# scale-lab/MTLoRA

Measured on AMD Instinct MI355X. Metric: images/sec (train step) Swin-T/448 r=64 4-task, higher is better.
Workload: dtype bf16; 1 GPU; BASELINE configs[1]: Swin-T 448, 4 tasks (semseg,normals,sal,human_parts), r_shared=64 r_task=4 scale4; train step (fwd+loss+bwd+clip+AdamW), dropout .05, drop_path .2; per_gpu_batch=32, global_batch=32, img_size=448, parallelism=dp1, trainable_params=8344634, allreduce_bytes=0

## Files before the change

### include/mtlora_hip.h

```cpp
#ifndef MTLORA_HIP_H
#define MTLORA_HIP_H

#include <stdint.h>

#ifdef __cplusplus
extern "C" {
#endif

#define MTLORA_ABI_VERSION 12
#define MTLORA_MAX_TASKS 8

typedef enum mtlora_dtype {
    MTLORA_F32 = 0,
    MTLORA_BF16 = 1,
    MTLORA_F16 = 2,
    MTLORA_U8 = 3
} mtlora_dtype;

typedef enum mtlora_status {
    MTLORA_OK = 0,
    MTLORA_ERR_DTYPE = -1,
    MTLORA_ERR_SHAPE = -2,
    MTLORA_ERR_ALIGN = -3,
    MTLORA_ERR_NULL = -4,
// ... 82 lines not shown
int mtlora_mlp_hid_proj(const mtlora_linear_desc* d1, const mtlora_linear_desc* d2, const void* h_base, const void* ctx1,
                        void* ctx2, void* scratch, int64_t scratch_bytes, void* stream);
int mtlora_mlp_hid_bwd(const mtlora_linear_desc* d1, const mtlora_linear_desc* d2, const void* h_base, const void* dh_s,
                       const void* ctx1, const void* ctx2, const void* scratch2, void* scratch1, void* g, float* const* dB1_t,
                       float* const* dA2_t, void* part, int64_t part_bytes, void* stream);

int64_t mtlora_gemm_tn_scratch_bytes(int64_t M, int Na, int Nb);
int mtlora_gemm_tn(const void* a, const void* b, float* out, int64_t M, int Na, int Nb, int64_t lda, int64_t ldb,
                   int dtype, void* scratch, int64_t scratch_bytes, void* stream);

typedef struct mtlora_attn_desc {
    int64_t B;
    int32_t H, W;
    int32_t window_size;
    int32_t shift;
    int32_t num_heads;
    int32_t head_dim;
    int32_t image_layout;
    int32_t dtype;
    float scale;
    float mask_value;
} mtlora_attn_desc;

int64_t mtlora_window_attn_bwd_scratch_bytes(const mtlora_attn_desc* d);

int mtlora_window_attn_fwd(const mtlora_attn_desc* d, const void* qkv, const float* bias, const float* mask,
                           const int32_t* mask_ids, void* out, void* stream);
int mtlora_window_attn_bwd(const mtlora_attn_desc* d, const void* qkv, const float* bias, const float* mask,
                           const int32_t* mask_ids, const void* dout, void* dqkv, float* dbias, void* scratch,
                           int64_t scratch_bytes, void* stream);

int mtlora_layernorm_fwd(const void* x, const float* gamma, const float* beta, void* y, float* mean, float* rstd,
                         int64_t M, int64_t C, float eps, int x_dtype, int y_dtype, int merge_h, int merge_w, void* stream);
int64_t mtlora_layernorm_bwd_scratch_bytes(int64_t M, int64_t C, int x_dtype);
int mtlora_layernorm_bwd(const void* dy, const void* x, const float* gamma, const float* mean, const float* rstd,
                         void* dx, float* dgamma, float* dbeta, int64_t M, int64_t C, int x_dtype, int dy_dtype,
                         void* scratch, int64_t scratch_bytes, const void* dx_addend, int merge_h, int merge_w, void* stream);

int mtlora_residual_layernorm_fwd(const void* shortcut, const void* branch, const float* scale, int64_t B, const float* gamma,
                                  const float* beta, void* x_new, void* y, float* mean, float* rstd, int64_t M, int64_t C,
                                  float eps, int x_dtype, int y_dtype, void* stream);
int mtlora_residual_layernorm_bwd(const void* dy, const void* x_new, const float* gamma, const float* mean, const float* rstd,
                                  void* d_shortcut, void* d_branch, float* dgamma, float* dbeta, const float* scale,
                                  int64_t B, int64_t M, int64_t C, int x_dtype, int dy_dtype, void* scratch,
                                  int64_t scratch_bytes, const void* dx_addend, void* stream);

int64_t mtlora_layernorm_multi_bwd_scratch_bytes(int n, int64_t M, int64_t C, int x_dtype);
int mtlora_layernorm_multi_fwd(int n, const void* const* x, const float* gamma, const float* beta, void* const* y,
                               float* const* mean, float* const* rstd, int64_t M, int64_t C, float eps, int x_dtype, int y_dtype,
                               int merge_h, int merge_w, void* stream);
int mtlora_layernorm_multi_bwd(int n, const void* const* dy, const void* const* x, const float* gamma, const float* const* mean,
                               const float* const* rstd, void* const* dx, float* dgamma, float* dbeta, int64_t M, int64_t C,
                               int x_dtype, int dy_dtype, void* scratch, int64_t scratch_bytes, const void* const* dx_addend,
                               int merge_h, int merge_w, void* stream);

int mtlora_residual_layernorm_streams_fwd(int n, const void* const* res, const void* const* branch, const float* scale,
                                          int64_t B, const float* gamma, const float* beta, void* const* x_new, void* const* y,
                                          float* const* mean, float* const* rstd, int64_t M, int64_t C, float eps, int x_dtype,
                                          int y_dtype, int merge_h, int merge_w, void* stream);
int mtlora_residual_layernorm_streams_bwd(int n, const void* const* dy, const void* const* x_new, const float* gamma,
                                          const float* const* mean, const float* const* rstd, void* const* d_res,
                                          void* const* d_branch, float* dgamma, float* dbeta, const float* scale, int64_t B,
                                          int64_t M, int64_t C, int x_dtype, int dy_dtype, void* scratch, int64_t scratch_bytes,
                                          const void* const* dx_addend, int merge_h, int merge_w, void* stream);

int mtlora_residual_layernorm_multi_fwd(int n, const void* shortcut, const void* const* branch, const float* scale, int64_t B,
                                        const float* gamma, const float* beta, void* const* x_new, void* const* y,
                                        float* const* mean, float* const* rstd, int64_t M, int64_t C, float eps, int x_dtype,
                                        int y_dtype, void* stream);
int mtlora_residual_layernorm_multi_bwd(int n, const void* const* dy, const void* const* x_new, const float* gamma,
                                        const float* const* mean, const float* const* rstd, const void* const* dx_addend,
                                        void* d_shortcut, void* const* d_branch, float* dgamma, float* dbeta, const float* scale,
                                        int64_t B, int64_t M, int64_t C, int x_dtype, int dy_dtype, void* scratch,
                                        int64_t scratch_bytes, void* stream);

int64_t mtlora_bn_scratch_bytes(int64_t R, int64_t C, int dtype);
int mtlora_bn_relu_fwd(const void* x, const float* gamma, const float* beta, float* running_mean, float* running_var,
                       float momentum, float eps, int relu, void* y, float* save_mean, float* save_rstd,
                       float* save_scale, float* save_shift, int64_t R, int64_t C, int dtype, void* scratch,
                       int64_t scratch_bytes, void* stream);
int mtlora_bn_relu_bwd(const void* dy, const void* x, const float* save_mean, const float* save_rstd,
                       const float* save_scale, const float* save_shift, int relu, void* dx, float* dgamma, float* dbeta,
                       int64_t R, int64_t C, int dtype, void* scratch, int64_t scratch_bytes, void* stream);

int mtlora_residual_droppath_fwd(int n, const void* const* res, const void* const* y, void* const* out,
                                 const float* scale, int64_t M, int64_t C, int64_t B, int res_dtype, int y_dtype,
                                 void* stream);
int mtlora_residual_droppath_bwd(int n, const void* const* g, void* const* dy, void* dres, const float* scale,
                                 int64_t M, int64_t C, int64_t B, int res_dtype, int y_dtype, void* stream);

int64_t mtlora_upsample_loss_partials(int64_t B, int h, int w, int scale);
int mtlora_upsample_loss(int kind, const void* low, const float* label, const float* stat, void* dlow, float* partials,
                         int64_t B, int h, int w, int C, int scale, int dtype, float ignore_index, void* stream);

int mtlora_upsample_metrics_sizes(int kind, int64_t B, int h, int w, int C, int scale, int64_t* n_int64,
                                  int64_t* n_float_partials);
int mtlora_upsample_metrics(int kind, const void* low, const float* label, const float* stat, int64_t* counts,
                            float* fpartials, int64_t B, int h, int w, int C, int scale, int dtype, float ignore_index,
                            void* stream);

int mtlora_upsample_predict(int kind, const void* low, void* out, int64_t B, int h, int w, int C, int scale, int dtype,
                            int out_dtype, void* stream);

int64_t mtlora_colsum_scratch_bytes(int64_t M, int64_t N);
int mtlora_colsum(const void* x, int64_t M, int64_t N, int dtype, float* out, void* scratch, int64_t scratch_bytes, void* stream);
int64_t mtlora_label_stat_scratch_bytes(int64_t n);
int mtlora_label_stat(const float* label, int64_t n, int kind, float ignore_index, float* out, void* scratch,
                      int64_t scratch_bytes, void* stream);

int mtlora_upsample_cl_fwd(const void* coarse, void* fine, int64_t B, int h, int w, int C, int scale, int64_t ld_fine,
                           int dtype, void* stream);
int mtlora_upsample_cl_bwd(const void* grad_fine, void* grad_coarse, int64_t B, int h, int w, int C, int scale,
                           int64_t ld_fine, int dtype, void* stream);

typedef struct mtlora_block_desc {
    int64_t B;
    int32_t H, W, C, hidden;
    int32_t num_heads, window_size, shift;
    int32_t dtype;
    int32_t x_dtype;
    int32_t has_norm1;
    float eps1, eps2, eps_next;
    float attn_scale, mask_value;
    mtlora_linear_desc lin[4];
} mtlora_block_desc;

typedef struct mtlora_block_params {
    const float *norm1_g, *norm1_b;
    const float *norm2_g, *norm2_b, *next_g, *next_b;
    const void* W[4];
    const void* Wt[4];
    const float* bias[4];
    const float* A[4];
    const float* Bf[4];
    const float* attn_bias;
    const int32_t* mask_ids;
    const float* mask;
    const float *scale1, *scale2;
} mtlora_block_params;

typedef struct mtlora_block_grads {
    void* g_x;
    void* g_normed;
    float *d_norm1_g, *d_norm1_b;
    float *d_norm2_g, *d_norm2_b, *d_next_g, *d_next_b;
    float* dA[4];
    float* dB[4];
    float* dbias;
} mtlora_block_grads;

int64_t mtlora_block_save_bytes(const mtlora_block_desc* d);
int64_t mtlora_block_fwd_tmp_bytes(const mtlora_block_desc* d);
int64_t mtlora_block_bwd_scratch_bytes(const mtlora_block_desc* d);
int mtlora_block_fwd(const mtlora_block_desc* d, const mtlora_block_params* p, const void* x, const void* normed, void* x_out,
                     void* normed_out, void* save, int64_t save_bytes, void* tmp, int64_t tmp_bytes, void* stream);
int mtlora_block_bwd(const mtlora_block_desc* d, const mtlora_block_params* p, const void* x, const void* normed,
                     const void* x_out, const void* g_x_out, const void* g_normed_out, const void* save, int64_t save_bytes,
                     const mtlora_block_grads* g, void* scratch, int64_t scratch_bytes, int phase, void* stream);

#define MTLORA_ADAMW_CHUNK 4096
#define MTLORA_ADAMW_MAX_GROUPS 16
#define MTLORA_ADAMW_CTRL_WORDS 64
#define MTLORA_ADAMW_GROUPS_DEV_BYTES 1152
typedef struct mtlora_adamw_group {
    double lr, beta1, beta2, eps, weight_decay;
} mtlora_adamw_group;
// ... 76 lines not shown
```

### mtlora_amd/_lib.py

```python
from __future__ import annotations

import ctypes
import os
from ctypes import POINTER, Structure, c_char_p, c_double, c_float, c_int, c_int32, c_int64, c_uint64, c_void_p

import torch

MAX_TASKS = 8
ABI_VERSION = 12
F32, BF16, F16, U8 = 0, 1, 2, 3
_DT = {torch.float32: F32, torch.bfloat16: BF16, torch.float16: F16}

_HERE = os.path.dirname(os.path.abspath(__file__))
LIB_PATH = os.path.join(_HERE, "csrc", "libmtlora_hip.so")


class LinearDesc(Structure):
    _fields_ = [("M", c_int64), ("K", c_int64), ("N", c_int64), ("dtype", c_int32), ("mode", c_int32),
                ("T", c_int32), ("r_s", c_int32), ("r_t", c_int32 * MAX_TASKS), ("scale_s", c_float),
                ("scale_t", c_float * MAX_TASKS), ("has_x_tasks", c_int32), ("dropout_p", c_float),
                ("seed", c_uint64), ("seed_offset", c_void_p), ("bwd_phase", c_int32),
                ("sel_stream", c_int32), ("sel_dense", c_int32), ("sel_tn", c_int32), ("sel_projk", c_int32),
                ("max_cu", c_int32), ("packed", c_void_p),
                ("hid", c_int32), ("hid_pad_", c_int32), ("hid_ptr", c_void_p)]
# ... 61 lines not shown


PtrArr = c_void_p * MAX_TASKS
PtrArr9 = c_void_p * (MAX_TASKS + 1)

_SIGS = {
    "mtlora_version": (c_int, []),
    "mtlora_error_string": (c_char_p, [c_int]),
    "mtlora_roll_and_window_partition_forward": (c_int, [c_void_p, c_void_p, c_int64, c_int64, c_int64, c_int64, c_int, c_int, c_int, c_void_p]),
    "mtlora_roll_and_window_partition_backward": (c_int, [c_void_p, c_void_p, c_int64, c_int64, c_int64, c_int64, c_int, c_int, c_int, c_void_p]),
    "mtlora_window_merge_and_roll_forward": (c_int, [c_void_p, c_void_p, c_int64, c_int64, c_int64, c_int64, c_int, c_int, c_int, c_void_p]),
    "mtlora_window_merge_and_roll_backward": (c_int, [c_void_p, c_void_p, c_int64, c_int64, c_int64, c_int64, c_int, c_int, c_int, c_void_p]),
    "mtlora_linear_ctx_bytes": (c_int64, [POINTER(LinearDesc)]),
    "mtlora_linear_bwd_scratch_bytes": (c_int64, [POINTER(LinearDesc)]),
    "mtlora_linear_packed_bytes": (c_int64, [POINTER(LinearDesc)]),
    "mtlora_linear_pack": (c_int, [POINTER(LinearDesc), c_void_p, c_void_p, POINTER(c_void_p), POINTER(c_void_p), c_void_p, c_int64,
                                   c_void_p]),
    "mtlora_linear_pack_entry_bytes": (c_int64, []),
    "mtlora_linear_pack_entry": (c_int, [POINTER(LinearDesc), c_void_p, c_void_p, POINTER(c_void_p), POINTER(c_void_p), c_void_p, c_int64,
                                         c_void_p]),
    "mtlora_linear_pack_table": (c_int, [c_void_p, c_int, c_int, c_void_p]),
    "mtlora_linear_fwd": (c_int, [POINTER(LinearDesc), c_void_p, POINTER(c_void_p), c_void_p, c_void_p, c_void_p, c_void_p,
                                  POINTER(c_void_p), POINTER(c_void_p), c_void_p, POINTER(c_void_p), c_void_p, c_int64,
                                  c_void_p]),
    "mtlora_linear_bwd": (c_int, [POINTER(LinearDesc), c_void_p, POINTER(c_void_p), c_void_p, c_void_p, POINTER(c_void_p),
                                  c_void_p, c_int64, c_void_p, POINTER(c_void_p), c_void_p, c_void_p, POINTER(c_void_p),
                                  POINTER(c_void_p), c_void_p, c_int64, c_void_p]),
    "mtlora_gemm_tn_scratch_bytes": (c_int64, [c_int64, c_int, c_int]),
    "mtlora_gemm_tn": (c_int, [c_void_p, c_void_p, c_void_p, c_int64, c_int, c_int, c_int64, c_int64, c_int, c_void_p, c_int64,
                               c_void_p]),
    "mtlora_linear_fwd_gelu": (c_int, [POINTER(LinearDesc), c_void_p, POINTER(c_void_p), c_void_p, c_void_p, c_void_p, c_void_p,
                                       POINTER(c_void_p), POINTER(c_void_p), c_void_p, POINTER(c_void_p), c_void_p,
                                       POINTER(c_void_p), c_void_p, c_int64, c_void_p]),
    "mtlora_linear_bwd_gelu": (c_int, [POINTER(LinearDesc), c_void_p, POINTER(c_void_p), c_void_p, c_void_p, POINTER(c_void_p),
                                       c_void_p, c_int64, c_void_p, POINTER(c_void_p), c_void_p, c_void_p, POINTER(c_void_p),
                                       POINTER(c_void_p), c_void_p, c_int64, c_void_p, POINTER(c_void_p), c_void_p]),
    "mtlora_mlp_hid_supported": (c_int, [POINTER(LinearDesc), POINTER(LinearDesc)]),
    "mtlora_mlp_hid_bwd_scratch_bytes": (c_int64, [POINTER(LinearDesc), POINTER(LinearDesc)]),
    "mtlora_mlp_hid_fwd_scratch_bytes": (c_int64, [POINTER(LinearDesc), POINTER(LinearDesc)]),
    "mtlora_mlp_hid_proj": (c_int, [POINTER(LinearDesc), POINTER(LinearDesc), c_void_p, c_void_p, c_void_p, c_void_p, c_int64, c_void_p]),
    "mtlora_mlp_hid_bwd": (c_int, [POINTER(LinearDesc), POINTER(LinearDesc), c_void_p, c_void_p, c_void_p, c_void_p, c_void_p, c_void_p,
                                   c_void_p, POINTER(c_void_p), POINTER(c_void_p), c_void_p, c_int64, c_void_p]),
    "mtlora_window_attn_bwd_scratch_bytes": (c_int64, [POINTER(AttnDesc)]),
    "mtlora_window_attn_fwd": (c_int, [POINTER(AttnDesc), c_void_p, c_void_p, c_void_p, c_void_p, c_void_p, c_void_p]),
    "mtlora_window_attn_bwd": (c_int, [POINTER(AttnDesc), c_void_p, c_void_p, c_void_p, c_void_p, c_void_p, c_void_p,
                                       c_void_p, c_void_p, c_int64, c_void_p]),
    "mtlora_layernorm_fwd": (c_int, [c_void_p, c_void_p, c_void_p, c_void_p, c_void_p, c_void_p, c_int64, c_int64, c_float,
                                     c_int, c_int, c_int, c_int, c_void_p]),
    "mtlora_layernorm_bwd_scratch_bytes": (c_int64, [c_int64, c_int64, c_int]),
    "mtlora_residual_layernorm_fwd": (c_int, [c_void_p, c_void_p, c_void_p, c_int64, c_void_p, c_void_p, c_void_p, c_void_p,
                                              c_void_p, c_void_p, c_int64, c_int64, c_float, c_int, c_int, c_void_p]),
    "mtlora_layernorm_multi_bwd_scratch_bytes": (c_int64, [c_int, c_int64, c_int64, c_int]),
    "mtlora_layernorm_multi_fwd": (c_int, [c_int, POINTER(c_void_p), c_void_p, c_void_p, POINTER(c_void_p), POINTER(c_void_p),
                                           POINTER(c_void_p), c_int64, c_int64, c_float, c_int, c_int, c_int, c_int, c_void_p]),
    "mtlora_layernorm_multi_bwd": (c_int, [c_int, POINTER(c_void_p), POINTER(c_void_p), c_void_p, POINTER(c_void_p),
                                           POINTER(c_void_p), POINTER(c_void_p), c_void_p, c_void_p, c_int64, c_int64, c_int,
                                           c_int, c_void_p, c_int64, POINTER(c_void_p), c_int, c_int, c_void_p]),
    "mtlora_residual_layernorm_streams_fwd": (c_int, [c_int, POINTER(c_void_p), POINTER(c_void_p), c_void_p, c_int64, c_void_p,
                                                      c_void_p, POINTER(c_void_p), POINTER(c_void_p), POINTER(c_void_p),
                                                      POINTER(c_void_p), c_int64, c_int64, c_float, c_int, c_int, c_int, c_int,
                                                      c_void_p]),
    "mtlora_residual_layernorm_streams_bwd": (c_int, [c_int, POINTER(c_void_p), POINTER(c_void_p), c_void_p, POINTER(c_void_p),
                                                      POINTER(c_void_p), POINTER(c_void_p), POINTER(c_void_p), c_void_p, c_void_p,
                                                      c_void_p, c_int64, c_int64, c_int64, c_int, c_int, c_void_p, c_int64,
                                                      POINTER(c_void_p), c_int, c_int, c_void_p]),
    "mtlora_residual_layernorm_multi_fwd": (c_int, [c_int, c_void_p, POINTER(c_void_p), c_void_p, c_int64, c_void_p, c_void_p,
                                                    POINTER(c_void_p), POINTER(c_void_p), POINTER(c_void_p), POINTER(c_void_p),
                                                    c_int64, c_int64, c_float, c_int, c_int, c_void_p]),
    "mtlora_residual_layernorm_multi_bwd": (c_int, [c_int, POINTER(c_void_p), POINTER(c_void_p), c_void_p, POINTER(c_void_p),
                                                    POINTER(c_void_p), POINTER(c_void_p), c_void_p, POINTER(c_void_p), c_void_p,
                                                    c_void_p, c_void_p, c_int64, c_int64, c_int64, c_int, c_int, c_void_p, c_int64,
                                                    c_void_p]),
    "mtlora_residual_layernorm_bwd": (c_int, [c_void_p, c_void_p, c_void_p, c_void_p, c_void_p, c_void_p, c_void_p, c_void_p,
                                              c_void_p, c_void_p, c_int64, c_int64, c_int64, c_int, c_int, c_void_p, c_int64,
                                              c_void_p, c_void_p]),
    "mtlora_layernorm_bwd": (c_int, [c_void_p, c_void_p, c_void_p, c_void_p, c_void_p, c_void_p, c_void_p, c_void_p,
                                     c_int64, c_int64, c_int, c_int, c_void_p, c_int64, c_void_p, c_int, c_int, c_void_p]),
    "mtlora_bn_scratch_bytes": (c_int64, [c_int64, c_int64, c_int]),
    "mtlora_bn_relu_fwd": (c_int, [c_void_p, c_void_p, c_void_p, c_void_p, c_void_p, c_float, c_float, c_int, c_void_p,
                                   c_void_p, c_void_p, c_void_p, c_void_p, c_int64, c_int64, c_int, c_void_p, c_int64,
                                   c_void_p]),
    "mtlora_bn_relu_bwd": (c_int, [c_void_p, c_void_p, c_void_p, c_void_p, c_void_p, c_void_p, c_int, c_void_p, c_void_p,
                                   c_void_p, c_int64, c_int64, c_int, c_void_p, c_int64, c_void_p]),
    "mtlora_residual_droppath_fwd": (c_int, [c_int, POINTER(c_void_p), POINTER(c_void_p), POINTER(c_void_p), c_void_p,
                                             c_int64, c_int64, c_int64, c_int, c_int, c_void_p]),
    "mtlora_residual_droppath_bwd": (c_int, [c_int, POINTER(c_void_p), POINTER(c_void_p), c_void_p, c_void_p, c_int64,
                                             c_int64, c_int64, c_int, c_int, c_void_p]),
    "mtlora_upsample_loss_partials": (c_int64, [c_int64, c_int, c_int, c_int]),
    "mtlora_colsum_scratch_bytes": (c_int64, [c_int64, c_int64]),
    "mtlora_colsum": (c_int, [c_void_p, c_int64, c_int64, c_int, c_void_p, c_void_p, c_int64, c_void_p]),
    "mtlora_label_stat_scratch_bytes": (c_int64, [c_int64]),
    "mtlora_label_stat": (c_int, [c_void_p, c_int64, c_int, c_float, c_void_p, c_void_p, c_int64, c_void_p]),
    "mtlora_upsample_loss": (c_int, [c_int, c_void_p, c_void_p, c_void_p, c_void_p, c_void_p, c_int64, c_int, c_int, c_int,
                                     c_int, c_int, ctypes.c_float, c_void_p]),
    "mtlora_upsample_metrics_sizes": (c_int, [c_int, c_int64, c_int, c_int, c_int, c_int, POINTER(c_int64), POINTER(c_int64)]),
    "mtlora_upsample_metrics": (c_int, [c_int, c_void_p, c_void_p, c_void_p, c_void_p, c_void_p, c_int64, c_int, c_int, c_int,
                                        c_int, c_int, ctypes.c_float, c_void_p]),
    "mtlora_upsample_predict": (c_int, [c_int, c_void_p, c_void_p, c_int64, c_int, c_int, c_int, c_int, c_int, c_int, c_void_p]),
    "mtlora_upsample_cl_fwd": (c_int, [c_void_p, c_void_p, c_int64, c_int, c_int, c_int, c_int, c_int64, c_int, c_void_p]),
    "mtlora_upsample_cl_bwd": (c_int, [c_void_p, c_void_p, c_int64, c_int, c_int, c_int, c_int, c_int64, c_int, c_void_p]),
    "mtlora_block_save_bytes": (c_int64, [POINTER(BlockDesc)]),
    "mtlora_block_fwd_tmp_bytes": (c_int64, [POINTER(BlockDesc)]),
    "mtlora_block_bwd_scratch_bytes": (c_int64, [POINTER(BlockDesc)]),
    "mtlora_block_fwd": (c_int, [POINTER(BlockDesc), POINTER(BlockParams), c_void_p, c_void_p, c_void_p, c_void_p, c_void_p, c_int64,
                                 c_void_p, c_int64, c_void_p]),
    "mtlora_block_bwd": (c_int, [POINTER(BlockDesc), POINTER(BlockParams), c_void_p, c_void_p, c_void_p, c_void_p, c_void_p, c_void_p,
                                 c_int64, POINTER(BlockGrads), c_void_p, c_int64, c_int, c_void_p]),
    "mtlora_adamw_sizes": (c_int, [c_int64, POINTER(c_int64), POINTER(c_int64), POINTER(c_int64), POINTER(c_int64)]),
    "mtlora_adamw_table": (c_int, [c_int64, POINTER(c_int64), POINTER(c_int32), POINTER(c_void_p), POINTER(c_void_p), POINTER(c_void_p),
                                   c_void_p, c_int64]),
    "mtlora_adamw_update": (c_int, [c_void_p, c_void_p, c_int64, c_int64, POINTER(AdamwGroup), c_int, c_float, c_void_p, c_void_p,
                                    c_void_p, c_void_p, c_float, c_float, c_int, c_void_p, c_int64, c_void_p]),
    "mtlora_adamw_update_dev": (c_int, [c_void_p, c_void_p, c_int64, c_int64, c_void_p, c_int, c_float, c_void_p, c_void_p,
                                        c_void_p, c_void_p, c_double, c_double, c_int, c_void_p, c_int64, c_void_p]),
    "mtlora_adamw_accum_layout": (c_int, [c_int64, POINTER(c_int64), POINTER(c_int64), POINTER(c_int64)]),
    "mtlora_adamw_accum_update_dev": (c_int, [c_void_p, c_void_p, c_int64, c_int64, c_void_p, c_int, c_float, c_void_p, c_void_p,
                                              c_void_p, c_void_p, c_double, c_double, c_int, c_void_p, c_int64, c_void_p, c_void_p,
                                              c_int, c_void_p]),
    "mtlora_ingest_scratch_bytes": (c_int64, [c_int, c_int64]),
    "mtlora_ingest_batch": (c_int, [POINTER(IngestJob), c_int, c_int64, c_int32, c_int32, c_void_p, c_void_p, c_void_p, c_int64,
                                    c_void_p]),
    "mtlora_augment_batch": (c_int, [POINTER(AugmentJob), c_int, c_int64, c_int32, c_int32, c_int32, c_int32, c_void_p, c_void_p,
                                     c_void_p, c_void_p, c_void_p, c_void_p]),
    "mtlora_selftest_layouts": (c_int, [c_void_p, c_void_p]),
    "mtlora_prof_begin": (c_int, [c_int]),
    "mtlora_prof_end": (c_int, [POINTER(ProfSummary)]),
    "mtlora_prof_kind_name": (c_char_p, [c_int]),
}
EXPORTS = tuple(_SIGS)

_lib = None


def lib() -> ctypes.CDLL:
    global _lib
    if _lib is None:
        if not os.path.exists(LIB_PATH):
            raise RuntimeError(
                f"mtlora_amd: {LIB_PATH} not found. Build it with `python -m mtlora_amd.csrc.build` "
                "(or __graft_entry__.build()). There is no eager/CPU fallback for the MTLoRA hot path.")
        L = ctypes.CDLL(LIB_PATH)
        for name, (res, args) in _SIGS.items():
            fn = getattr(L, name)
            fn.restype, fn.argtypes = res, args
        v = L.mtlora_version()
        if v != ABI_VERSION:
            raise RuntimeError(f"mtlora_amd: libmtlora_hip.so ABI {v} != binding ABI {ABI_VERSION}; rebuild")
        _lib = L
    return _lib


def check(status: int, what: str) -> None:
    if status != 0:
        msg = lib().mtlora_error_string(status).decode()
        raise RuntimeError(f"mtlora_amd: {what} failed: {msg} (status {status})")


def dtype_code(t: torch.Tensor, allow_f16: bool = True) -> int:
    code = _DT.get(t.dtype)
    if code is None or (code == F16 and not allow_f16):
        raise RuntimeError(f"mtlora_amd: unsupported dtype {t.dtype} (fp32, bf16 and fp16 are supported)")
    return code


def require_gpu(*tensors: torch.Tensor) -> None:
    cur = None
# ... 41 lines not shown
```

### mtlora_amd/csrc/dense.h

```cpp
#pragma once

#include "nt.h"
#include "stream.h"

namespace {

constexpr int ND_TM = 256, ND_TN = 128, ND_KE = 64;
constexpr int ND_ROWS = ND_TM + ND_TN;
constexpr int ND_STAGE = ND_ROWS * 128;
constexpr int ND_NST = 3;
constexpr int ND_LDS = ND_NST * ND_STAGE;
constexpr int ND_DPW = ND_ROWS / 8 / 8;
constexpr int ND_OPS = ND_DPW;
constexpr int ND_ORS = 128 + 8;

template <bool ACT, bool MLR, bool GATE>
__global__ __launch_bounds__(512, 2) void k_ntd(const NlParams P) {
    constexpr int EPI_OPS = 8 * (1 + (ACT ? 1 : 0));
    extern __shared__ __attribute__((aligned(16))) unsigned char smem[];
    const int tid = threadIdx.x, lane = tid & 63, wave = __builtin_amdgcn_readfirstlane(tid >> 6);
    const int wm = wave >> 1, wn = wave & 1;
    const int h = lane >> 5, rl = lane & 31;
    const int M = P.M, n_rows = P.n_rows, Kb = P.K, seg_lo = P.seg_lo, seg_hi = P.seg_hi, n_tiles = P.n_tiles;
    const uint32_t q8 = P.q8, r8 = P.r8, nt_magic = P.nt_magic;
// ... 170 lines not shown
                            }
                    }
                }
            }
            slot = slot == ND_NST - 1 ? 0 : slot + 1;
        }
        const int img_slot = slot >= 1 ? slot - 1 : ND_NST - 1;
        const int m0c = m0, n0c = n0;
        {
            const uint32_t nt = tile + gridDim.x;
            if (nt < n_wg_tiles) {
                tile_coords(nt, m0, n0);
                set_rows(m0, n0);
                issue(0, slot);
                if (total > 1) issue(1, slot == ND_NST - 1 ? 0 : slot + 1);
            }
        }
        base_slot = slot;
        first = false;

        if (!bias_first && (alpha || bias) && use_base) {
#pragma unroll
            for (int sn = 0; sn < 2; ++sn)
#pragma unroll
                for (int q = 0; q < 4; ++q) {
                    int n = n0c + wn * 64 + sn * 32 + 8 * q + 4 * h;
                    n = n < n_rows - 4 ? n : n_rows - 4;
                    f32x4 al = {1.f, 1.f, 1.f, 1.f}, bi = {0.f, 0.f, 0.f, 0.f};
                    if (alpha) al = *reinterpret_cast<const f32x4*>(alpha + n);
                    if (bias) bi = *reinterpret_cast<const f32x4*>(bias + n);
#pragma unroll
                    for (int sm = 0; sm < 2; ++sm)
#pragma unroll
                        for (int e = 0; e < 4; ++e) acc[sn][sm][q * 4 + e] = acc[sn][sm][q * 4 + e] * al[e] + bi[e];
                }
        }

        __syncthreads();
        unsigned char* img = smem + img_slot * ND_STAGE + wave * (32 * ND_ORS);
        const int c16 = lane & 7;
        const int n = n0c + wn * 64 + c16 * 8;
#pragma unroll
        for (int sm = 0; sm < 2; ++sm) {
#pragma unroll
            for (int sn = 0; sn < 2; ++sn)
#pragma unroll
                for (int q = 0; q < 4; ++q) {
                    const int nl = sn * 32 + 8 * q + 4 * h;
                    u32x2 pk = {mtl_pack_bf16(acc[sn][sm][q * 4], acc[sn][sm][q * 4 + 1]),
                                mtl_pack_bf16(acc[sn][sm][q * 4 + 2], acc[sn][sm][q * 4 + 3])};
                    *reinterpret_cast<u32x2*>(img + rl * ND_ORS + nl * 2) = pk;
                }
            __builtin_amdgcn_s_waitcnt(0xc07f);
            __builtin_amdgcn_wave_barrier();
#pragma unroll
            for (int it = 0; it < 4; ++it) {
                const int ml = it * 8 + (lane >> 3);
                const int m = m0c + wm * 64 + sm * 32 + ml;
                u32x4 v = *reinterpret_cast<const u32x4*>(img + ml * ND_ORS + c16 * 16);
                const uint32_t off = (m < M && n < n_rows) ? (uint32_t)m * ldo2 + (uint32_t)n * 2u : 0xFFFFFFFFu;
                if constexpr (GATE) {
                    v = mtl_gelu_gate_pk4<bf16, false>(v, hv[sm][it]);
                }
                sp_bstore(v, orsrc, off);
                if constexpr (ACT) {
                    const u32x4 av = mtl_gelu_pk4<bf16, false>(v);
                    sp_bstore(av, arsrc, off);
                }
            }
            __builtin_amdgcn_wave_barrier();
        }
    }
}


constexpr int NE_TM = 256, NE_TN = 128, NE_KE = 32;
constexpr int NE_ROWS = NE_TM + NE_TN;
constexpr int NE_STAGE = NE_ROWS * 64;
constexpr int NE_NST = 3;
constexpr int NE_LDS = NE_NST * NE_STAGE;
constexpr int NE_DPW = NE_ROWS / 16 / 4;
constexpr int NE_ORS = 128 + 8;

template <bool ACT, bool MLR, bool GATE>
__global__ __launch_bounds__(256, 2) void k_nte(const NlParams P) {
    constexpr int EPI_OPS = 16 * (1 + (ACT ? 1 : 0)) + (GATE ? 16 : 0);
    extern __shared__ __attribute__((aligned(16))) unsigned char smem[];
    const int tid = threadIdx.x, lane = tid & 63, wave = __builtin_amdgcn_readfirstlane(tid >> 6);
    const int wm = wave >> 1, wn = wave & 1;
    const int h = lane >> 5, rl = lane & 31;
    const int M = P.M, n_rows = P.n_rows, Kb = P.K, seg_lo = P.seg_lo, seg_hi = P.seg_hi, n_tiles = P.n_tiles;
    const uint32_t q8 = P.q8, r8 = P.r8, nt_magic = P.nt_magic;
    const unsigned char* const wgt_b = reinterpret_cast<const unsigned char*>(P.wgt);
    const unsigned char* const act_b = reinterpret_cast<const unsigned char*>(P.act);
    const unsigned char* const wgt_r = reinterpret_cast<const unsigned char*>(P.Rm);
    const unsigned char* const act_r = reinterpret_cast<const unsigned char*>(P.L);
    const uint32_t ldw_b = (uint32_t)(P.ld_wgt * 2), lda_b = (uint32_t)(P.ld_act * 2), ldw_r = (uint32_t)(P.ldR * 2), lda_r = (uint32_t)(P.ldL * 2);
    const uint32_t ldo2 = (uint32_t)(P.ld_out * 2);
    const float* const bias = P.bias;
    const float* const alpha = P.alpha;
    const int use_base = P.use_base;
    DropoutCfg drop = P.drop;
    mtl_dropout_resolve(drop);
    const __amdgpu_buffer_rsrc_t orsrc = sp_rsrc(P.out, (int64_t)M * P.ld_out * 2);
    const __amdgpu_buffer_rsrc_t arsrc = sp_rsrc(P.act2, ACT ? (int64_t)M * P.ld_out * 2 : 0);
    const __amdgpu_buffer_rsrc_t grsrc = sp_rsrc(const_cast<bf16*>(P.gate), GATE ? (int64_t)M * P.ld_out * 2 : 0);
    (void)arsrc;
    (void)grsrc;

    const int n1 = seg_hi > seg_lo ? (seg_hi - seg_lo + NE_KE - 1) / NE_KE : 0;
    const int n2 = (use_base && Kb > 0) ? (Kb + NE_KE - 1) / NE_KE : 0;
    const int total = n1 + n2;
    const uint32_t n_wg_tiles = q8 * 8u + r8;
    if (total == 0) return;

    int co[2];
#pragma unroll
    for (int ks = 0; ks < 2; ++ks) co[ks] = (((2 * ks + h) ^ ((rl >> 2) & 3)) << 4) + rl * 64;
    const int w_off = (wn * 64) * 64, a_off = (NE_TN + wm * 128) * 64;

    uint32_t rowc[NE_DPW], q16[NE_DPW];
#pragma unroll
    for (int t = 0; t < NE_DPW; ++t) {
        const int row = 16 * (wave + 4 * t) + (lane >> 2), p = lane & 3;
        q16[t] = (uint32_t)((p ^ ((row >> 2) & 3)) * 16);
    }
    auto tile_coords = [&](uint32_t tile, int& m0, int& n0) __attribute__((always_inline)) {
        uint32_t b = tile;
        b = ((b & 7u) < r8 ? (b & 7u) * (q8 + 1u) : r8 * (q8 + 1u) + ((b & 7u) - r8) * q8) + (b >> 3);
        const uint32_t bm = n_tiles == 1 ? b : __umulhi(b, nt_magic);
        m0 = (int)bm * NE_TM;
        n0 = (int)(b - bm * (uint32_t)n_tiles) * NE_TN;
    };
    auto set_rows = [&](int m0, int n0) __attribute__((always_inline)) {
#pragma unroll
        for (int t = 0; t < NE_DPW; ++t) {
            const int j = wave + 4 * t, row = 16 * j + (lane >> 2);
            if (j < NE_TN / 16) {
                const int wr = n0 + row;
                rowc[t] = (uint32_t)(wr < n_rows ? wr : n_rows - 1);
            } else {
                const int ar = m0 + row - NE_TN;
                rowc[t] = (uint32_t)(ar < M ? ar : M - 1);
            }
        }
    };
    auto issue = [&](int i, int slot) __attribute__((always_inline)) {
        const bool lr = i < n1;
        const int k0 = lr ? seg_lo + i * NE_KE : (i - n1) * NE_KE;
        const int khi = lr ? seg_hi : Kb;
        unsigned char* dst = smem + slot * NE_STAGE;
        const unsigned char* wb = (lr ? wgt_r : wgt_b) + (int64_t)k0 * 2;
        const unsigned char* ab = (lr ? act_r : act_b) + (int64_t)k0 * 2;
        const uint32_t ldw2 = lr ? ldw_r : ldw_b, lda2 = lr ? lda_r : lda_b;
        if (k0 + NE_KE <= khi) {
#pragma unroll
            for (int t = 0; t < NE_DPW; ++t) {
                const int j = wave + 4 * t;
                const bool isw = j < NE_TN / 16;
                sp_dma16((isw ? wb : ab) + (rowc[t] * (isw ? ldw2 : lda2) + q16[t]), dst + j * 1024);
            }
        } else {
#pragma unroll
            for (int t = 0; t < NE_DPW; ++t) {
                const int j = wave + 4 * t;
                const bool isw = j < NE_TN / 16;
                const void* g = k0 + (int)(q16[t] >> 1) < khi ? (const void*)((isw ? wb : ab) + (rowc[t] * (isw ? ldw2 : lda2) + q16[t]))
                                                              : (const void*)g_zero16;
// ... 35 lines not shown
            const bool nxt = i + 1 < total, epi = !first && i < 2;
            if (nxt && epi)
                SP_WAIT_VM(NE_DPW + EPI_OPS);
            else if (epi)
                SP_WAIT_VM(EPI_OPS);
            else if (nxt)
                SP_WAIT_VM(NE_DPW);
            else
                SP_WAIT_VM(0);
            __syncthreads();
            if (i + 2 < total) issue(i + 2, slot >= 1 ? slot - 1 : slot + 2);
            const unsigned char* st = smem + slot * NE_STAGE;
            const unsigned char* sw = st + w_off;
            const unsigned char* sa = st + a_off;
#pragma unroll
            for (int ks = 0; ks < 2; ++ks) {
                u32x4 fw[2], fa[4];
#pragma unroll
                for (int bq = 0; bq < 2; ++bq) fw[bq] = *reinterpret_cast<const u32x4*>(sw + bq * 32 * 64 + co[ks]);
#pragma unroll
                for (int bq = 0; bq < 4; ++bq) fa[bq] = *reinterpret_cast<const u32x4*>(sa + bq * 32 * 64 + co[ks]);
#pragma unroll
                for (int sm = 0; sm < 4; ++sm)
#pragma unroll
                    for (int sn = 0; sn < 2; ++sn) sp_mma1<bf16>(fw[sn], fa[sm], acc[sn][sm]);
            }
            if constexpr (MLR) {
                if (i + 1 == n1 && drop.thr16 != 0) {
#pragma unroll
                    for (int sm = 0; sm < 4; ++sm) {
                        const uint32_t rh = mtl_dropout_rowhash(drop, 0u, (uint32_t)(m0 + wm * 128 + sm * 32 + rl));
#pragma unroll
                        for (int sn = 0; sn < 2; ++sn)
#pragma unroll
                            for (int q = 0; q < 4; ++q) {
                                const int n = n0 + wn * 64 + sn * 32 + 8 * q + 4 * h;
                                const uint32_t h0 = mtl_dropout_pairbits(drop, rh, (uint32_t)n);
                                const uint32_t h1 = mtl_dropout_pairbits(drop, rh, (uint32_t)(n + 2));
                                if ((h0 & 0xFFFFu) < drop.thr16) acc[sn][sm][q * 4 + 0] = 0.f;
                                if ((h0 >> 16) < drop.thr16) acc[sn][sm][q * 4 + 1] = 0.f;
                                if ((h1 & 0xFFFFu) < drop.thr16) acc[sn][sm][q * 4 + 2] = 0.f;
                                if ((h1 >> 16) < drop.thr16) acc[sn][sm][q * 4 + 3] = 0.f;
                            }
                    }
                }
            }
            slot = slot == NE_NST - 1 ? 0 : slot + 1;
        }
        const int img_slot = slot >= 1 ? slot - 1 : NE_NST - 1;
        const int m0c = m0, n0c = n0;
        {
            const uint32_t nt = tile + gridDim.x;
            if (nt < n_wg_tiles) {
                tile_coords(nt, m0, n0);
                set_rows(m0, n0);
                issue(0, slot);
                if (total > 1) issue(1, slot == NE_NST - 1 ? 0 : slot + 1);
            }
        }
        base_slot = slot;
        first = false;

        if (!bias_first && (alpha || bias) && use_base) {
#pragma unroll
            for (int sn = 0; sn < 2; ++sn)
#pragma unroll
                for (int q = 0; q < 4; ++q) {
                    int n = n0c + wn * 64 + sn * 32 + 8 * q + 4 * h;
                    n = n < n_rows - 4 ? n : n_rows - 4;
                    f32x4 al = {1.f, 1.f, 1.f, 1.f}, bi = {0.f, 0.f, 0.f, 0.f};
                    if (alpha) al = *reinterpret_cast<const f32x4*>(alpha + n);
                    if (bias) bi = *reinterpret_cast<const f32x4*>(bias + n);
#pragma unroll
                    for (int sm = 0; sm < 4; ++sm)
#pragma unroll
                        for (int e = 0; e < 4; ++e) acc[sn][sm][q * 4 + e] = acc[sn][sm][q * 4 + e] * al[e] + bi[e];
                }
        }

        __syncthreads();
        unsigned char* img = smem + img_slot * NE_STAGE + wave * (32 * NE_ORS);
        const int c16 = lane & 7;
        const int n = n0c + wn * 64 + c16 * 8;
#pragma unroll
        for (int sm = 0; sm < 4; ++sm) {
            u32x4 hv[4];
            (void)hv;
            if constexpr (GATE) {
#pragma unroll
                for (int it = 0; it < 4; ++it) {
                    const int m = m0c + wm * 128 + sm * 32 + it * 8 + (lane >> 3);
                    const uint32_t off = (m < M && n < n_rows) ? (uint32_t)m * ldo2 + (uint32_t)n * 2u : 0xFFFFFFFFu;
                    hv[it] = __builtin_amdgcn_raw_buffer_load_b128(grsrc, (int)off, 0, 0);
                }
            }
#pragma unroll
            for (int sn = 0; sn < 2; ++sn)
#pragma unroll
                for (int q = 0; q < 4; ++q) {
                    const int nl = sn * 32 + 8 * q + 4 * h;
                    u32x2 pk = {mtl_pack_bf16(acc[sn][sm][q * 4], acc[sn][sm][q * 4 + 1]),
                                mtl_pack_bf16(acc[sn][sm][q * 4 + 2], acc[sn][sm][q * 4 + 3])};
                    *reinterpret_cast<u32x2*>(img + rl * NE_ORS + nl * 2) = pk;
                }
            __builtin_amdgcn_s_waitcnt(0xc07f);
            __builtin_amdgcn_wave_barrier();
#pragma unroll
            for (int it = 0; it < 4; ++it) {
                const int ml = it * 8 + (lane >> 3);
                const int m = m0c + wm * 128 + sm * 32 + ml;
                u32x4 v = *reinterpret_cast<const u32x4*>(img + ml * NE_ORS + c16 * 16);
                const uint32_t off = (m < M && n < n_rows) ? (uint32_t)m * ldo2 + (uint32_t)n * 2u : 0xFFFFFFFFu;
                if constexpr (GATE) {
                    v = mtl_gelu_gate_pk4<bf16, false>(v, hv[it]);
                }
                sp_bstore(v, orsrc, off);
                if constexpr (ACT) {
                    const u32x4 av = mtl_gelu_pk4<bf16, false>(v);
                    sp_bstore(av, arsrc, off);
                }
            }
            __builtin_amdgcn_wave_barrier();
        }
    }
}

}
```

### mtlora_amd/csrc/glue.hip

```cpp
#include "common.h"
#include "internal.h"
#include "vec.h"

namespace {

struct BnParams {
    const void* x;
    const void* dy;
    void* y;
    void* dx;
    const float* gamma;
    const float* beta;
    float* running_mean;
    float* running_var;
    float* mean;
    float* rstd;
    float* scale;
    float* shift;
    float* part;
    float* dgamma;
    float* dbeta;
    float* c1;
    float* c2;
    int64_t R;
// ... 160 lines not shown
    constexpr int UN = 4;
    const int tid = threadIdx.x;
    const int ro = tid / p.VW, v = tid % p.VW;
    if (ro >= p.rows_per_iter) return;
    const T* x = reinterpret_cast<const T*>(p.x);
    const T* dy = reinterpret_cast<const T*>(p.dy);
    T* out = reinterpret_cast<T*>(BWD ? p.dx : p.y);
    float sc[VE], sh[VE], kx[VE], k0[VE];
#pragma unroll
    for (int e = 0; e < VE; ++e) {
        const int c = v * VE + e;
        sc[e] = p.scale[c];
        sh[e] = p.shift[c];
        if (BWD) {
            const float t = sc[e] * p.c2[c] * p.rstd[c];
            kx[e] = -t;
            k0[e] = t * p.mean[c] - sc[e] * p.c1[c];
        }
    }
    const int64_t rows_blk = mtl_ceil_div(p.R, (int64_t)gridDim.x);
    const int64_t r_lo = (int64_t)blockIdx.x * rows_blk;
    int64_t r_hi = r_lo + rows_blk;
    if (r_hi > p.R) r_hi = p.R;
    for (int64_t r = r_lo + ro; r < r_hi; r += (int64_t)UN * p.rows_per_iter) {
        u32x4 rx[UN], rg[UN];
#pragma unroll
        for (int u = 0; u < UN; ++u) {
            const int64_t rr = r + (int64_t)u * p.rows_per_iter;
            const bool ok = rr < r_hi;
            rx[u] = ok ? *reinterpret_cast<const u32x4*>(x + rr * p.C + v * VE) : u32x4{0u, 0u, 0u, 0u};
            if (BWD) rg[u] = ok ? *reinterpret_cast<const u32x4*>(dy + rr * p.C + v * VE) : u32x4{0u, 0u, 0u, 0u};
        }
#pragma unroll
        for (int u = 0; u < UN; ++u) {
            const int64_t rr = r + (int64_t)u * p.rows_per_iter;
            if (rr >= r_hi) continue;
            float fx[8], o[8];
            cvt_vec<T>(rx[u], fx);
            if (!BWD) {
#pragma unroll
                for (int e = 0; e < VE; ++e) {
                    const float yv = fx[e] * sc[e] + sh[e];
                    o[e] = (p.relu && yv < 0.f) ? 0.f : yv;
                }
            } else {
                float fg[8];
                cvt_vec<T>(rg[u], fg);
#pragma unroll
                for (int e = 0; e < VE; ++e) {
                    const float yv = fx[e] * sc[e] + sh[e];
                    const float g = (p.relu && yv <= 0.f) ? 0.f : fg[e];
                    o[e] = sc[e] * g + kx[e] * fx[e] + k0[e];
                }
            }
            st_vec<T, VE>(out + rr * p.C + v * VE, o);
        }
    }
}

int bn_setup(BnParams& p, int64_t R, int64_t C, int dtype) {
    if (dtype != MTLORA_F32 && dtype != MTLORA_BF16 && dtype != MTLORA_F16) return MTLORA_ERR_DTYPE;
    const int ve = dtype == MTLORA_F32 ? 4 : 8;
    if (R <= 0 || C <= 0 || C % ve) return MTLORA_ERR_SHAPE;
    p.R = R;
    p.C = (int)C;
    p.VW = (int)(C / ve);
    if (p.VW > 512) return MTLORA_ERR_UNSUPPORTED;
    p.rows_per_iter = 512 / p.VW;
    if (p.rows_per_iter > 8) p.rows_per_iter = 8;
    int64_t nblk = mtl_ceil_div(R, 64);
    if (nblk > 512) nblk = 512;
    p.nblk = (int)nblk;
    return MTLORA_OK;
}

}

extern "C" {

int64_t mtlora_bn_scratch_bytes(int64_t R, int64_t C, int dtype) {
    BnParams p = {};
    if (bn_setup(p, R, C, dtype) != MTLORA_OK) return -1;
    return ((int64_t)p.nblk * 2 * C + 4 * C) * 4 + 256;
}

int mtlora_bn_relu_fwd(const void* x, const float* gamma, const float* beta, float* running_mean, float* running_var,
                       float momentum, float eps, int relu, void* y, float* save_mean, float* save_rstd,
                       float* save_scale, float* save_shift, int64_t R, int64_t C, int dtype, void* scratch,
                       int64_t scratch_bytes, void* stream) {
    BnParams p = {};
    int st = bn_setup(p, R, C, dtype);
    if (st != MTLORA_OK) return st;
    if (!x || !gamma || !beta || !y || !save_mean || !save_rstd || !save_scale || !save_shift || !scratch)
        return MTLORA_ERR_NULL;
    if (((uintptr_t)x | (uintptr_t)y | (uintptr_t)scratch) & 15u) return MTLORA_ERR_ALIGN;
    if (scratch_bytes < mtlora_bn_scratch_bytes(R, C, dtype) - 256) return MTLORA_ERR_WORKSPACE;
    p.x = x;
    p.y = y;
    p.gamma = gamma;
    p.beta = beta;
    p.running_mean = running_mean;
    p.running_var = running_var;
    p.mean = save_mean;
    p.rstd = save_rstd;
    p.scale = save_scale;
    p.shift = save_shift;
    p.part = reinterpret_cast<float*>(scratch);
    p.momentum = momentum;
    p.eps = eps;
    p.relu = relu;
    hipStream_t s = (hipStream_t)stream;
    const int threads = (int)mtl_round_up((int64_t)p.rows_per_iter * p.VW, 64);
    const unsigned apply_blocks = (unsigned)(mtl_ceil_div(R, 16) < BN_APPLY_BLOCKS ? mtl_ceil_div(R, 16) : BN_APPLY_BLOCKS);
    const size_t lds = (size_t)p.rows_per_iter * 2 * C * 4;
    const int es = mtl_elem_size(dtype);
    {
        MtlProfScope prof(PK_BN, (double)R * C * es, s);
        if (dtype == MTLORA_F32)
            hipLaunchKernelGGL((k_bn_colsum<float, false>), dim3(p.nblk), dim3(threads), lds, s, p);
        else if (dtype == MTLORA_F16)
            hipLaunchKernelGGL((k_bn_colsum<f16, false>), dim3(p.nblk), dim3(threads), lds, s, p);
        else
            hipLaunchKernelGGL((k_bn_colsum<bf16, false>), dim3(p.nblk), dim3(threads), lds, s, p);
    }
    hipLaunchKernelGGL(k_bn_finalize, dim3((unsigned)mtl_ceil_div(C, 64)), dim3(64 * BN_FW), 0, s, p);
    {
        MtlProfScope prof(PK_BN, (double)R * C * es * 2, s);
        if (dtype == MTLORA_F32)
            hipLaunchKernelGGL((k_bn_apply<float, false>), dim3(apply_blocks), dim3(threads), 0, s, p);
        else if (dtype == MTLORA_F16)
            hipLaunchKernelGGL((k_bn_apply<f16, false>), dim3(apply_blocks), dim3(threads), 0, s, p);
        else
            hipLaunchKernelGGL((k_bn_apply<bf16, false>), dim3(apply_blocks), dim3(threads), 0, s, p);
    }
    MTL_CHECK_LAUNCH();
    return MTLORA_OK;
}

int mtlora_bn_relu_bwd(const void* dy, const void* x, const float* save_mean, const float* save_rstd,
                       const float* save_scale, const float* save_shift, int relu, void* dx, float* dgamma, float* dbeta,
                       int64_t R, int64_t C, int dtype, void* scratch, int64_t scratch_bytes, void* stream) {
    BnParams p = {};
    int st = bn_setup(p, R, C, dtype);
    if (st != MTLORA_OK) return st;
    if (!dy || !x || !save_mean || !save_rstd || !save_scale || !save_shift || !dx || !dgamma || !dbeta || !scratch)
        return MTLORA_ERR_NULL;
    if (((uintptr_t)x | (uintptr_t)dy | (uintptr_t)dx | (uintptr_t)scratch) & 15u) return MTLORA_ERR_ALIGN;
    if (scratch_bytes < mtlora_bn_scratch_bytes(R, C, dtype) - 256) return MTLORA_ERR_WORKSPACE;
    p.x = x;
    p.dy = dy;
    p.dx = dx;
    p.mean = const_cast<float*>(save_mean);
    p.rstd = const_cast<float*>(save_rstd);
    p.scale = const_cast<float*>(save_scale);
    p.shift = const_cast<float*>(save_shift);
    p.part = reinterpret_cast<float*>(scratch);
    p.c1 = p.part + (int64_t)p.nblk * 2 * C;
    p.c2 = p.c1 + C;
    p.dgamma = dgamma;
    p.dbeta = dbeta;
    p.relu = relu;
    hipStream_t s = (hipStream_t)stream;
    const int threads = (int)mtl_round_up((int64_t)p.rows_per_iter * p.VW, 64);
    const unsigned apply_blocks = (unsigned)(mtl_ceil_div(R, 16) < BN_APPLY_BLOCKS ? mtl_ceil_div(R, 16) : BN_APPLY_BLOCKS);
    const size_t lds = (size_t)p.rows_per_iter * 2 * C * 4;
    const int es = mtl_elem_size(dtype);
    {
        MtlProfScope prof(PK_BN, (double)R * C * es * 2, s);
        if (dtype == MTLORA_F32)
            hipLaunchKernelGGL((k_bn_colsum<float, true>), dim3(p.nblk), dim3(threads), lds, s, p);
        else if (dtype == MTLORA_F16)
            hipLaunchKernelGGL((k_bn_colsum<f16, true>), dim3(p.nblk), dim3(threads), lds, s, p);
        else
            hipLaunchKernelGGL((k_bn_colsum<bf16, true>), dim3(p.nblk), dim3(threads), lds, s, p);
    }
    hipLaunchKernelGGL(k_bn_bwd_finalize, dim3((unsigned)mtl_ceil_div(C, 64)), dim3(64 * BN_FW), 0, s, p);
    {
        MtlProfScope prof(PK_BN, (double)R * C * es * 3, s);
        if (dtype == MTLORA_F32)
            hipLaunchKernelGGL((k_bn_apply<float, true>), dim3(apply_blocks), dim3(threads), 0, s, p);
        else if (dtype == MTLORA_F16)
            hipLaunchKernelGGL((k_bn_apply<f16, true>), dim3(apply_blocks), dim3(threads), 0, s, p);
        else
            hipLaunchKernelGGL((k_bn_apply<bf16, true>), dim3(apply_blocks), dim3(threads), 0, s, p);
    }
    MTL_CHECK_LAUNCH();
    return MTLORA_OK;
}
}

namespace {

struct ResParams {
    const void* res[MTLORA_MAX_TASKS + 1];
    const void* y[MTLORA_MAX_TASKS + 1];
    void* out[MTLORA_MAX_TASKS + 1];
    void* dres;
    const float* scale;
    int64_t M;
    int C, n, B;
    int64_t rows_per_sample;
};

template <typename TR, typename TY>
__global__ __launch_bounds__(256) void k_residual_fwd(const ResParams p) {
    const int64_t nvec = p.M * p.C / 8;
    const int k = blockIdx.y;
    const TR* res = reinterpret_cast<const TR*>(p.res[k]);
    const TY* y = reinterpret_cast<const TY*>(p.y[k]);
    TR* out = reinterpret_cast<TR*>(p.out[k]);
    for (int64_t i = (int64_t)blockIdx.x * 256 + threadIdx.x; i < nvec; i += (int64_t)gridDim.x * 256) {
        const int64_t row = (i * 8) / p.C;
        const float s = p.scale ? p.scale[(int64_t)k * p.B + row / p.rows_per_sample] : 1.f;
        float fr[8], fy[8], o[8];
        if constexpr (sizeof(TR) == 4) {
            ld_vec<TR>(res + i * 8, fr);
            float hi[8];
            ld_vec<TR>(res + i * 8 + 4, hi);
#pragma unroll
// ... 155 lines not shown
```

### mtlora_amd/csrc/linear.hip

```cpp
#include <string.h>
#include <algorithm>
#include <atomic>
#include <type_traits>

#include "common.h"
#include "internal.h"
#include "hid_params.h"
#include "nt.h"
#include "stream.h"
#include "dense.h"
#include "pq.h"
#include "tn.h"

namespace {

static Segs make_segs(const mtlora_linear_desc* d) {
    Segs s;
    s.n = 1 + d->T;
    int off = 0;
    for (int o = 0; o < s.n; ++o) {
        int r = (o == 0) ? d->r_s : d->r_t[o - 1];
        s.r[o] = r;
        s.rp[o] = (int)mtl_round_up(r, 8);
        s.off[o] = off;
// ... 56 lines not shown
};
static Tune make_tune(const mtlora_linear_desc* d) {
    auto tri = [](int v) { return v == 1 ? 0 : (v == 2 ? 2 : 1); };
    Tune t;
    t.sp = d->sel_stream == 1 ? 0 : 1;
    t.ntd = d->sel_dense >= 3 ? d->sel_dense : tri(d->sel_dense);
    t.tn = tri(d->sel_tn);
    t.projk = d->sel_projk == 3 ? 3 : tri(d->sel_projk);
    t.max_cu = d->max_cu > 0 ? d->max_cu : 0;
    return t;
}
constexpr int MTL_MAX_DEV = 64;
static int cur_dev() {
    int dev = 0;
    (void)hipGetDevice(&dev);
    return dev >= 0 && dev < MTL_MAX_DEV ? dev : 0;
}
static int dev_num_cu() {
    static std::atomic<int> cache[MTL_MAX_DEV];
    const int dev = cur_dev();
    int cu = cache[dev].load(std::memory_order_relaxed);
    if (cu == 0) {
        cu = 256;
        (void)hipDeviceGetAttribute(&cu, hipDeviceAttributeMultiprocessorCount, dev);
        if (cu <= 0) cu = 256;
        cache[dev].store(cu, std::memory_order_relaxed);
    }
    return cu;
}
static int num_cu(const Tune& tu) {
    const int cu = dev_num_cu();
    return tu.max_cu > 0 && tu.max_cu < cu ? tu.max_cu : cu;
}
static bool raise_lds(std::atomic<unsigned long long>& done, const void* fn, int bytes) {
    const int dev = cur_dev();
    if ((done.load(std::memory_order_relaxed) >> dev) & 1ull) return true;
    if (hipFuncSetAttribute(fn, hipFuncAttributeMaxDynamicSharedMemorySize, bytes) != hipSuccess) {
        (void)hipGetLastError();
        return false;
    }
    done.fetch_or(1ull << dev, std::memory_order_relaxed);
    return true;
}
#define MTL_RAISE_LDS(KERNEL, BYTES)                                        \
    do {                                                                    \
        static std::atomic<unsigned long long> done__{0};                   \
        (void)raise_lds(done__, (const void*)(KERNEL), (int)(BYTES));       \
    } while (0)

static bool nte_prefer(int64_t tiles, int ksteps, int64_t cus) {
    const double eff_d = (double)tiles / (double)(mtl_ceil_div(tiles, cus) * cus);
    return (ksteps >= 4 && ksteps <= 12 && tiles * 2 >= 3 * cus) || (ksteps >= 6 && eff_d < 0.7 && tiles >= cus);
}

static NlParams make_nl(const NtParams& P, int64_t mt, int64_t nt, bool dense) {
    NlParams q;
    q.act = reinterpret_cast<const bf16*>(P.act[0]);
    q.wgt = reinterpret_cast<const bf16*>(P.wgt);
    q.L = reinterpret_cast<const bf16*>(P.L);
    q.Rm = reinterpret_cast<const bf16*>(P.Rm);
    q.out = reinterpret_cast<bf16*>(P.out[0].ptr);
    q.act2 = reinterpret_cast<bf16*>(P.out[0].act);
    q.gate = dense ? reinterpret_cast<const bf16*>(P.out[0].gate) : nullptr;
    q.bias = P.bias;
    q.alpha = P.alpha;
    q.ld_act = P.ld_act;
    q.ld_wgt = P.ld_wgt;
    q.ldL = P.ldL;
    q.ldR = P.ldR;
    q.ld_out = P.ld_out;
    q.M = (int)P.M;
    q.n_rows = P.n_rows;
    q.K = P.act[0] ? P.K : 0;
    q.seg_lo = P.L ? P.out[0].seg_lo : 0;
    q.seg_hi = P.L ? P.out[0].seg_hi : 0;
    q.n_tiles = (int)nt;
    q.nt_magic = (uint32_t)(((uint64_t)1 << 32) / (uint64_t)nt) + 1u;
    const uint32_t nwg = (uint32_t)(mt * nt);
    q.q8 = nwg / 8u;
    q.r8 = nwg % 8u;
    q.act_mask = dense ? 0 : P.act_mask;
    q.use_base = P.out[0].use_base;
    q.drop = P.drop;
    return q;
}

template <typename F>
static void nl_dispatch(const NlParams& q, bool ml0, F&& go) {
    using Y = std::true_type;
    using N = std::false_type;
    if (q.act2)
        go(Y{}, N{}, N{});
    else if (q.gate && ml0)
        go(N{}, Y{}, Y{});
    else if (q.gate)
        go(N{}, N{}, Y{});
    else if (ml0)
        go(N{}, Y{}, N{});
    else
        go(N{}, N{}, N{});
}

template <typename T>
static void launch_nt(const Tune& tu, const NtParams& P, hipStream_t s, int kind, double alg_bytes, double s8d_bytes = 0.0, double flops = 0.0) {
    mtl_prof_tag("M%lld K%d N%d ldL%lld no%d na%d nz%d", (long long)P.M, P.K, P.n_rows, (long long)P.ldL, P.n_out, P.n_act, P.nz);
    MtlProfScope prof(kind, alg_bytes, s, s8d_bytes, flops);
    int max_rows = P.n_rows;
    if (P.nz > 0) {
        max_rows = 0;
        for (int z = 0; z < P.nz; ++z) max_rows = P.zrows[z] > max_rows ? P.zrows[z] : max_rows;
    }
    const int64_t m_tiles = mtl_ceil_div(P.M, TILE);
    const int64_t n_tiles = mtl_ceil_div(max_rows, TILE);
    if (m_tiles * n_tiles == 0) return;
    dim3 g((unsigned)(m_tiles * n_tiles), 1, (unsigned)(P.nz > 0 ? P.nz : 1));
    int base_users = 0;
    for (int o = 0; o < P.n_out; ++o) base_users += P.out[o].use_base ? 1 : 0;
    const size_t lds = (size_t)STAGE_BYTES;
    const int variant = base_users > 1 ? 0 : (P.n_act > 1 ? 1 : 2);
    constexpr bool W8 = sizeof(T) == 2;
    bool mlr = false, gated = false, acted = false;
    for (int o = 0; o < P.n_out; ++o) {
        mlr = mlr || P.out[o].mask_lr != 0;
        gated = gated || P.out[o].gate != nullptr;
        acted = acted || P.out[o].act != nullptr;
    }
    mlr = mlr && P.drop.enabled();
    if constexpr (std::is_same<T, bf16>::value) {
        const int ntd_mode = tu.ntd;
        bool dense = false, use_e = false;
        int ksteps = 0;
        if (variant == 2 && P.n_out == 1 && P.nz == 0 && ntd_mode != 0 && P.act_mask == 0 && P.n_rows % 8 == 0 && P.n_rows >= 64 &&
            P.M < (int64_t)0x7FFFFF00 && P.out[0].ptr != nullptr && !(P.out[0].gate && P.out[0].act)) {
            const int seg = P.L ? P.out[0].seg_hi - P.out[0].seg_lo : 0;
            const int kk = (P.act[0] && P.out[0].use_base ? P.K : 0);
            ksteps = (seg + ND_KE - 1) / ND_KE + (kk + ND_KE - 1) / ND_KE;
            const int64_t tiles = mtl_ceil_div(P.M, ND_TM) * mtl_ceil_div(P.n_rows, ND_TN);
            const int64_t lim = ((int64_t)1 << 32) - 4096;
            const bool fits = P.M * P.ld_out * 2 < lim && P.M * P.ld_act * 2 < lim && P.M * P.ldL * 2 < lim && (int64_t)P.n_rows * P.ld_wgt * 2 < lim &&
                              (int64_t)P.n_rows * P.ldR * 2 < lim && P.K % 8 == 0 && seg % 8 == 0 && (P.ld_act % 8) == 0 && (P.ld_wgt % 8) == 0 &&
                              (P.ldL % 8) == 0 && (P.ldR % 8) == 0 && (P.L == nullptr || (P.out[0].seg_lo % 8) == 0);
            const int64_t slots = num_cu(tu);
            const double eff = (double)tiles / (double)(mtl_ceil_div(tiles, slots) * slots);
            use_e = ntd_mode == 3 || (ntd_mode == 1 && nte_prefer(tiles, ksteps, slots) && (P.n_rows % ND_TN == 0 || P.n_rows > 2 * ND_TN));
            dense = fits && ksteps >= 1 &&
                    (ntd_mode == 2 || ntd_mode == 3 || use_e ||
                     (ksteps >= 6 && (eff >= 0.7 || (tiles <= slots && tiles >= slots / 2)) && (P.n_rows % ND_TN == 0 || P.n_rows > 2 * ND_TN)));
        }
        if (dense) {
            const int64_t mt = mtl_ceil_div(P.M, ND_TM), nt = mtl_ceil_div(P.n_rows, ND_TN);
            const NlParams q = make_nl(P, mt, nt, true);
            const bool ml0 = P.out[0].mask_lr != 0 && P.drop.enabled() && q.seg_hi > q.seg_lo;
            const uint32_t nwg = (uint32_t)(mt * nt), cus = (uint32_t)num_cu(tu);
            nl_dispatch(q, ml0, [&](auto ac, auto ml, auto ga) {
                constexpr bool AC = decltype(ac)::value, ML = decltype(ml)::value, GA = decltype(ga)::value;
                if (use_e) {
                    MTL_RAISE_LDS((k_nte<AC, ML, GA>), SP_LDS_MAX);
                    hipLaunchKernelGGL((k_nte<AC, ML, GA>), dim3(nwg < 2u * cus ? nwg : 2u * cus), dim3(256), (size_t)NE_LDS, s, q);
                } else {
                    MTL_RAISE_LDS((k_ntd<AC, ML, GA>), SP_LDS_MAX);
                    hipLaunchKernelGGL((k_ntd<AC, ML, GA>), dim3(nwg < cus ? nwg : cus), dim3(512), (size_t)ND_LDS, s, q);
                }
            });
            return;
        }
        if (variant == 2 && P.n_out == 1 && P.out[0].gate == nullptr && P.nz == 0 && P.M < (int64_t)0x7FFFFF00 &&
            m_tiles * n_tiles < ((int64_t)1 << 28) && P.n_rows >= 8 && P.n_rows % 8 == 0) {
            if (P.out[0].ptr == nullptr) return;
            const int64_t t128 = m_tiles * mtl_ceil_div(P.n_rows, 128), t192 = m_tiles * mtl_ceil_div(P.n_rows, 192);
            const int64_t slots = 2 * (int64_t)dev_num_cu();
            const double c128 = (double)mtl_ceil_div(t128, slots), c192 = 1.5 * (double)mtl_ceil_div(t192, slots);
            const bool wide = !P.out[0].act && P.n_rows >= 192 && c192 < c128 - 0.01;
            const int64_t nt = wide ? mtl_ceil_div(P.n_rows, 192) : n_tiles;
            const NlParams q = make_nl(P, m_tiles, nt, false);
            const bool ml0 = P.out[0].mask_lr != 0 && P.drop.enabled() && q.seg_hi > q.seg_lo;
            const uint32_t nwg = (uint32_t)(m_tiles * nt);
            constexpr size_t LDS192 = (size_t)(192 + 128) * LDSB;
#define MTL_NTL_GO(AC, ML, SNV, LDSV)                                                         \
    do {                                                                                      \
        if ((LDSV) > 64 * 1024) MTL_RAISE_LDS((k_ntl<AC, ML, SNV>), 160 * 1024 - 512);        \
        hipLaunchKernelGGL((k_ntl<AC, ML, SNV>), dim3(nwg), dim3(512), (size_t)(LDSV), s, q); \
    } while (0)
            if (q.act2)
                MTL_NTL_GO(true, false, 2, STAGE_BYTES);
            else if (wide && ml0)
                MTL_NTL_GO(false, true, 3, LDS192);
            else if (wide)
                MTL_NTL_GO(false, false, 3, LDS192);
            else if (ml0)
                MTL_NTL_GO(false, true, 2, STAGE_BYTES);
            else
                MTL_NTL_GO(false, false, 2, STAGE_BYTES);
#undef MTL_NTL_GO
            return;
        }
    }
#define MTL_NT_GO(MU, MSRC, ML, GA, AC)                                                                   \
    do {                                                                                                \
        if (W8 && !(MU))                                                                                \
            hipLaunchKernelGGL((k_nt<T, false, MSRC, ML, 8, GA, AC>), g, dim3(512), lds, s, P);         \
        else                                                                                            \
            hipLaunchKernelGGL((k_nt<T, MU, MSRC, ML, 4, GA, AC>), g, dim3(256), lds, s, P);            \
    } while (0)
    if (acted) {
        if (variant == 0)
            MTL_NT_GO(true, false, false, false, true);
        else
            MTL_NT_GO(false, false, false, false, true);
    } else if (gated) {
        if (variant == 1)
            MTL_NT_GO(false, true, true, true, false);
        else if (mlr)
            MTL_NT_GO(false, false, true, true, false);
        else
            MTL_NT_GO(false, false, false, true, false);
    } else if (variant == 0) {
        MTL_NT_GO(true, false, false, false, false);
    } else if (variant == 1) {
        MTL_NT_GO(false, true, true, false, false);
    } else if (mlr) {
        MTL_NT_GO(false, false, true, false, false);
    } else {
        MTL_NT_GO(false, false, false, false, false);
    }
#undef MTL_NT_GO
}

template <typename T>
static int sp_proj_plan(const Tune& tu, SpProjParams& q, int& ch) {
    if (sizeof(T) != 2 || tu.sp == 0 || q.M <= 0 || q.n_src <= 0) return 0;
    ch = q.K % 96 == 0 ? 96 : (q.K % 64 == 0 ? 64 : 0);
    if (ch == 0 || q.M >= ((int64_t)1 << 31) - 64) return 0;
    q.n_blk_total = (q.Rw + 31) / 32;
    for (int s = 0; s < q.n_src; ++s) {
        if (q.src[s].n_blk > SP_MAXB || q.src[s].n_blk <= 0) return 0;
        if (((uintptr_t)q.src[s].act & 15u) != 0) return 0;
    }
    if ((q.ld_out % 8) != 0 || ((uintptr_t)q.out & 15u) != 0 || ((uintptr_t)q.wproj & 15u) != 0) return 0;
    if (q.M * q.ld_out * 2 >= ((int64_t)1 << 32) - 64) return 0;
    q.n_slabs = (int)mtl_ceil_div(q.M, 32);
    if ((int64_t)q.n_slabs * q.n_src >= ((int64_t)1 << 30)) return 0;
    q.n_items = q.n_slabs * q.n_src;
    const int64_t wbytes = (int64_t)q.n_blk_total * 32 * q.K * 2;
    const int64_t slot = 32 * ch * 2;
    for (int ns = 3; ns >= 1; --ns)
        if (wbytes + (int64_t)SP_WAVES * ns * slot <= SP_LDS_MAX) return ns;
    return 0;
}
template <typename T>
static void launch_sp_proj(const Tune& tu, const SpProjParams& q, int ch, int ns, hipStream_t s, int kind, double alg_bytes, double s8d, double flops) {
    mtl_prof_tag("sp_proj M%lld K%d R%d src%d ch%d ns%d", (long long)q.M, q.K, q.Rw, q.n_src, ch, ns);
    MtlProfScope prof(kind, alg_bytes, s, s8d, flops);
    const size_t lds = (size_t)q.n_blk_total * 32 * q.K * 2 + (size_t)SP_WAVES * ns * 32 * ch * 2;
    const int per_cu = lds * 2 <= (size_t)SP_LDS_MAX ? 2 : 1;
    int64_t wgs = mtl_ceil_div(q.n_items, SP_WAVES);
    if (wgs > (int64_t)num_cu(tu) * per_cu) wgs = (int64_t)num_cu(tu) * per_cu;
#define MTL_SP_PROJ(CHV, NSV)                                                                              \
    do {                                                                                                   \
        MTL_RAISE_LDS((k_sp_proj<T, CHV, NSV>), SP_LDS_MAX);                                               \
        hipLaunchKernelGGL((k_sp_proj<T, CHV, NSV>), dim3((unsigned)wgs), dim3(64 * SP_WAVES), lds, s, q); \
    } while (0)
    if constexpr (sizeof(T) == 2) {
        if (ch == 96) {
            if (ns == 3) MTL_SP_PROJ(96, 3);
            else if (ns == 2) MTL_SP_PROJ(96, 2);
            else MTL_SP_PROJ(96, 1);
        } else {
            if (ns == 3) MTL_SP_PROJ(64, 3);
            else if (ns == 2) MTL_SP_PROJ(64, 2);
            else MTL_SP_PROJ(64, 1);
        }
    }
#undef MTL_SP_PROJ
}

template <typename T>
static int pq_plan(const Tune& tu, const SpProjParams& q, PqParams& pq) {
    if (sizeof(T) != 2 || tu.sp == 0 || tu.projk == 0 || tu.projk == 2 || q.M <= 0 || q.n_src < 1 || q.n_src > MAXO) return 0;
    if (q.Rw % 8 != 0 || q.K % 8 != 0 || q.K < 32 || (q.ld_out % 8) != 0) return 0;
    if ((((uintptr_t)q.wproj | (uintptr_t)q.out) & 15u) != 0) return 0;
    if (q.M >= ((int64_t)1 << 31) - 256 || q.M * q.ld_out * 2 >= ((int64_t)1 << 32) - 64) return 0;
    int wmax = 0;
    for (int s = 0; s < q.n_src; ++s) {
        const SpSrc& ss = q.src[s];
        if (((uintptr_t)ss.act & 15u) != 0 || ss.col_lo % 8 != 0 || ss.col_hi % 8 != 0 || ss.col_hi <= ss.col_lo || ss.col_hi > q.Rw) return 0;
        if (ss.col_hi - ss.col_lo > 1024) return 0;
        pq.src[s].act = ss.act;
// ... 514 lines not shown
    } else if (mb > 0) {
        launch_pq<T>(pq, mb, s, j.kind, j.alg_bytes, j.s8d, j.flops);
    } else {
        NtParams q = {};
        q.n_act = 1;
        q.ld_act = j.K;
        q.wgt = j.wcat;
        q.ld_wgt = j.K;
        q.M = j.M;
        q.K = j.K;
        q.alpha = j.alpha;
        q.n_out = 1;
        q.out[0].ptr = j.out;
        q.out[0].use_base = 1;
        q.ld_out = sg.R;
        q.drop = dc;
        if (j.one_panel) {
            q.act[0] = src[0].act;
            q.act_mask = src[0].mask;
            q.n_rows = sg.R;
        } else {
            for (int i = 0; i < n_src; ++i) {
                q.zact[i] = src[i].act;
                q.zrow0[i] = src[i].col_lo;
                q.zrows[i] = src[i].col_hi - src[i].col_lo;
                q.zmask[i] = src[i].mask;
            }
            q.nz = n_src;
        }
        launch_nt<T>(tu, q, s, j.kind, j.alg_bytes, j.s8d, j.flops);
    }
}

static double rank_sum(const Segs& sg, const void* const* live = nullptr) {
    double rsum = 0.0;
    for (int o = 0; o < sg.n; ++o)
        if (!live || (sg.rp[o] > 0 && live[o])) rsum += sg.r[o];
    return rsum;
}
static double fused_bytes(const mtlora_linear_desc* d, int es) { return (double)es * d->M * (d->K + (double)d->N); }
static double fused_flops(const mtlora_linear_desc* d, const Segs& sg) {
    return 2.0 * d->M * (double)d->K * d->N + 2.0 * d->M * (double)sg.r[0] * (d->K + d->N);
}

template <typename T>
static bool fwd_one_pass(const mtlora_linear_desc* d, const Tune& tu, const Segs& sg, const CtxLayout& L, const unsigned char* pk, const void* x,
                         const void* W, const float* bias, void* y_s, void* a_s, T* Pm, const DropoutCfg& dc, hipStream_t s) {
    SpLinParams q = {};
    q.act = x;
    q.w = W;
    q.proj = pk + L.a_proj;
    q.expand = pk + L.b_frag;
    q.bias = bias;
    q.out = y_s;
    q.out2 = a_s;
    q.pout = Pm;
    q.ld_out = d->N;
    q.ldp = sg.R;
    q.M = d->M;
    q.n_cols = (int)d->N;
    q.R = sg.R;
    q.mask_act = 1;
    q.mask_lr = 0;
    q.drop = dc;
    SpXresPlan pl;
    const double b8d = fused_bytes(d, (int)sizeof(T)), fl = fused_flops(d, sg);
    if (sp_xres_plan<T>(tu, q, (int)d->K, pl)) {
        launch_sp_xres<T>(q, pl, a_s != nullptr, s, PK_NT_FWD_MAIN, b8d + (a_s ? (double)sizeof(T) * d->M * d->N : 0.0), b8d, fl);
        return true;
    }
    SpAresPlan pa;
    q.estep = q.estep2 = 0;
    if (a_s == nullptr && sp_ares_plan<T>(tu, q, (int)d->K, pa)) {
        launch_sp_ares<T>(q, pa, s, PK_NT_FWD_MAIN, b8d, b8d, fl);
        return true;
    }
    return false;
}

template <typename T>
static int fwd_impl(const mtlora_linear_desc* d, const void* x, const void* const* x_t, const void* W,
                    const float* bias, const float* A_s, const float* B_s, const float* const* A_t,
                    const float* const* B_t, void* y_s, void* const* y_t, void* ctx, hipStream_t s, void* a_s = nullptr,
                    void* const* a_t = nullptr) {
    const Segs sg = make_segs(d);
    const Tune tu = make_tune(d);
    const CtxLayout L = ctx_layout(d, sg);
    unsigned char* c = reinterpret_cast<unsigned char*>(ctx);
    unsigned char* pk = d->packed ? const_cast<unsigned char*>(reinterpret_cast<const unsigned char*>(d->packed)) : c;
    T* a_cat = reinterpret_cast<T*>(pk + L.a_cat);
    T* b_cat = reinterpret_cast<T*>(pk + L.b_cat);
    float* alpha = reinterpret_cast<float*>(pk + L.alpha);
    T* Pm = reinterpret_cast<T*>(c + L.p);
    const DropoutCfg dc = mtl_make_dropout(d->dropout_p, d->seed, d->seed_offset);

    if (sg.R > 0) {
        if (!d->packed) launch_pack<T>(d, sg, L, pk, A_s, B_s, A_t, B_t, s);
        if (d->T == 0 && d->mode == 0 && fwd_one_pass<T>(d, tu, sg, L, pk, x, W, bias, y_s, a_s, Pm, dc, s)) return MTLORA_OK;

        const bool own = d->T > 0 && d->has_x_tasks;
        ProjSrc src[MAXO];
        int n_src = 0;
        if (!own) src[n_src++] = ProjSrc{x, 0, sg.used, 1};
        for (int o = 0; own && o < sg.n; ++o) {
            if (sg.rp[o] == 0) continue;
            if (o > 0 && (d->hid & MTLORA_HID_P_GIVEN)) continue;
            src[n_src++] = ProjSrc{o == 0 ? x : x_t[o - 1], sg.off[o], sg.off[o] + sg.rp[o], o == 0 ? 1 : 0};
        }
        const double xb = (double)sizeof(T) * ((d->has_x_tasks && !(d->hid & MTLORA_HID_P_GIVEN)) ? d->T : 0) * d->M * d->K;
        ProjJob<T> j = {};
        j.wproj = pk + L.a_proj;
        j.wcat = a_cat;
        j.alpha = alpha;
        j.out = Pm;
        j.M = d->M;
        j.K = (int)d->K;
        j.one_panel = !own;
        j.kind = PK_NT_FWD_P;
        j.alg_bytes = j.s8d = xb;
        j.flops = 2.0 * d->M * d->K * rank_sum(sg);
        launch_proj<T>(tu, sg, dc, s, src, n_src, j);
    }

    NtParams m = {};
    m.act[0] = x;
    m.n_act = 1;
    m.ld_act = d->K;
    m.wgt = W;
    m.ld_wgt = d->K;
    m.M = d->M;
    m.n_rows = (int)d->N;
    m.K = (int)d->K;
    m.bias = bias;
    m.L = Pm;
    m.ldL = sg.R;
    m.Rm = b_cat;
    m.ldR = sg.R;
    m.ld_out = d->N;
    m.drop = dc;
    m.n_out = 1 + d->T;
    for (int o = 0; o < sg.n; ++o) {
        NtOut& O = m.out[o];
        O.ptr = (o == 0) ? y_s : y_t[o - 1];
        O.seg_lo = sg.off[o];
        O.seg_hi = sg.off[o] + sg.rp[o];
        O.use_base = 1;
        O.mask_lr = 0;
        O.fold = (o == 0 && d->mode == 1 && d->T > 0) ? 1 : 0;
        O.act = (o == 0) ? a_s : (a_t ? a_t[o - 1] : nullptr);
    }
    if (d->hid & MTLORA_HID_FWD_BASE) {
        m.n_out = 2;
        NtOut& O = m.out[1];
        O.ptr = const_cast<void*>(d->hid_ptr);
        O.seg_lo = O.seg_hi = 0;
        O.use_base = 1;
        O.mask_lr = 0;
        O.fold = 0;
        O.act = nullptr;
    }
    int n_actout = 0;
    for (int o = 0; o < m.n_out; ++o) n_actout += m.out[o].act ? 1 : 0;
    const double b8d = (double)sizeof(T) * d->M * (d->K + (double)(1 + d->T) * d->N);
    const double fl = 2.0 * d->M * d->K * d->N + 2.0 * d->M * d->N * rank_sum(sg);
    const bool plain = sg.R == 0;
    launch_nt<T>(tu, m, s, plain ? PK_NT_PLAIN_FWD : PK_NT_FWD_MAIN, b8d + (double)sizeof(T) * d->M * (double)n_actout * d->N,
                 plain ? 0.0 : b8d, fl);
    return MTLORA_OK;
}

constexpr int64_t TN_TARGET_CTAS = 512;
struct BwdScratch {
    int64_t q, g, part, total;
    int nsplit;
    int64_t rows_per_split;
};
static BwdScratch bwd_scratch(const mtlora_linear_desc* d, const Segs& sg) {
    const int es = mtl_elem_size(d->dtype);
    BwdScratch S;
    int64_t o = 0;
    auto take = [&](int64_t bytes) {
        int64_t at = o;
        o += mtl_round_up(bytes, 256);
        return at;
    };
    S.q = take(d->M * sg.R * es);
    S.g = take(d->T > 0 ? d->M * d->N * es : 0);
    int64_t tiles = 0;
    for (int oo = 0; oo < sg.n; ++oo) {
        if (sg.rp[oo] == 0) continue;
        tiles += mtl_ceil_div(sg.rp[oo], TN_A) * mtl_ceil_div(d->N, TN_B);
        tiles += mtl_ceil_div(sg.rp[oo], TN_A) * mtl_ceil_div(d->K, TN_B);
    }
    int nsplit = 1;
    if (tiles > 0) {
        nsplit = (int)(TN_TARGET_CTAS / tiles);
        const int64_t max_by_rows = mtl_ceil_div(d->M, 256);
        if (nsplit > max_by_rows) nsplit = (int)max_by_rows;
        if (nsplit > 256) nsplit = 256;
        if (nsplit < 1) nsplit = 1;
    }
    S.nsplit = nsplit;
    int64_t rps = mtl_ceil_div(d->M > 0 ? d->M : 1, nsplit);
    rps = mtl_round_up(rps, 64);
    S.rows_per_split = rps;
    {
        const int64_t tiled = tiles * nsplit * (int64_t)TN_TILE * 4, streamed = sp_tn_part_bytes(d, sg);
        S.part = take(tiled > streamed ? tiled : streamed);
    }
    S.total = o;
    return S;
}

template <typename T>
struct Bwd {
    const mtlora_linear_desc* d;
    Segs sg;
    Tune tu;
    CtxLayout L;
    BwdScratch S;
    hipStream_t s;
    DropoutCfg dc;
// ... 790 lines not shown
    memcpy(entry_host, &e, sizeof(e));
    return MTLORA_OK;
}

int mtlora_linear_pack_table(const void* table_dev, int n_entries, int dtype, void* stream) {
    if (dtype != MTLORA_F32 && dtype != MTLORA_BF16 && dtype != MTLORA_F16) return MTLORA_ERR_DTYPE;
    if (n_entries < 0 || n_entries > 65535) return MTLORA_ERR_SHAPE;
    if (n_entries == 0) return MTLORA_OK;
    if (!table_dev) return MTLORA_ERR_NULL;
    if (((uintptr_t)table_dev & 7u) != 0) return MTLORA_ERR_ALIGN;
    hipStream_t s = (hipStream_t)stream;
    const PackEntry* tb = reinterpret_cast<const PackEntry*>(table_dev);
    MtlProfScope prof(PK_PACK, 0.0, s);
    const dim3 g(256, (unsigned)n_entries);
    if (dtype == MTLORA_F32)
        hipLaunchKernelGGL(k_pack_table<float>, g, dim3(256), 0, s, tb);
    else if (dtype == MTLORA_F16)
        hipLaunchKernelGGL(k_pack_table<f16>, g, dim3(256), 0, s, tb);
    else
        hipLaunchKernelGGL(k_pack_table<bf16>, g, dim3(256), 0, s, tb);
    MTL_CHECK_LAUNCH();
    return MTLORA_OK;
}

static int linear_fwd_entry(const mtlora_linear_desc* d, const void* x, const void* const* x_t, const void* W,
                            const float* bias, const float* A_s, const float* B_s, const float* const* A_t,
                            const float* const* B_t, void* y_s, void* const* y_t, void* a_s, void* const* a_t, void* ctx,
                            int64_t ctx_bytes, void* stream) {
    int st = check_desc(d);
    if (st != MTLORA_OK) return st;
    if (!x || !W || !y_s) return MTLORA_ERR_NULL;
    if (d->r_s > 0 && !d->packed && (!A_s || !B_s)) return MTLORA_ERR_NULL;
    if (misaligned(x) || misaligned(W) || misaligned(y_s) || misaligned(bias) || misaligned(d->packed)) return MTLORA_ERR_ALIGN;
    const bool hid_base = (d->hid & MTLORA_HID_FWD_BASE) != 0, hid_p = (d->hid & MTLORA_HID_P_GIVEN) != 0;
    if (hid_base && (!d->hid_ptr || d->T < 1 || !d->has_x_tasks || d->mode != 0)) return MTLORA_ERR_NULL;
    if (hid_base && misaligned(d->hid_ptr)) return MTLORA_ERR_ALIGN;
    if (hid_p && (d->T < 1 || !d->has_x_tasks || d->mode != 0)) return MTLORA_ERR_UNSUPPORTED;
    for (int t = 0; t < d->T; ++t) {
        if (!hid_base && (!y_t || !y_t[t])) return MTLORA_ERR_NULL;
        if (!d->packed && (!A_t || !B_t || !A_t[t] || !B_t[t])) return MTLORA_ERR_NULL;
        if (!hid_base && misaligned(y_t[t])) return MTLORA_ERR_ALIGN;
        if (d->has_x_tasks && !hid_p && (!x_t || !x_t[t])) return MTLORA_ERR_NULL;
        if (d->has_x_tasks && !hid_p && misaligned(x_t[t])) return MTLORA_ERR_ALIGN;
    }
    const Segs sg = make_segs(d);
    if (sg.R > 0) {
        if (!ctx) return MTLORA_ERR_NULL;
        if (misaligned(ctx)) return MTLORA_ERR_ALIGN;
        if (ctx_bytes < ctx_layout(d, sg).total) return MTLORA_ERR_WORKSPACE;
    }
    if (d->M == 0) return MTLORA_OK;
    hipStream_t s = (hipStream_t)stream;
    if (d->dtype == MTLORA_F32)
        st = fwd_impl<float>(d, x, x_t, W, bias, A_s, B_s, A_t, B_t, y_s, y_t, ctx, s, a_s, a_t);
    else if (d->dtype == MTLORA_F16)
        st = fwd_impl<f16>(d, x, x_t, W, bias, A_s, B_s, A_t, B_t, y_s, y_t, ctx, s, a_s, a_t);
    else
        st = fwd_impl<bf16>(d, x, x_t, W, bias, A_s, B_s, A_t, B_t, y_s, y_t, ctx, s, a_s, a_t);
    if (st != MTLORA_OK) return st;
    MTL_CHECK_LAUNCH();
    return MTLORA_OK;
}

int mtlora_linear_fwd(const mtlora_linear_desc* d, const void* x, const void* const* x_t, const void* W,
                      const float* bias, const float* A_s, const float* B_s, const float* const* A_t,
                      const float* const* B_t, void* y_s, void* const* y_t, void* ctx, int64_t ctx_bytes,
                      void* stream) {
    return linear_fwd_entry(d, x, x_t, W, bias, A_s, B_s, A_t, B_t, y_s, y_t, nullptr, nullptr, ctx, ctx_bytes, stream);
}

int mtlora_linear_fwd_gelu(const mtlora_linear_desc* d, const void* x, const void* const* x_t, const void* W,
                           const float* bias, const float* A_s, const float* B_s, const float* const* A_t,
                           const float* const* B_t, void* y_s, void* const* y_t, void* a_s, void* const* a_t, void* ctx,
                           int64_t ctx_bytes, void* stream) {
    if (!a_s || !d) return MTLORA_ERR_NULL;
    if (misaligned(a_s)) return MTLORA_ERR_ALIGN;
    for (int t = 0; t < d->T && !(d->hid & MTLORA_HID_FWD_BASE); ++t) {
        if (!a_t || !a_t[t]) return MTLORA_ERR_NULL;
        if (misaligned(a_t[t])) return MTLORA_ERR_ALIGN;
    }
    return linear_fwd_entry(d, x, x_t, W, bias, A_s, B_s, A_t, B_t, y_s, y_t, a_s, a_t, ctx, ctx_bytes, stream);
}

static int linear_bwd_entry(const mtlora_linear_desc* d, const void* x, const void* const* x_t, const void* Wt,
                            const void* dy_s, const void* const* dy_t, const void* ctx, int64_t ctx_bytes, void* dx,
                            void* const* dx_t, float* dA_s, float* dB_s, float* const* dA_t, float* const* dB_t,
                            void* scratch, int64_t scratch_bytes, const void* gate_s, const void* const* gate_t,
                            void* stream) {
    int st = check_desc(d);
    if (st != MTLORA_OK) return st;
    if (!x || !Wt) return MTLORA_ERR_NULL;
    if (misaligned(x) || misaligned(Wt) || misaligned(dx) || misaligned(dy_s)) return MTLORA_ERR_ALIGN;
    const Segs sg = make_segs(d);
    if (sg.R > 0) {
        if (!ctx || !scratch) return MTLORA_ERR_NULL;
        if (misaligned(ctx) || misaligned(scratch)) return MTLORA_ERR_ALIGN;
        if (ctx_bytes < ctx_layout(d, sg).total) return MTLORA_ERR_WORKSPACE;
        if (scratch_bytes < bwd_scratch(d, sg).total) return MTLORA_ERR_WORKSPACE;
    }
    if ((d->hid & MTLORA_HID_Q_GIVEN) && (d->T < 1 || !d->has_x_tasks || d->mode != 0 || misaligned(d->hid_ptr))) return MTLORA_ERR_UNSUPPORTED;
    for (int t = 0; t < d->T; ++t) {
        if (d->has_x_tasks && dA_t && dA_t[t] && (!x_t || !x_t[t])) return MTLORA_ERR_NULL;
        if (d->has_x_tasks && x_t && misaligned(x_t[t])) return MTLORA_ERR_ALIGN;
        if (dy_t && misaligned(dy_t[t])) return MTLORA_ERR_ALIGN;
        if (dx_t && misaligned(dx_t[t])) return MTLORA_ERR_ALIGN;
    }
    if (d->M == 0) return MTLORA_OK;
    hipStream_t s = (hipStream_t)stream;
    if (d->dtype == MTLORA_F32)
        st = bwd_impl<float>(d, x, x_t, Wt, dy_s, dy_t, ctx, dx, dx_t, dA_s, dB_s, dA_t, dB_t, scratch, s, gate_s, gate_t);
    else if (d->dtype == MTLORA_F16)
        st = bwd_impl<f16>(d, x, x_t, Wt, dy_s, dy_t, ctx, dx, dx_t, dA_s, dB_s, dA_t, dB_t, scratch, s, gate_s, gate_t);
    else
        st = bwd_impl<bf16>(d, x, x_t, Wt, dy_s, dy_t, ctx, dx, dx_t, dA_s, dB_s, dA_t, dB_t, scratch, s, gate_s, gate_t);
    if (st != MTLORA_OK) return st;
    MTL_CHECK_LAUNCH();
    return MTLORA_OK;
}

int mtlora_linear_bwd(const mtlora_linear_desc* d, const void* x, const void* const* x_t, const void* Wt,
                      const void* dy_s, const void* const* dy_t, const void* ctx, int64_t ctx_bytes, void* dx,
                      void* const* dx_t, float* dA_s, float* dB_s, float* const* dA_t, float* const* dB_t,
                      void* scratch, int64_t scratch_bytes, void* stream) {
    return linear_bwd_entry(d, x, x_t, Wt, dy_s, dy_t, ctx, ctx_bytes, dx, dx_t, dA_s, dB_s, dA_t, dB_t, scratch, scratch_bytes,
                            nullptr, nullptr, stream);
}

int mtlora_linear_bwd_gelu(const mtlora_linear_desc* d, const void* x, const void* const* x_t, const void* Wt,
                           const void* dy_s, const void* const* dy_t, const void* ctx, int64_t ctx_bytes, void* dx,
                           void* const* dx_t, float* dA_s, float* dB_s, float* const* dA_t, float* const* dB_t,
                           void* scratch, int64_t scratch_bytes, const void* h_s, const void* const* h_t, void* stream) {
    if (!h_s || !dx) return MTLORA_ERR_NULL;
    if (misaligned(h_s)) return MTLORA_ERR_ALIGN;
    for (int t = 0; t < d->T && d->has_x_tasks; ++t) {
        if (dx_t && dx_t[t] && (!h_t || !h_t[t])) return MTLORA_ERR_NULL;
        if (h_t && misaligned(h_t[t])) return MTLORA_ERR_ALIGN;
    }
    return linear_bwd_entry(d, x, x_t, Wt, dy_s, dy_t, ctx, ctx_bytes, dx, dx_t, dA_s, dB_s, dA_t, dB_t, scratch, scratch_bytes,
                            h_s, h_t, stream);
}

static int tn_plan(int64_t M, int Na, int Nb, int& tiles_a, int& tiles_b, int& nsplit, int64_t& rps) {
    tiles_a = (int)mtl_ceil_div(Na, TN_A);
    tiles_b = (int)mtl_ceil_div(Nb, TN_B);
    const int64_t tiles = (int64_t)tiles_a * tiles_b;
    nsplit = (int)(TN_TARGET_CTAS / (tiles > 0 ? tiles : 1));
    const int64_t max_by_rows = mtl_ceil_div(M, 256);
    if (nsplit > max_by_rows) nsplit = (int)max_by_rows;
    if (nsplit > 256) nsplit = 256;
    if (nsplit < 1) nsplit = 1;
    rps = mtl_round_up(mtl_ceil_div(M > 0 ? M : 1, nsplit), 64);
    return MTLORA_OK;
}

int64_t mtlora_gemm_tn_scratch_bytes(int64_t M, int Na, int Nb) {
    if (M < 0 || Na <= 0 || Nb <= 0) return -1;
    int ta, tb, ns;
    int64_t rps;
    tn_plan(M, Na, Nb, ta, tb, ns, rps);
    return (int64_t)ta * tb * ns * TN_TILE * 4 + 256;
}

int mtlora_gemm_tn(const void* a, const void* b, float* out, int64_t M, int Na, int Nb, int64_t lda, int64_t ldb,
                   int dtype, void* scratch, int64_t scratch_bytes, void* stream) {
    if (dtype != MTLORA_F32 && dtype != MTLORA_BF16 && dtype != MTLORA_F16) return MTLORA_ERR_DTYPE;
    const int vec = dtype == MTLORA_F32 ? 4 : 8;
// ... 53 lines not shown
```

### mtlora_amd/csrc/nt.h

```cpp
#pragma once

#include "common.h"
#include "internal.h"

namespace {

constexpr int TILE = 128;
constexpr int SUBT = 3;
constexpr int VPT = SUBT;
constexpr int ROWB = 64 * SUBT;
constexpr int LDSB = ROWB + 16;
constexpr int EPI_ROW = 64 * 2 + 8;
constexpr int EPI_BYTES = 4 * 64 * EPI_ROW;
constexpr int STAGE_BYTES = 2 * TILE * LDSB > EPI_BYTES ? 2 * TILE * LDSB : EPI_BYTES;
constexpr int MAXO = MTLORA_MAX_TASKS + 1;

struct Segs {
    int n;
    int r[MAXO], rp[MAXO], off[MAXO];
    int R;
    int used;
};
struct CtxLayout {
    int64_t a_cat, b_cat, at_cat, bt_cat, alpha, a_proj, bt_proj, b_frag, at_frag, pack_total, p, total;
// ... 87 lines not shown
                if (rr < R && n < N) {
                    const float v = tile[tx][rl];
                    bt_cat[(int64_t)rr * N + n] = mtl_from_f32<T>(v);
                    bt_proj[(int64_t)rr * N + n] = mtl_from_f32<T>(v * p.alpha[pack_seg_of(p, rr)]);
                }
            }
        }
        if constexpr (FRAG) {
            T* __restrict__ dst = isa ? at_frag : b_frag;
            const int blk0 = (isa ? col0 : row0) >> 5, t0 = (isa ? row0 : col0) >> 4, nblk32 = (isa ? K32 : N32) >> 5;
#pragma unroll
            for (int h2 = 0; h2 < 2; ++h2) {
                const int q = threadIdx.x + 256 * h2, fl = q >> 6, ln = q & 63;
                const int bl = fl >> 2, tl = fl & 3, rl = bl * 32 + (ln & 31);
                if (blk0 + bl < nblk32 && t0 + tl < R16) {
                    T tmp[8];
#pragma unroll
                    for (int sidx = 0; sidx < 8; ++sidx) {
                        const int kl = 16 * tl + 8 * (sidx >> 2) + 4 * (ln >> 5) + (sidx & 3);
                        tmp[sidx] = mtl_from_f32<T>(isa ? tile[kl][rl] : tile[rl][kl]);
                    }
                    const int64_t f = (int64_t)(blk0 + bl) * R16 + (t0 + tl);
                    *reinterpret_cast<uint4*>(dst + f * 512 + ln * 8) = *reinterpret_cast<const uint4*>(tmp);
                }
            }
        }
        __syncthreads();
    }
}

template <typename T>
__global__ __launch_bounds__(256) void k_pack(PackParams p, T* a_cat, T* b_cat, T* at_cat, T* bt_cat, float* alpha, T* a_proj,
                                              T* bt_proj, T* b_frag, T* at_frag) {
    pack_body<T>(p, a_cat, b_cat, at_cat, bt_cat, alpha, a_proj, bt_proj, b_frag, at_frag, (int)blockIdx.x, (int)gridDim.x);
}

struct PackEntry {
    PackParams pp;
    unsigned char* dst;
    int64_t off[9];
};
template <typename T>
__global__ __launch_bounds__(256) void k_pack_table(const PackEntry* __restrict__ table) {
    const PackEntry& e = table[blockIdx.y];
    unsigned char* d = e.dst;
    pack_body<T>(e.pp, reinterpret_cast<T*>(d + e.off[0]), reinterpret_cast<T*>(d + e.off[1]), reinterpret_cast<T*>(d + e.off[2]),
                 reinterpret_cast<T*>(d + e.off[3]), reinterpret_cast<float*>(d + e.off[4]), reinterpret_cast<T*>(d + e.off[5]),
                 reinterpret_cast<T*>(d + e.off[6]), reinterpret_cast<T*>(d + e.off[7]), reinterpret_cast<T*>(d + e.off[8]), (int)blockIdx.x,
                 (int)gridDim.x);
}

struct NtOut {
    void* ptr;
    int seg_lo, seg_hi;
    int use_base;
    int mask_lr;
    int fold;
    const void* gate;
    void* act;
};

struct NtParams {
    const void* act[MAXO];
    int n_act;
    int act_mask;
    int64_t ld_act;
    const void* wgt;
    int64_t ld_wgt;
    int64_t M;
    int n_rows;
    int K;
    const float* bias;
    const float* alpha;
    const void* L;
    const void* Rm;
    int64_t ldL, ldR;
    int n_out;
    NtOut out[MAXO];
    int64_t ld_out;
    int nz;
    const void* zact[MAXO];
    int zrow0[MAXO], zrows[MAXO], zmask[MAXO];
    DropoutCfg drop;
};

typedef const __attribute__((address_space(4))) NtParams* NtPtr;

template <int RI>
__device__ __forceinline__ void nt_map(int tid, int slot, int& row, int& vec) {
    constexpr int NT = 512 / RI;
    if constexpr (RI == 2) {
        row = (tid >> 2) + (slot & 1) * 64;
        vec = (tid & 3) + 4 * (slot >> 1);
    } else if (slot < 2 * RI) {
        const int idx = tid + NT * slot;
        row = idx >> 3;
        vec = idx & 7;
    } else {
        const int idx = tid + NT * (slot - 2 * RI);
        const int g = idx >> 3, l = idx & 7;
        row = (g >> 2) * 8 + (g & 3) + 4 * (l >> 2);
        vec = 8 + (l & 3);
    }
}

template <typename T, int RI>
struct TileRegs {
    u32x4 w[3 * RI], a[3 * RI];
    int mask;
    int k0;
};

template <typename T, bool MS, int RI>
__device__ __forceinline__ void nt_load(TileRegs<T, RI>& rg, int tid, const T* wgt, int64_t ld_w, int w_row0, int w_rows,
                                        const void* act0, NtPtr P, int n_act, int64_t ld_a, int64_t a_row0,
                                        int64_t a_rows, int k0, int k_hi, bool mask, int w_lo = 0) {
    constexpr int VEC = ET<T>::VEC;
    rg.mask = mask ? 1 : 0;
    rg.k0 = k0;
#pragma unroll
    for (int sl = 0; sl < 3 * RI; ++sl) {
        int r, v;
        nt_map<RI>(tid, sl, r, v);
        const int k = k0 + v * VEC;
        const bool kin = k < k_hi;
        const int wr = w_row0 + r;
        const bool wok = wr < w_rows && wr >= w_lo;
        rg.w[sl] = (kin && wok) ? *reinterpret_cast<const u32x4*>(wgt + (int64_t)wr * ld_w + k) : u32x4{0u, 0u, 0u, 0u};
        const int64_t ar = a_row0 + r;
        const bool aok = ar < a_rows && act0 != nullptr;
        const int64_t aoff = ar * ld_a;
        if (kin && aok) {
            u32x4 x = *reinterpret_cast<const u32x4*>(reinterpret_cast<const T*>(act0) + aoff + k);
            if (MS && n_act > 1) {
                if constexpr (sizeof(T) == 4) {
                    f32x4 fx = __builtin_bit_cast(f32x4, x);
#pragma unroll
                    for (int s = 1; s < MAXO; ++s) {
                        if (s < n_act) fx += *reinterpret_cast<const f32x4*>(reinterpret_cast<const T*>(P->act[s]) + aoff + k);
                    }
                    x = __builtin_bit_cast(u32x4, fx);
                } else {
                    float f[8];
                    VOps<T>::unpack(x, f);
#pragma unroll
                    for (int s = 1; s < MAXO; ++s) {
                        if (s < n_act) {
                            const u32x4 y = *reinterpret_cast<const u32x4*>(reinterpret_cast<const T*>(P->act[s]) + aoff + k);
                            float g[8];
                            VOps<T>::unpack(y, g);
#pragma unroll
                            for (int e = 0; e < 8; ++e) f[e] += g[e];
                        }
                    }
                    x = VOps<T>::pack(f);
                }
            }
            rg.a[sl] = x;
        } else {
            rg.a[sl] = u32x4{0u, 0u, 0u, 0u};
        }
    }
}

template <typename T, int RI>
__device__ __forceinline__ void nt_store_lds(TileRegs<T, RI>& rg, int tid, unsigned char* sW, unsigned char* sA,
// ... 57 lines not shown
    O.use_base = P->out[o].use_base;
    O.mask_lr = P->out[o].mask_lr;
    O.fold = P->out[o].fold;
    O.gate = P->out[o].gate;
    O.act = P->out[o].act;
    return O;
}

template <bool MULTI>
__device__ __forceinline__ void nt_part(NtPtr P, int q, int& lr, int& k_lo, int& k_hi) {
    if (MULTI) {
        if (q == 0) {
            lr = 0;
            k_lo = 0;
            k_hi = P->K;
        } else {
            const NtOut O = nt_out(P, q - 1);
            lr = 1;
            k_lo = O.seg_lo;
            k_hi = O.seg_hi;
        }
    } else {
        const NtOut O = nt_out(P, q >> 1);
        if (q & 1) {
            lr = 0;
            k_lo = 0;
            k_hi = O.use_base ? P->K : 0;
        } else {
            lr = 1;
            k_lo = O.seg_lo;
            k_hi = O.seg_hi;
        }
    }
}

template <bool MULTI>
__device__ __forceinline__ NtCursor nt_seek(NtPtr P, int q, int nseq, int bn) {
    NtCursor c;
    c.valid = 0;
    c.q = q;
    c.k0 = c.k_hi = c.lr = 0;
    c.bn = bn;
    for (; q < nseq; ++q) {
        int lr, lo, hi;
        nt_part<MULTI>(P, q, lr, lo, hi);
        if (hi > lo) {
            c.q = q;
            c.k0 = lo;
            c.k_hi = hi;
            c.lr = lr;
            c.valid = 1;
            return c;
        }
    }
    return c;
}

__device__ __forceinline__ float gelu_grad(float h) {
    const float z = fabsf(h) * 0.70710678118654752f;
    const float t = __builtin_amdgcn_rcpf(1.f + 0.3275911f * z);
    const float e = __expf(-z * z);
    float p = 1.061405429f;
    p = p * t - 1.453152027f;
    p = p * t + 1.421413741f;
    p = p * t - 0.284496736f;
    p = p * t + 0.254829592f;
    const float erf_abs = 1.f - p * t * e;
    const float cdf = 0.5f + 0.5f * copysignf(erf_abs, h);
    return cdf + h * e * 0.39894228040143268f;
}

__device__ __forceinline__ float gelu_fwd(float h) {
    const float z = fabsf(h) * 0.70710678118654752f;
    const float t = __builtin_amdgcn_rcpf(1.f + 0.3275911f * z);
    float p = 1.061405429f;
    p = p * t - 1.453152027f;
    p = p * t + 1.421413741f;
    p = p * t - 0.284496736f;
    p = p * t + 0.254829592f;
    const float erf_abs = 1.f - p * t * __expf(-z * z);
    return h * (0.5f + 0.5f * copysignf(erf_abs, h));
}

template <typename T, bool MULTI, bool MS, bool MLR, int NW, bool GATE = false, bool ACT = false>
__global__ __launch_bounds__(64 * NW, NW == 4 ? 2 : 4) void k_nt(const NtParams Pv) {
    constexpr int SM = 8 / NW;
    constexpr int MW = 32 * SM;
    constexpr int NT = 64 * NW;
    (void)Pv;
    NtPtr P = (NtPtr)__builtin_amdgcn_kernarg_segment_ptr();
    constexpr int KE = ROWB / (int)sizeof(T);
    extern __shared__ __attribute__((aligned(16))) unsigned char smem[];
    unsigned char* sW = smem;
    unsigned char* sA = smem + TILE * LDSB;
    const int tid = threadIdx.x, lane = tid & 63, wave = tid >> 6;
    const int wn = NW == 4 ? wave >> 1 : wave >> 2, wm = NW == 4 ? wave & 1 : wave & 3;

    const void* act0 = P->act[0];
    int row_off = 0, n_rows = P->n_rows;
    bool act_mask = P->act_mask != 0;
    if (P->nz > 0) {
        const int z = blockIdx.z;
        act0 = P->zact[z];
        row_off = P->zrow0[z];
        n_rows = P->zrows[z];
        act_mask = P->zmask[z] != 0;
    }
    if (n_rows <= 0) return;
    act_mask = act_mask && P->drop.thr16 != 0;

    const int n_tiles = (n_rows + TILE - 1) / TILE;
    const int64_t m_tiles = (P->M + TILE - 1) / TILE;
    const int64_t nwg = m_tiles * n_tiles;
    int64_t b = blockIdx.x;
    if (b >= nwg) return;
    {
        const int64_t q = nwg / 8, r = nwg % 8, xcd = b % 8;
        b = (xcd < r ? xcd * (q + 1) : r * (q + 1) + (xcd - r) * q) + b / 8;
    }
    const int64_t bm = b / n_tiles;
    const int bn0 = (int)(b % n_tiles);
    const int64_t m0 = bm * TILE;
    const int n0 = bn0 * TILE;

    const T* wgt = reinterpret_cast<const T*>(P->wgt) + (int64_t)row_off * P->ld_wgt;
    DropoutCfg drop;
    drop.seed_lo = P->drop.seed_lo;
    drop.seed_hi = P->drop.seed_hi;
    drop.thr16 = P->drop.thr16;
    drop.off = P->drop.off;
    mtl_dropout_resolve(drop);
    const int nseq = MULTI ? 1 + P->n_out : 2 * P->n_out;

    TileRegs<T, SM> rg;
    NtCursor ld = nt_seek<MULTI>(P, 0, nseq, bn0);
    auto issue = [&](const NtCursor& c) __attribute__((always_inline)) {
        if (c.lr)
            nt_load<T, false, SM>(rg, tid, reinterpret_cast<const T*>(P->Rm), P->ldR, c.bn * TILE, n_rows, P->L, P, 1, P->ldL, m0, P->M, c.k0,
                                  c.k_hi, false);
        else
            nt_load<T, MS, SM>(rg, tid, wgt, P->ld_wgt, c.bn * TILE, n_rows, act0, P, P->n_act, P->ld_act, m0, P->M, c.k0, c.k_hi, act_mask);
    };
    if (ld.valid) issue(ld);
    auto step = [&](f32x16(&acc)[2][SM], int k_left) __attribute__((always_inline)) {
        nt_store_lds<T, SM>(rg, tid, sW, sA, drop, m0);
        __syncthreads();
        ld.k0 += KE;
        if (ld.k0 >= ld.k_hi) ld = nt_seek<MULTI>(P, ld.q + 1, nseq, bn0);
        if (ld.valid) issue(ld);
        if (n0 + wn * 64 < n_rows) nt_compute<T, SM>(acc, sW, sA, lane, wn, wm, k_left);
        __syncthreads();
    };
    auto run_part = [&](int q, f32x16(&acc)[2][SM]) __attribute__((always_inline)) {
        int lr, lo, hi;
        nt_part<MULTI>(P, q, lr, lo, hi);
        for (int k0 = lo; k0 < hi; k0 += KE) step(acc, hi - k0);
        return hi > lo;
    };
    auto zero = [](f32x16(&a)[2][SM]) __attribute__((always_inline)) {
#pragma unroll
        for (int i = 0; i < 2; ++i)
#pragma unroll
            for (int j = 0; j < SM; ++j)
#pragma unroll
                for (int r = 0; r < 16; ++r) a[i][j][r] = 0.f;
    };
    auto affine = [&](f32x16(&a)[2][SM]) __attribute__((always_inline)) {
        if (!(P->alpha || P->bias)) return;
#pragma unroll
        for (int sn = 0; sn < 2; ++sn)
#pragma unroll
            for (int q = 0; q < 4; ++q) {
                const int n = n0 + wn * 64 + sn * 32 + 8 * q + 4 * (lane >> 5);
                if (n < n_rows) {
                    f32x4 al = {1.f, 1.f, 1.f, 1.f}, bi = {0.f, 0.f, 0.f, 0.f};
                    if (P->alpha) al = *reinterpret_cast<const f32x4*>(P->alpha + row_off + n);
                    if (P->bias) bi = *reinterpret_cast<const f32x4*>(P->bias + row_off + n);
#pragma unroll
                    for (int sm = 0; sm < SM; ++sm)
#pragma unroll
                        for (int e = 0; e < 4; ++e) a[sn][sm][q * 4 + e] = a[sn][sm][q * 4 + e] * al[e] + bi[e];
                }
            }
    };
    auto apply_mask = [&](f32x16(&a)[2][SM]) __attribute__((always_inline)) {
#pragma unroll
        for (int sm = 0; sm < SM; ++sm) {
            const int64_t m = m0 + wm * MW + sm * 32 + (lane & 31);
            const uint32_t rh = mtl_dropout_rowhash(drop, 0u, (uint32_t)m);
#pragma unroll
            for (int sn = 0; sn < 2; ++sn)
#pragma unroll
                for (int q = 0; q < 4; ++q) {
                    const int n = n0 + wn * 64 + sn * 32 + 8 * q + 4 * (lane >> 5);
                    const uint32_t h0 = mtl_dropout_pairbits(drop, rh, (uint32_t)n);
                    const uint32_t h1 = mtl_dropout_pairbits(drop, rh, (uint32_t)(n + 2));
                    if ((h0 & 0xFFFFu) < drop.thr16) a[sn][sm][q * 4 + 0] = 0.f;
                    if ((h0 >> 16) < drop.thr16) a[sn][sm][q * 4 + 1] = 0.f;
                    if ((h1 & 0xFFFFu) < drop.thr16) a[sn][sm][q * 4 + 2] = 0.f;
                    if ((h1 >> 16) < drop.thr16) a[sn][sm][q * 4 + 3] = 0.f;
                }
        }
    };
    auto store = [&](const f32x16(&a)[2][SM], void* ptr, const void* gate_ptr, void* act_ptr) __attribute__((always_inline)) {
        T* outp = reinterpret_cast<T*>(ptr);
        const T* gate = reinterpret_cast<const T*>(gate_ptr);
        T* actp = reinterpret_cast<T*>(act_ptr);
        (void)gate;
        (void)actp;
        if (!outp || n0 + wn * 64 >= n_rows) return;
        if constexpr (sizeof(T) == 2) {
            constexpr int ORS = EPI_ROW;
            unsigned char* img = smem + wave * (MW * ORS);
#pragma unroll
            for (int sm = 0; sm < SM; ++sm)
#pragma unroll
                for (int sn = 0; sn < 2; ++sn)
#pragma unroll
                    for (int q = 0; q < 4; ++q) {
                        const int ml = sm * 32 + (lane & 31), nl = sn * 32 + 8 * q + 4 * (lane >> 5);
                        u32x2 pk = {mtl_pack2<T>(a[sn][sm][q * 4], a[sn][sm][q * 4 + 1]),
                                    mtl_pack2<T>(a[sn][sm][q * 4 + 2], a[sn][sm][q * 4 + 3])};
                        *reinterpret_cast<u32x2*>(img + ml * ORS + nl * 2) = pk;
                    }
            __builtin_amdgcn_s_waitcnt(0xc07f);
            __builtin_amdgcn_wave_barrier();
#pragma unroll
            for (int it = 0; it < 4 * SM; ++it) {
                const int ml = it * 8 + (lane >> 3), c16 = lane & 7;
                const int64_t m = m0 + wm * MW + ml;
                const int n = n0 + wn * 64 + c16 * 8;
                u32x4 v = *reinterpret_cast<const u32x4*>(img + ml * ORS + c16 * 16);
                if (m < P->M && n < n_rows) {
                    if constexpr (GATE) {
                        if (gate) {
                            const u32x4 hv = __builtin_nontemporal_load(reinterpret_cast<const u32x4*>(gate + m * P->ld_out + row_off + n));
                            v = mtl_gelu_gate_pk4<T, false>(v, hv);
                        }
                    }
                    __builtin_nontemporal_store(v, reinterpret_cast<u32x4*>(outp + m * P->ld_out + row_off + n));
                    if constexpr (ACT) {
                        if (actp) {
                            const u32x4 av = mtl_gelu_pk4<T, false>(v);
                            __builtin_nontemporal_store(av, reinterpret_cast<u32x4*>(actp + m * P->ld_out + row_off + n));
                        }
                    }
                }
            }
            __builtin_amdgcn_wave_barrier();
        } else {
#pragma unroll
            for (int sm = 0; sm < SM; ++sm) {
                const int64_t m = m0 + wm * MW + sm * 32 + (lane & 31);
#pragma unroll
                for (int sn = 0; sn < 2; ++sn)
#pragma unroll
                    for (int q = 0; q < 4; ++q) {
                        const int n = n0 + wn * 64 + sn * 32 + 8 * q + 4 * (lane >> 5);
                        if (m < P->M && n < n_rows) {
                            T* dst = outp + m * P->ld_out + row_off + n;
                            f32x4 o4 = {a[sn][sm][q * 4], a[sn][sm][q * 4 + 1], a[sn][sm][q * 4 + 2], a[sn][sm][q * 4 + 3]};
                            if constexpr (GATE) {
                                if (gate) {
                                    const f32x4 hv = *reinterpret_cast<const f32x4*>(gate + m * P->ld_out + row_off + n);
#pragma unroll
                                    for (int e = 0; e < 4; ++e) o4[e] *= gelu_grad(hv[e]);
                                }
                            }
                            *reinterpret_cast<f32x4*>(dst) = o4;
                            if constexpr (ACT) {
                                if (actp) {
                                    f32x4 a4;
#pragma unroll
                                    for (int e = 0; e < 4; ++e) a4[e] = gelu_fwd(o4[e]);
                                    *reinterpret_cast<f32x4*>(actp + m * P->ld_out + row_off + n) = a4;
                                }
                            }
                        }
                    }
            }
        }
    };

    if constexpr (MULTI) {
        f32x16 base[2][SM], acc[2][SM];
        zero(base);
        run_part(0, base);
        affine(base);
        for (int o = 0; o < P->n_out; ++o) {
            const NtOut O = nt_out(P, o);
#pragma unroll
            for (int i = 0; i < 2; ++i)
#pragma unroll
                for (int j = 0; j < SM; ++j) acc[i][j] = base[i][j];
            run_part(1 + o, acc);
            if (O.fold) {
#pragma unroll
                for (int i = 0; i < 2; ++i)
#pragma unroll
                    for (int j = 0; j < SM; ++j) base[i][j] = acc[i][j];
            }
            store(acc, O.ptr, O.gate, O.act);
            __syncthreads();
        }
    } else {
        f32x16 acc[2][SM];
        for (int o = 0; o < P->n_out; ++o) {
            const NtOut O = nt_out(P, o);
            zero(acc);
            const bool had_lr = run_part(2 * o, acc);
            if constexpr (MLR) {
                if (had_lr && O.mask_lr && drop.enabled()) apply_mask(acc);
            } else {
                (void)had_lr;
            }
            run_part(2 * o + 1, acc);
            if (O.use_base) affine(acc);
            store(acc, O.ptr, O.gate, O.act);
            __syncthreads();
        }
    }
}

__device__ __attribute__((aligned(16))) const uint32_t g_zero16[4] = {0u, 0u, 0u, 0u};

struct NlParams {
    const bf16* act;
    const bf16* wgt;
    const bf16* L;
    const bf16* Rm;
    bf16* out;
    bf16* act2;
    const bf16* gate;
    const float* bias;
    const float* alpha;
    int64_t ld_act, ld_wgt, ldL, ldR, ld_out;
    int M, n_rows, K, seg_lo, seg_hi;
    int n_tiles;
    uint32_t nt_magic;
    uint32_t q8, r8;
    int act_mask, use_base;
    DropoutCfg drop;
};

template <bool ACT, bool MLR, int SN>
__global__ __launch_bounds__(512, 4) void k_ntl(const NlParams P) {
    constexpr int KE = ROWB / 2;
    constexpr int TN = 64 * SN;
    extern __shared__ __attribute__((aligned(16))) unsigned char smem[];
    unsigned char* sW = smem;
    unsigned char* sA = smem + TN * LDSB;
    const int tid = threadIdx.x, lane = tid & 63, wave = tid >> 6;
    const int wn = wave >> 2, wm = wave & 3;

    uint32_t b = blockIdx.x;
    {
        const uint32_t xcd = b & 7u, q = P.q8, r = P.r8;
        b = (xcd < r ? xcd * (q + 1u) : r * (q + 1u) + (xcd - r) * q) + (b >> 3);
    }
    const uint32_t bm = P.n_tiles == 1 ? b : __umulhi(b, P.nt_magic);
    const int bn = (int)(b - bm * (uint32_t)P.n_tiles);
    const int m0 = (int)bm * TILE, n0 = bn * TN;
    const int M = P.M, n_rows = P.n_rows;

    DropoutCfg drop = P.drop;
    mtl_dropout_resolve(drop);
    const bool act_mask = P.act_mask != 0 && drop.thr16 != 0;

    const int n1 = P.seg_hi > P.seg_lo ? (P.seg_hi - P.seg_lo + KE - 1) / KE : 0;
    const int n2 = (P.use_base && P.K > 0) ? (P.K + KE - 1) / KE : 0;
    const int total = n1 + n2;

    f32x16 acc[SN];
    const bool bias_first = !MLR && P.bias != nullptr && P.alpha == nullptr && P.use_base != 0;
#pragma unroll
    for (int sn = 0; sn < SN; ++sn)
#pragma unroll
        for (int q = 0; q < 4; ++q) {
            f32x4 bi = {0.f, 0.f, 0.f, 0.f};
            if (bias_first) {
                int n = n0 + wn * (32 * SN) + sn * 32 + 8 * q + 4 * (lane >> 5);
                n = n < n_rows - 4 ? n : n_rows - 4;
                bi = *reinterpret_cast<const f32x4*>(P.bias + n);
            }
#pragma unroll
            for (int e = 0; e < 4; ++e) acc[sn][q * 4 + e] = bi[e];
        }

    u32x4 rw[3], rw2[SN == 3 ? 3 : 1], ra[3];
    (void)rw2;
    int cur_mask = 0, cur_k0 = 0;
    auto issue = [&](int i) __attribute__((always_inline)) {
        const bool lr = i < n1;
        const bf16* wp = lr ? P.Rm : P.wgt;
        const bf16* ap = lr ? P.L : P.act;
        const int64_t ldw = lr ? P.ldR : P.ld_wgt, lda = lr ? P.ldL : P.ld_act;
        const int k0 = lr ? P.seg_lo + i * KE : (i - n1) * KE;
        const int khi = lr ? P.seg_hi : P.K;
        cur_mask = (!lr && act_mask) ? 1 : 0;
        cur_k0 = k0;
        const bf16* zp = reinterpret_cast<const bf16*>(g_zero16);
#pragma unroll
        for (int sl = 0; sl < 3; ++sl) {
            int r, v;
            nt_map<1>(tid, sl, r, v);
            const int k = k0 + v * 8;
            const bool kin = k < khi;
            int wr = n0 + r, ar = m0 + r;
            wr = wr < n_rows ? wr : n_rows - 1;
            ar = ar < M ? ar : M - 1;
            rw[sl] = *reinterpret_cast<const u32x4*>(kin ? wp + (int64_t)wr * ldw + k : zp);
            ra[sl] = *reinterpret_cast<const u32x4*>(kin ? ap + (int64_t)ar * lda + k : zp);
            if constexpr (SN == 3) {
                int wr2 = n0 + 128 + r;
                wr2 = wr2 < n_rows ? wr2 : n_rows - 1;
                if (r < 64) rw2[sl] = *reinterpret_cast<const u32x4*>(kin ? wp + (int64_t)wr2 * ldw + k : zp);
            }
        }
    };
    auto stage = [&]() __attribute__((always_inline)) {
#pragma unroll
        for (int sl = 0; sl < 3; ++sl) {
            int r, v;
            nt_map<1>(tid, sl, r, v);
            if (cur_mask) {
                const uint32_t rh = mtl_dropout_rowhash(drop, 0u, (uint32_t)(m0 + r));
                VOps<bf16>::drop(ra[sl], drop, rh, (uint32_t)(cur_k0 + v * 8));
            }
            *reinterpret_cast<u32x4*>(sW + r * LDSB + v * 16) = rw[sl];
            *reinterpret_cast<u32x4*>(sA + r * LDSB + v * 16) = ra[sl];
            if constexpr (SN == 3) {
                if (r < 64) *reinterpret_cast<u32x4*>(sW + (128 + r) * LDSB + v * 16) = rw2[sl];
            }
        }
    };
    auto compute = [&](int k_left) __attribute__((always_inline)) {
        const int h = lane >> 5, rl = lane & 31;
#pragma unroll
        for (int t = 0; t < SUBT; ++t) {
            if (t * 32 >= k_left) break;
            Frag<bf16> fw[SN], fa;
#pragma unroll
            for (int sn = 0; sn < SN; ++sn) {
                const unsigned char* pw = sW + (wn * (32 * SN) + sn * 32 + rl) * LDSB + t * 64;
                fw[sn].v[0] = *reinterpret_cast<const u32x4*>(pw + h * 16);
                fw[sn].v[1] = *reinterpret_cast<const u32x4*>(pw + (2 + h) * 16);
            }
            const unsigned char* pa = sA + (wm * 32 + rl) * LDSB + t * 64;
            fa.v[0] = *reinterpret_cast<const u32x4*>(pa + h * 16);
            fa.v[1] = *reinterpret_cast<const u32x4*>(pa + (2 + h) * 16);
#pragma unroll
            for (int sn = 0; sn < SN; ++sn) mtl_mma(fw[sn], fa, acc[sn]);
        }
    };
    const bool wave_live = n0 + wn * (32 * SN) < n_rows;
    if (total > 0) issue(0);
    for (int i = 0; i < total; ++i) {
        const bool lr = i < n1;
        const int k_left = lr ? P.seg_hi - (P.seg_lo + i * KE) : P.K - (i - n1) * KE;
        stage();
        __syncthreads();
        if (i + 1 < total) issue(i + 1);
        if (wave_live) compute(k_left);
        if constexpr (MLR) {
            if (i + 1 == n1 && wave_live && drop.thr16 != 0) {
                const uint32_t rh = mtl_dropout_rowhash(drop, 0u, (uint32_t)(m0 + wm * 32 + (lane & 31)));
#pragma unroll
                for (int sn = 0; sn < SN; ++sn)
#pragma unroll
                    for (int q = 0; q < 4; ++q) {
                        const int n = n0 + wn * (32 * SN) + sn * 32 + 8 * q + 4 * (lane >> 5);
                        const uint32_t h0 = mtl_dropout_pairbits(drop, rh, (uint32_t)n);
                        const uint32_t h1 = mtl_dropout_pairbits(drop, rh, (uint32_t)(n + 2));
                        if ((h0 & 0xFFFFu) < drop.thr16) acc[sn][q * 4 + 0] = 0.f;
                        if ((h0 >> 16) < drop.thr16) acc[sn][q * 4 + 1] = 0.f;
                        if ((h1 & 0xFFFFu) < drop.thr16) acc[sn][q * 4 + 2] = 0.f;
                        if ((h1 >> 16) < drop.thr16) acc[sn][q * 4 + 3] = 0.f;
                    }
            }
        }
        __syncthreads();
    }
    if (!wave_live) return;

    if (!bias_first && (P.alpha || P.bias) && P.use_base) {
#pragma unroll
        for (int sn = 0; sn < SN; ++sn)
#pragma unroll
            for (int q = 0; q < 4; ++q) {
                int n = n0 + wn * (32 * SN) + sn * 32 + 8 * q + 4 * (lane >> 5);
                n = n < n_rows - 4 ? n : n_rows - 4;
                f32x4 al = {1.f, 1.f, 1.f, 1.f}, bi = {0.f, 0.f, 0.f, 0.f};
                if (P.alpha) al = *reinterpret_cast<const f32x4*>(P.alpha + n);
                if (P.bias) bi = *reinterpret_cast<const f32x4*>(P.bias + n);
#pragma unroll
                for (int e = 0; e < 4; ++e) acc[sn][q * 4 + e] = acc[sn][q * 4 + e] * al[e] + bi[e];
            }
    }

    {
        constexpr int ORS = 64 * SN + 8;
        constexpr int CPRW = 4 * SN;
        unsigned char* img = smem + wave * (32 * ORS);
#pragma unroll
        for (int sn = 0; sn < SN; ++sn)
#pragma unroll
            for (int q = 0; q < 4; ++q) {
                const int ml = lane & 31, nl = sn * 32 + 8 * q + 4 * (lane >> 5);
                u32x2 pk = {mtl_pack_bf16(acc[sn][q * 4], acc[sn][q * 4 + 1]), mtl_pack_bf16(acc[sn][q * 4 + 2], acc[sn][q * 4 + 3])};
                *reinterpret_cast<u32x2*>(img + ml * ORS + nl * 2) = pk;
            }
        __builtin_amdgcn_s_waitcnt(0xc07f);
        __builtin_amdgcn_wave_barrier();
#pragma unroll
        for (int it = 0; it < 2 * SN; ++it) {
            const int idx = it * 64 + lane;
            const int ml = idx / CPRW, c16 = idx - ml * CPRW;
            const int m = m0 + wm * 32 + ml;
            const int n = n0 + wn * (32 * SN) + c16 * 8;
            u32x4 v = *reinterpret_cast<const u32x4*>(img + ml * ORS + c16 * 16);
            if (m < M && n < n_rows) {
                const int64_t o = (int64_t)m * P.ld_out + n;
                __builtin_nontemporal_store(v, reinterpret_cast<u32x4*>(P.out + o));
                if constexpr (ACT) {
                    if (P.act2) {
                        const u32x4 av = mtl_gelu_pk4<bf16, false>(v);
                        __builtin_nontemporal_store(av, reinterpret_cast<u32x4*>(P.act2 + o));
                    }
                }
            }
        }
    }
}

}
```

### mtlora_amd/functional.py

```python
from __future__ import annotations

import ctypes
import os
from dataclasses import dataclass, field
from typing import List, Optional, Sequence, Tuple

import torch

from . import _lib as L

_seed_counter = 0


_seed_offset: Optional[torch.Tensor] = None


def set_seed_offset(t: Optional[torch.Tensor]) -> None:
    global _seed_offset
    if t is not None and not (t.is_cuda and t.dtype == torch.int64 and t.numel() == 1):
        raise RuntimeError("mtlora_amd: the seed offset must be a CUDA int64 tensor with one element")
    _seed_offset = t


_factor_stream: Optional["torch.cuda.Stream"] = None
# ... 1020 lines not shown
        C, M = 4 * Ct, B * Lt // 4
        r2 = [x.contiguous() for x in res]
        b2 = [x.contiguous() for x in brs]
        w, b = _ln_affine(weight, bias)
        xs = [torch.empty_like(x) for x in r2]
        y = torch.empty((n, M, C), dtype=out_dtype, device=r2[0].device)
        stats, means, rstds = _ln_stream_stats(n, M, r2[0].device)
        st = L.lib().mtlora_residual_layernorm_streams_fwd(n, L.ptr_array9(r2), L.ptr_array9(b2), L.ptr(scale), B, L.ptr(w), L.ptr(b),
                                                           L.ptr_array9(xs), L.ptr_array9([y[k] for k in range(n)]),
                                                           L.ptr_array9(means), L.ptr_array9(rstds), M, C, float(eps),
                                                           L.dtype_code(r2[0]), L.dtype_code(y), H, W, L.stream_ptr())
        L.check(st, "mtlora_residual_layernorm_streams_fwd")
        ctx.save_for_backward(w, stats, scale, *xs)
        ctx.cfg = (n, M, C, H, W, B, res[0].shape, brs[0].dtype)
        return y.view(n * B, Lt // 4, C)

    @staticmethod
    def backward(ctx, g):
        w, stats, scale, *xs = ctx.saved_tensors
        n, M, C, H, W, B, shape, bdt = ctx.cfg
        g3 = g.reshape(n, M, C)
        if g3.dtype != bdt:
            g3 = g3.to(bdt)
        g3 = g3.contiguous()
        dev = xs[0].device
        scratch, sb, dg, db = _ln_bwd_buffers(M, C, xs[0], n)
        dres = [torch.empty_like(x) for x in xs]
        dbr = [torch.empty(shape, dtype=bdt, device=dev) for _ in range(n)]
        _, means, rstds = _ln_stream_stats(n, M, stats=stats)
        st = L.lib().mtlora_residual_layernorm_streams_bwd(n, L.ptr_array9([g3[k] for k in range(n)]), L.ptr_array9(xs), L.ptr(w),
                                                       L.ptr_array9(means), L.ptr_array9(rstds), L.ptr_array9(dres),
                                                       L.ptr_array9(dbr), L.ptr(dg), L.ptr(db), L.ptr(scale), B, M, C,
                                                       L.dtype_code(xs[0]), L.dtype_code(g3), L.ptr(scratch), sb, L.ptr_array9(None),
                                                       H, W, L.stream_ptr())
        L.check(st, "mtlora_residual_layernorm_streams_bwd")
        return (None, dg, db, None, None, None, None, None, *[d.view(shape) for d in dres], *dbr)


def residual_merge_norm_streams(mod: torch.nn.Module, res, branches, H: int, W: int, drop_prob: float, training: bool):
    n = len(res)
    B, Lt, C = res[0].shape
    ok = (_ln_module_ok(mod) and 2 <= n <= L.MAX_TASKS + 1
          and len(branches) == n and all(x.is_cuda and x.dtype == res[0].dtype and x.shape == res[0].shape for x in res)
          and all(x.shape == res[0].shape and x.dtype == branches[0].dtype for x in branches)
          and _ln_width_ok(res[0], multiple=_ln_vec(res[0]), width=4 * C) and Lt == H * W and H % 2 == 0 and W % 2 == 0
          and torch.is_grad_enabled())
    if ok:
        out_dtype = glue_dtype(res[0])
        ok = branches[0].dtype == out_dtype
    if not ok:
        return None
    scale = None
    if training and drop_prob > 0.0:
        keep = 1.0 - drop_prob
        scale = droppath_scale(n, B, keep, res[0].device)
    return ResidualMergeNormStreamsFn.apply(scale, mod.weight, mod.bias, mod.eps, out_dtype, H, W, n, *res, *branches)


def layer_norm_merge_multi(mod: torch.nn.Module, xs, H: int, W: int):
    B, Lt, C = xs[0].shape
    ok = (_ln_module_ok(mod) and 2 <= len(xs) <= L.MAX_TASKS + 1
          and all(x.is_cuda and x.dtype == xs[0].dtype and x.shape == xs[0].shape for x in xs)
          and _ln_width_ok(xs[0], multiple=_ln_vec(xs[0]), width=4 * C) and Lt == H * W and H % 2 == 0 and W % 2 == 0)
    if not ok:
        return None
    return LayerNormMergeMultiFn.apply(mod.weight, mod.bias, mod.eps, glue_dtype(xs[0]), H, W, len(xs), *xs)


def layer_norm(mod: torch.nn.Module, x: torch.Tensor, feeds_linear: bool = True, _fork: bool = False):
    ok = _ln_module_ok(mod, last_dim_only=True) and _ln_width_ok(x, multiple=8, width=x.shape[-1])
    if not ok:
        return mod(x)
    if feeds_linear:
        out_dtype = glue_dtype(x)
    else:
        out_dtype = torch.float32 if torch.is_autocast_enabled() else x.dtype
    if _fork and x.requires_grad:
        return LayerNormForkFn.apply(x, mod.weight, mod.bias, mod.eps, out_dtype)
    return LayerNormFn.apply(x, mod.weight, mod.bias, mod.eps, out_dtype)


class BatchNormReluFn(torch.autograd.Function):
    @staticmethod
    def forward(ctx, x, weight, bias, running_mean, running_var, momentum: float, eps: float, relu: bool):
        L.require_gpu(x, weight, bias)
        R, C = x.shape
        x = x.contiguous()
        w, b = weight.detach().float().contiguous(), bias.detach().float().contiguous()
        y = torch.empty_like(x)
        saves = torch.empty(4, C, dtype=torch.float32, device=x.device)
        lib = L.lib()
        sb = lib.mtlora_bn_scratch_bytes(R, C, L.dtype_code(x))
        if sb < 0:
            raise RuntimeError(f"mtlora_amd: unsupported BatchNorm shape ({R}, {C}) {x.dtype}")
        scratch = torch.empty(sb, dtype=torch.uint8, device=x.device)
        st = lib.mtlora_bn_relu_fwd(L.ptr(x), L.ptr(w), L.ptr(b), L.ptr(running_mean), L.ptr(running_var), float(momentum),
                                    float(eps), int(relu), L.ptr(y), L.ptr(saves[0]), L.ptr(saves[1]), L.ptr(saves[2]),
                                    L.ptr(saves[3]), R, C, L.dtype_code(x), L.ptr(scratch), sb, L.stream_ptr())
        L.check(st, "mtlora_bn_relu_fwd")
        ctx.save_for_backward(x, saves)
        ctx.relu = relu
        return y

    @staticmethod
    def backward(ctx, dy):
        x, saves = ctx.saved_tensors
        R, C = x.shape
        dy = dy.to(x.dtype).contiguous()
        lib = L.lib()
        sb = lib.mtlora_bn_scratch_bytes(R, C, L.dtype_code(x))
        scratch = torch.empty(sb, dtype=torch.uint8, device=x.device)
        dx = torch.empty_like(x)
        dg = torch.empty(C, dtype=torch.float32, device=x.device)
        db = torch.empty(C, dtype=torch.float32, device=x.device)
        st = lib.mtlora_bn_relu_bwd(L.ptr(dy), L.ptr(x), L.ptr(saves[0]), L.ptr(saves[1]), L.ptr(saves[2]), L.ptr(saves[3]),
                                    int(ctx.relu), L.ptr(dx), L.ptr(dg), L.ptr(db), R, C, L.dtype_code(x), L.ptr(scratch), sb,
                                    L.stream_ptr())
        L.check(st, "mtlora_bn_relu_bwd")
        return dx, dg, db, None, None, None, None, None


class ResidualDropPathFn(torch.autograd.Function):

    @staticmethod
    def forward(ctx, scale, shared: bool, n: int, *tensors):
        nres = 1 if shared else n
        res, ys = list(tensors[:nres]), list(tensors[nres:nres + n])
        L.require_gpu(*res, *ys)
        B = res[0].shape[0]
        C = res[0].shape[-1]
        M = res[0].numel() // C
        res_c = [r.contiguous() for r in res]
        ys_c = [y.contiguous() for y in ys]
        outs = [torch.empty_like(res_c[0]) for _ in range(n)]
        rlist = res_c * n if shared else res_c
        st = L.lib().mtlora_residual_droppath_fwd(n, L.ptr_array9(rlist), L.ptr_array9(ys_c), L.ptr_array9(outs), L.ptr(scale),
                                                  M, C, B, L.dtype_code(res_c[0]), L.dtype_code(ys_c[0]), L.stream_ptr())
        L.check(st, "mtlora_residual_droppath_fwd")
        ctx.cfg = (shared, n, M, C, B, res_c[0].dtype, ys_c[0].dtype, res_c[0].shape)
        ctx.save_for_backward(scale)
        ctx.set_materialize_grads(False)
        return tuple(outs)

    @staticmethod
    def backward(ctx, *grads):
        shared, n, M, C, B, rdt, ydt, shape = ctx.cfg
        (scale,) = ctx.saved_tensors
        if all(g is None for g in grads):
            return (None,) * (3 + (1 if shared else n) + n)
        dev = next(g for g in grads if g is not None).device
        gs = [None if g is None else g.to(rdt).contiguous() for g in grads]
        dys = [None if g is None else torch.empty(shape, dtype=ydt, device=dev) for g in gs]
        dres = torch.empty(shape, dtype=rdt, device=dev) if shared else None
        st = L.lib().mtlora_residual_droppath_bwd(n, L.ptr_array9(gs), L.ptr_array9(dys), L.ptr(dres), L.ptr(scale), M, C, B,
                                                  L.dtype_code(gs[[g is not None for g in gs].index(True)]),
                                                  _DT_CODE.get(ydt, L.F32), L.stream_ptr())
        L.check(st, "mtlora_residual_droppath_bwd")
        dres_out = [dres] if shared else gs
        return (None, None, None, *dres_out, *dys)


def residual_droppath(res, ys, drop_prob: float, training: bool):
    shared = not isinstance(res, (list, tuple))
    rl = [res] if shared else list(res)
    n = len(ys)
    ok = (rl[0].is_cuda and rl[0].shape[-1] % 8 == 0 and all(t.dtype in _GLUE_DTYPES for t in rl + list(ys))
          and len({t.dtype for t in rl}) == 1 and len({t.dtype for t in ys}) == 1 and n <= L.MAX_TASKS + 1
          and all(t.shape == rl[0].shape for t in list(ys) + rl))
    scale = None
    if training and drop_prob > 0.0:
        keep = 1.0 - drop_prob
        scale = droppath_scale(n, rl[0].shape[0], keep, rl[0].device)
    if not ok:
        out = []
        for k in range(n):
            y = ys[k] if scale is None else ys[k] * scale[k].view(-1, *([1] * (ys[k].ndim - 1))).to(ys[k].dtype)
            out.append((rl[0] if shared else rl[k]) + y)
        return out
    return list(ResidualDropPathFn.apply(scale, shared, n, *rl, *ys))


def column_sum(g2: torch.Tensor) -> torch.Tensor:
    M, N = g2.shape
    ve = 4 if g2.dtype == torch.float32 else 8
    if g2.dtype not in (torch.float32, torch.bfloat16) or N % ve or not g2.is_contiguous() or M == 0:
        return g2.sum(0, dtype=torch.float32)
    lib = L.lib()
    sb = lib.mtlora_colsum_scratch_bytes(M, N)
    scratch = torch.empty(sb, dtype=torch.uint8, device=g2.device)
    out = torch.empty(N, dtype=torch.float32, device=g2.device)
    L.check(lib.mtlora_colsum(L.ptr(g2), M, N, L.dtype_code(g2), L.ptr(out), L.ptr(scratch), sb, L.stream_ptr()), "mtlora_colsum")
    return out


def label_stat(lab: torch.Tensor, kind: int, ignore_index: float) -> torch.Tensor:
    n = lab.numel()
    lib = L.lib()
    sb = lib.mtlora_label_stat_scratch_bytes(n)
    scratch = torch.empty(sb, dtype=torch.uint8, device=lab.device)
    out = torch.empty(1, dtype=torch.float32, device=lab.device)
    L.check(lib.mtlora_label_stat(L.ptr(lab), n, kind, float(ignore_index), L.ptr(out), L.ptr(scratch), sb, L.stream_ptr()),
            "mtlora_label_stat")
# ... 200 lines not shown
    for i, (kind, src) in enumerate(jobs):
        if kind not in AUGMENT_KINDS:
            raise RuntimeError(f"mtlora_amd: unknown augment kind {kind!r}")
        dt, C = _AUGMENT_FORM[kind]
        want = (B, Hc, Wc, 3) if C == 3 else (B, Hc, Wc)
        if src.dtype != dt or tuple(src.shape) != want or not src.is_contiguous():
            raise RuntimeError(f"mtlora_amd: augment job {i} ({kind}) must be a contiguous {dt} tensor of shape {want}, got "
                               f"{src.dtype} {tuple(src.shape)}")
        out = torch.empty((B, Ho, Wo, 3) if C == 3 else (B, Ho, Wo), dtype=dt, device=src.device)
        outs.append(out)
        arr[i].src, arr[i].dst, arr[i].kind = src.data_ptr(), out.data_ptr(), AUGMENT_KINDS[kind]
        arr[i].flags = 0 if renormalize else L.AUGMENT_FLAG_NO_RENORM
    st = L.lib().mtlora_augment_batch(arr, len(jobs), B, Hc, Wc, Ho, Wo, L.ptr(size), L.ptr(coef), L.ptr(side), L.ptr(cubic_q15),
                                      L.ptr(cubic_f32), L.stream_ptr())
    L.check(st, "mtlora_augment_batch")
    return outs


def _layout_weight(weight, bias, cdtype, col_index, n_cols, pad_rows):
    w = weight.detach().to(cdtype)
    if col_index is not None:
        w = w.new_zeros(w.shape[0], n_cols).index_copy(1, col_index, w)
    b = None if bias is None else bias.detach()
    if pad_rows:
        w = torch.cat([w, w.new_zeros(pad_rows, w.shape[1])], 0)
        b = None if b is None else torch.cat([b, b.new_zeros(pad_rows)], 0)
    return w.contiguous(), b


def _unlayout_grads(dw, db, col_index, pad_rows):
    if pad_rows:
        dw = None if dw is None else dw[:dw.shape[0] - pad_rows]
        db = None if db is None else db[:db.shape[0] - pad_rows].contiguous()
    if col_index is not None and dw is not None:
        dw = dw.index_select(1, col_index)
    elif dw is not None and pad_rows:
        dw = dw.contiguous()
    return dw, db


class SplitKLinearFn(torch.autograd.Function):

    @staticmethod
    def forward(ctx, x, weight, bias, splits: int, zero_bias_grad: bool, cdtype, col_index=None, n_cols=0, pad_rows=0):
        w, bl = _layout_weight(weight, bias, cdtype, col_index, n_cols, pad_rows)
        ctx.save_for_backward(x, w)
        ctx.wlayout = (col_index, pad_rows)
        ctx.has_bias = bias is not None
        ctx.splits = splits
        ctx.zero_bias_grad = zero_bias_grad
        ctx.wdtype = weight.dtype
        ctx.bdtype = None if bias is None else bias.dtype
        return torch.nn.functional.linear(x, w, None if bl is None else bl.to(cdtype))

    @staticmethod
    def backward(ctx, gy):
        x, w = ctx.saved_tensors
        gy = gy.contiguous()
        M, K = x.shape
        N = w.shape[0]
        S = ctx.splits
        dx = gy @ w if ctx.needs_input_grad[0] else None

        def wgrads():
            dw = None
            if ctx.needs_input_grad[1]:
                part = torch.bmm(gy.view(S, M // S, N).transpose(1, 2), x.view(S, M // S, K))
                dw = part.sum(0, dtype=torch.float32).to(ctx.wdtype)
            db = None
            if ctx.has_bias and ctx.needs_input_grad[2]:
                if ctx.zero_bias_grad:
                    db = torch.zeros(N, dtype=ctx.bdtype, device=gy.device)
                else:
                    db = column_sum(gy).to(ctx.bdtype)
            return _unlayout_grads(dw, db, *ctx.wlayout)

        dw, db = wgrads()
        return dx, dw, db, None, None, None, None, None, None


class PlainLinearFn(torch.autograd.Function):

    @staticmethod
    def forward(ctx, x, weight, bias, splits: int, zero_bias_grad: bool, cdtype, col_index=None, n_cols=0, pad_rows=0):
        L.require_gpu(x, weight)
        M, K = x.shape
        w, bias_l = _layout_weight(weight, bias, cdtype, col_index, n_cols, pad_rows)
        N = w.shape[0]
        meta = LinearMeta(K=K, N=N, r_s=0, r_t=(), scale_s=0.0, scale_t=(), mode=0, has_x_tasks=False, dropout_p=0.0, seed=0,
                          dtype=cdtype)
        d = meta.desc(M)
        lib = L.lib()
        ctx_bytes = _desc_bytes("ctx", lib.mtlora_linear_ctx_bytes, meta, M, d)
        if ctx_bytes < 0:
            raise RuntimeError(f"mtlora_amd: invalid plain-linear shape M={M} K={K} N={N}")
        ctxbuf = torch.empty(max(ctx_bytes, 16), dtype=torch.uint8, device=x.device)
        y = torch.empty((M, N), dtype=cdtype, device=x.device)
        bf = None if bias_l is None else bias_l.float().contiguous()
        st = lib.mtlora_linear_fwd(ctypes.byref(d), L.ptr(x), L.ptr_array(None), L.ptr(w), L.ptr(bf), L.ptr(None), L.ptr(None),
                                   L.ptr_array(None), L.ptr_array(None), L.ptr(y), L.ptr_array(None), L.ptr(ctxbuf), ctx_bytes,
                                   L.stream_ptr())
        L.check(st, "mtlora_linear_fwd (rank 0)")
        ctx.save_for_backward(x, w, ctxbuf)
        ctx.wlayout = (col_index, pad_rows)
        ctx.meta, ctx.splits, ctx.zero_bias_grad = meta, splits, zero_bias_grad
        ctx.has_bias, ctx.wdtype = bias is not None, weight.dtype
        ctx.bdtype = None if bias is None else bias.dtype
        return y

    @staticmethod
    def backward(ctx, gy):
        x, w, ctxbuf = ctx.saved_tensors
        gy = gy.contiguous()
        M, K = x.shape
        N = w.shape[0]
        S = ctx.splits
        dx = None
        if ctx.needs_input_grad[0]:
            d = ctx.meta.desc(M)
            lib = L.lib()
            sb = _desc_bytes("bwd", lib.mtlora_linear_bwd_scratch_bytes, ctx.meta, M, d)
            scratch = torch.empty(max(sb, 16), dtype=torch.uint8, device=x.device)
            wt = w.t().contiguous()
            dx = torch.empty((M, K), dtype=x.dtype, device=x.device)
            st = lib.mtlora_linear_bwd(ctypes.byref(d), L.ptr(x), L.ptr_array(None), L.ptr(wt), L.ptr(gy), L.ptr_array(None),
                                       L.ptr(ctxbuf), ctxbuf.numel(), L.ptr(dx), L.ptr_array(None), L.ptr(None), L.ptr(None),
                                       L.ptr_array(None), L.ptr_array(None), L.ptr(scratch), sb, L.stream_ptr())
            L.check(st, "mtlora_linear_bwd (rank 0)")
        def wgrads():
            dw = None
            if ctx.needs_input_grad[1]:
                if N <= 64:
                    dw = gemm_tn(gy, x).to(ctx.wdtype)
                else:
                    part = torch.bmm(gy.view(S, M // S, N).transpose(1, 2), x.view(S, M // S, K))
                    dw = part.sum(0, dtype=torch.float32).to(ctx.wdtype)
            db = None
            if ctx.has_bias and ctx.needs_input_grad[2]:
                if ctx.zero_bias_grad:
                    db = torch.zeros(N, dtype=ctx.bdtype, device=gy.device)
                else:
                    db = column_sum(gy).to(ctx.bdtype)
            return _unlayout_grads(dw, db, *ctx.wlayout)

        dw, db = wgrads()
        return dx, dw, db, None, None, None, None, None, None


def gemm_tn(a: torch.Tensor, b: torch.Tensor) -> torch.Tensor:
    L.require_gpu(a, b)
    if a.dtype != b.dtype or a.dim() != 2 or b.dim() != 2 or a.shape[0] != b.shape[0]:
        raise ValueError("gemm_tn: (M, Na) and (M, Nb) matrices of one dtype expected")
    a, b = a.contiguous(), b.contiguous()
    M, Na = a.shape
    Nb = b.shape[1]
    lib = L.lib()
    sb = lib.mtlora_gemm_tn_scratch_bytes(M, Na, Nb)
    if sb < 0:
        raise RuntimeError(f"mtlora_amd: invalid gemm_tn shape M={M} Na={Na} Nb={Nb}")
    scratch = torch.empty(sb, dtype=torch.uint8, device=a.device)
    out = torch.empty((Na, Nb), dtype=torch.float32, device=a.device)
    st = lib.mtlora_gemm_tn(L.ptr(a), L.ptr(b), L.ptr(out), M, Na, Nb, Na, Nb, _DT_CODE[a.dtype],
                            L.ptr(scratch), sb, L.stream_ptr())
    L.check(st, "mtlora_gemm_tn")
    return out


_PLAIN_VIA_KNT = os.environ.get("MTLORA_HEAD_GEMM", "knt") != "blas"


def _big_linear(x, weight, bias, S, feeds_batchnorm, cdtype, col_index=None, pad_rows=0):
    K, N = x.shape[1], weight.shape[0] + pad_rows
    if (_PLAIN_VIA_KNT and cdtype in _HOT_DTYPES and K % 8 == 0 and N % 8 == 0
            and x.dtype == cdtype):
        return PlainLinearFn.apply(x, weight, bias, S, feeds_batchnorm, cdtype, col_index, K, pad_rows)
    return SplitKLinearFn.apply(x, weight, bias, S, feeds_batchnorm, cdtype, col_index, K, pad_rows)


def linear_big_m(x: torch.Tensor, weight: torch.Tensor, bias: Optional[torch.Tensor],
                 feeds_batchnorm: bool = False, col_index: Optional[torch.Tensor] = None, pad_rows: int = 0) -> torch.Tensor:
    M = x.shape[0]
    if x.dim() == 2 and x.is_cuda and weight.requires_grad and torch.is_grad_enabled() and M >= 1 and x.is_contiguous():
        S = 1
        if M >= 16384:
            tiles = ((weight.shape[0] + 63) // 64) * ((weight.shape[1] + 63) // 64)
            S = 4
            while S < 64 and S * tiles < 2048 and M % (2 * S) == 0 and M // (2 * S) >= 1024:
                S *= 2
            if M % S:
                S = 1
        if torch.is_autocast_enabled("cuda"):
            dt = torch.get_autocast_dtype("cuda")
            with torch.autocast("cuda", enabled=False):
                return _big_linear(x.to(dt), weight, bias, S, feeds_batchnorm, dt, col_index, pad_rows)
        return _big_linear(x, weight, bias, S, feeds_batchnorm, x.dtype, col_index, pad_rows)
    if col_index is not None:
        weight = weight.new_zeros(weight.shape[0], x.shape[1]).index_copy(1, col_index, weight)
    if pad_rows:
        weight = torch.cat([weight, weight.new_zeros(pad_rows, weight.shape[1])], 0)
        bias = None if bias is None else torch.cat([bias, bias.new_zeros(pad_rows)], 0)
    return torch.nn.functional.linear(x, weight, bias)


def _pad4(c: int) -> int:
    return (c + 3) // 4 * 4


class ConcatUpsampleFn(torch.autograd.Function):

    @staticmethod
    def layout(channels):
        offs, o = [], 0
        for c in channels:
            offs.append(o)
            o += _pad4(c)
        return offs, (o + 7) // 8 * 8

    @staticmethod
    def forward(ctx, *maps):
        L.require_gpu(*maps)
        B, H, W, _ = maps[0].shape
        chans = [m.shape[3] for m in maps]
        offs, ld = ConcatUpsampleFn.layout(chans)
        dt = maps[0].dtype
        out = torch.empty(B * H * W, ld, dtype=dt, device=maps[0].device)
        o3 = out.view(B, H, W, ld)
        o3[..., :chans[0]].copy_(maps[0])
        lib = L.lib()
        end = chans[0]
        for i in range(1, len(maps)):
            if offs[i] > end:
                o3[..., end:offs[i]].zero_()
            m = maps[i].contiguous()
            _, h, w, C = m.shape
            if H % h or W % w or H // h != W // w or C % 4 or m.dtype != dt:
                raise RuntimeError("mtlora_amd: ConcatUpsampleFn needs integer scales, C % 4 == 0 and one dtype")
            st = lib.mtlora_upsample_cl_fwd(L.ptr(m), ctypes.c_void_p(out.data_ptr() + offs[i] * out.element_size()), B, h, w, C,
                                            H // h, ld, L.dtype_code(m), L.stream_ptr())
            L.check(st, "mtlora_upsample_cl_fwd")
            end = offs[i] + C
        if ld > end:
            o3[..., end:].zero_()
        ctx.shapes = [tuple(m.shape) for m in maps]
        ctx.offs, ctx.ld = offs, ld
        return out

    @staticmethod
    def backward(ctx, g):
        g = g.contiguous()
        B, H, W, C0 = ctx.shapes[0]
        ld = ctx.ld
        grads = [g.view(B, H, W, ld)[..., :C0]]
        lib = L.lib()
        for i in range(1, len(ctx.shapes)):
            _, h, w, C = ctx.shapes[i]
            d = torch.empty(ctx.shapes[i], dtype=g.dtype, device=g.device)
            st = lib.mtlora_upsample_cl_bwd(ctypes.c_void_p(g.data_ptr() + ctx.offs[i] * g.element_size()), L.ptr(d), B, h, w, C,
                                            H // h, ld, L.dtype_code(g), L.stream_ptr())
            L.check(st, "mtlora_upsample_cl_bwd")
            grads.append(d)
        return tuple(grads)


class BlockCall:
    __slots__ = ("has_norm1", "metas", "weights", "mask", "mask_ids", "H", "W", "num_heads", "window_size", "shift", "hidden",
                 "eps", "attn_scale", "mask_value", "factor_params", "norm_params", "desc", "params", "n_flat")

    def __init__(self, has_norm1, metas, weights, mask, mask_ids, H, W, num_heads, window_size, shift, hidden, eps, attn_scale,
                 factor_params, norm_params=(), mask_value=-100.0):
        self.has_norm1, self.metas, self.weights, self.mask, self.mask_ids = has_norm1, metas, weights, mask, mask_ids
        self.H, self.W, self.num_heads, self.window_size, self.shift, self.hidden = H, W, num_heads, window_size, shift, hidden
        self.eps, self.attn_scale, self.mask_value, self.factor_params = eps, attn_scale, mask_value, factor_params
        self.norm_params = tuple(norm_params)
        self.desc = self.params = None
        self.n_flat = 17 if has_norm1 else 15

    def build_desc(self, B: int, C: int, cdtype: torch.dtype, x_dtype: torch.dtype) -> "L.BlockDesc":
        d = L.BlockDesc()
# ... 157 lines not shown
```

### mtlora_amd/mtl_harness.py

```python
from __future__ import annotations

import contextlib
import ctypes
import os
from typing import Dict, List, Mapping, Optional, Sequence

import torch
import torch.nn as nn
import torch.nn.functional as F

from . import functional as Fn
from .functional import BatchNormReluFn, UpsampleLossFn
from .lora import MTLoRALinear, mark_only_lora_as_trainable
from .optim import FusedAdamW, accumulation_steps_of
from .swin_transformer_mtlora import SwinTransformerMTLoRA

NUM_OUTPUT = {"semseg": 21, "normals": 3, "sal": 1, "human_parts": 7, "depth": 1, "edge": 1}
EDGE_POS_WEIGHT = 0.95
NYUD4 = ("semseg", "depth", "normals", "edge")
NYUD_NUM_OUTPUT = {"semseg": 40}
LOSS_WEIGHTS = {"depth": 1.0, "semseg": 1.0, "human_parts": 2.0, "sal": 5.0, "edge": 50.0, "normals": 10.0}


def is_synthetic_task(t: str) -> bool:
# ... 42 lines not shown
    c = config(name)
    c.update(over)
    return build_model(img_size=c["img_size"], tasks=c["tasks"], embed_dim=c["embed_dim"], depths=c["depths"],
                       num_heads=c["num_heads"], r_shared=c["r_shared"], r_task=c["r_task"], seed=seed,
                       **{k: v for k, v in c.items() if k not in ("img_size", "tasks", "embed_dim", "depths", "num_heads",
                                                                    "r_shared", "r_task", "batch", "what")})


class AttrDict(dict):
    __getattr__ = dict.__getitem__
    __setattr__ = dict.__setitem__


def mtlora_namespace(tasks: Sequence[str], r_shared=64, r_task=4, scale=4.0, dropout=0.05, shared_mode="matrix",
                     n_stages=4, **over) -> AttrDict:
    ns = AttrDict(ENABLED=True, QKV_ENABLED=True, PROJ_ENABLED=True, FC1_ENABLED=True, FC2_ENABLED=True,
                  DOWNSAMPLER_ENABLED=False, INTERMEDIATE_SPECIALIZATION=False, TRAINABLE_SCALE_SHARED=False,
                  TRAINABLE_SCALE_PER_TASK=False, SHARED_MODE=shared_mode, DROPOUT=[dropout] * n_stages,
                  SHARED_SCALE=[scale] * n_stages,
                  R_PER_TASK_LIST=[{"shared": r_shared, **{t: r_task for t in tasks}} for _ in range(n_stages)],
                  SCALE_PER_TASK_LIST=[{t: scale for t in tasks} for _ in range(n_stages)])
    ns.update(over)
    return ns


_TASK_STREAMS = os.environ.get("MTLORA_TASK_STREAMS", "1") != "0"
_GRAPH_STREAMS = os.environ.get("MTLORA_GRAPH_STREAMS", "1") != "0"


def _streams_allowed() -> bool:
    return _GRAPH_STREAMS or not torch.cuda.is_current_stream_capturing()


class Downsampler(nn.Module):

    def __init__(self, dims, channels, input_res, bias=False, enabled=True):
        super().__init__()
        self.dims, self.input_res, self.enabled = dims, input_res, enabled
        if enabled:
            for i, (d, c) in enumerate(zip(dims, channels)):
                setattr(self, f"downsample_{i}", nn.Conv2d(d, c, 1, bias=bias))

    def forward(self, feats):
        maps = []
        for i, (f, r, d) in enumerate(zip(feats, self.input_res, self.dims)):
            if self.enabled:
                conv = getattr(self, f"downsample_{i}")
                B_, L_, _ = f.shape
                f = Fn.linear_big_m(f.reshape(B_ * L_, d), conv.weight.view(conv.out_channels, d), conv.bias).view(B_, L_, -1)
            maps.append(f.view(-1, r, r, f.shape[-1]).permute(0, 3, 1, 2))
        return maps


class HighResolutionHead(nn.Module):

    def __init__(self, backbone_channels, num_outputs):
        super().__init__()
        c = sum(backbone_channels)
        self.last_layer = nn.Sequential(nn.Conv2d(c, 4 * c, 1), nn.BatchNorm2d(4 * c, momentum=0.1),
                                        nn.ReLU(inplace=False), nn.Conv2d(4 * c, num_outputs, 1))

    def forward(self, x, channels_last_out: bool = False):
        B, _, Hh, Ww = x[0].shape
        c0, bn, _, c3 = self.last_layer
        w2d = c0.weight.view(c0.out_channels, c0.in_channels)
        xc = [m.permute(0, 2, 3, 1) for m in x]
        chans = [t.shape[3] for t in xc]
        if (x[0].is_cuda and all(t.is_contiguous() for t in xc) and all(c % 4 == 0 for c in chans[1:])
                and len({t.dtype for t in xc}) == 1 and xc[0].dtype in (torch.float32, torch.bfloat16, torch.float16)
                and all(Hh % t.shape[1] == 0 and Ww % t.shape[2] == 0 and Hh // t.shape[1] == Ww // t.shape[2] for t in xc)):
            t = Fn.ConcatUpsampleFn.apply(*xc)
            offs, ld = Fn.ConcatUpsampleFn.layout(chans)
            col_idx = None
            if ld != w2d.shape[1]:
                key = (tuple(offs), tuple(chans), w2d.device)
                if getattr(self, "_col_key", None) != key:
                    self._col_idx = torch.cat([torch.arange(o, o + c) for o, c in zip(offs, chans)]).to(w2d.device)
                    self._col_key = key
                col_idx = self._col_idx
        else:
            cat = torch.cat([x[0]] + [F.interpolate(m, (Hh, Ww), mode="bilinear") for m in x[1:]], 1)
            t = cat.permute(0, 2, 3, 1).reshape(B * Hh * Ww, cat.shape[1])
            col_idx = None
        h = Fn.linear_big_m(t, w2d, c0.bias, feeds_batchnorm=bn.training, col_index=col_idx)
        if bn.training and bn.track_running_stats and bn.num_batches_tracked is not None:
            bn.num_batches_tracked.add_(1)
        if bn.training and h.is_cuda and h.dtype in (torch.float32, torch.bfloat16, torch.float16) and h.shape[1] % 8 == 0:
            h = BatchNormReluFn.apply(h, bn.weight, bn.bias, bn.running_mean, bn.running_var, bn.momentum, bn.eps,
                                      getattr(self, "relu", True))
        else:
            h = F.batch_norm(h, bn.running_mean, bn.running_var, bn.weight, bn.bias, bn.training or not bn.track_running_stats,
                             bn.momentum, bn.eps)
            if getattr(self, "relu", True):
                h = F.relu(h)
        w3, b3, nc = c3.weight.view(c3.out_channels, c3.in_channels), c3.bias, c3.out_channels
        o = Fn.linear_big_m(h, w3, b3, pad_rows=(8 - nc % 8) if (h.is_cuda and nc % 8) else 0)
        o = (o if o.shape[1] == nc else o[:, :nc].contiguous()).view(B, Hh, Ww, nc)
        return o if channels_last_out else o.permute(0, 3, 1, 2)


class DecoderGroup(nn.Module):
    def __init__(self, tasks, num_outputs, channels, out_size):
        super().__init__()
        self.tasks, self.out_size = tasks, out_size
        self.decoders = nn.ModuleDict({t: HighResolutionHead(channels, num_outputs[t]) for t in tasks})

    def forward(self, x, upsample: bool = True, tasks=None):
        tasks = self.tasks if tasks is None else tasks
        if not upsample:
            return {t: self.decoders[t](x[t], channels_last_out=True) for t in tasks}
        return {t: F.interpolate(self.decoders[t](x[t]), self.out_size, mode="bilinear") for t in tasks}


class MultiTaskSwin(nn.Module):

    def __init__(self, backbone: SwinTransformerMTLoRA, tasks: Sequence[str], num_outputs: Mapping[str, int] = NUM_OUTPUT,
                 decoder_channels=(18, 36, 72, 144)):
        super().__init__()
        self.backbone = backbone
        self.tasks = list(tasks)
        res = backbone.patch_embed.patches_resolution
        n = backbone.num_layers
        self.dims = [int(backbone.embed_dim * 2 ** ((i + 1) if i < n - 1 else i)) for i in range(n)]
        self.input_res = [res[0] // (2 ** ((i + 1) if i < n - 1 else i)) for i in range(n)]
        self.img_size = backbone.patch_embed.img_size
        self.downsampler = nn.ModuleDict({t: Downsampler(self.dims, decoder_channels, self.input_res) for t in self.tasks})
        self.decoders = DecoderGroup(self.tasks, num_outputs, decoder_channels, self.img_size)

    def task_streams(self, device):
        key = str(device)
        if getattr(self, "_streams_key", None) != key:
            self._streams = [torch.cuda.Stream(device=device) for _ in self.tasks]
            self._streams_key = key
        return self._streams

    def forward(self, x, upsample: bool = True, per_task_fn=None, concurrent: Optional[bool] = None):
        stages = self.backbone(x, return_stages=True)
        if concurrent is None:
            concurrent = (x.is_cuda and _TASK_STREAMS and len(self.tasks) > 1 and torch.is_grad_enabled()
                          and _streams_allowed())
        if not concurrent:
            feats = {t: self.downsampler[t]([tl[t] for _, tl in stages]) for t in self.tasks}
            out = self.decoders(feats, upsample=upsample)
            return out if per_task_fn is None else {t: per_task_fn(t, out[t]) for t in self.tasks}
        main = torch.cuda.current_stream(x.device)
        streams = self.task_streams(x.device)
        out = {}
        for t, st in zip(self.tasks, streams):
            ins = [tl[t] for _, tl in stages]
            st.wait_stream(main)
            with torch.cuda.stream(st):
                for f in ins:
                    f.record_stream(st)
                y = self.decoders({t: self.downsampler[t](ins)}, upsample=upsample, tasks=[t])[t]
                if per_task_fn is not None:
                    y = per_task_fn(t, y)
                y.record_stream(main)
            out[t] = y
        for st in streams:
            main.wait_stream(st)
        return out


def task_loss(task: str, out: torch.Tensor, label: torch.Tensor) -> torch.Tensor:
    out = out.float()
    task = task_kind(task)
    if task in ("semseg", "human_parts"):
        return F.nll_loss(F.log_softmax(out, 1), label[:, 0].long(), ignore_index=255)
    if task == "normals":
        mask = (label != 255).to(out.dtype)
        on = out / (torch.norm(out, p=2, dim=1, keepdim=True) + 1e-12)
        return ((on - label).abs() * mask).sum() / mask.sum().clamp_min(1e-6)
# ... 481 lines not shown
```

Before: 1160 images/sec.

## Fuse BatchNorm column statistics into decoder head linear epilogue

After: 1165 images/sec, median of 6. Within noise of the previous version (+0.5%).

```diff
diff --git a/include/mtlora_hip.h b/include/mtlora_hip.h
--- a/include/mtlora_hip.h
+++ b/include/mtlora_hip.h
@@ -188,6 +188,14 @@
 int mtlora_bn_relu_bwd(const void* dy, const void* x, const float* save_mean, const float* save_rstd,
                        const float* save_scale, const float* save_shift, int relu, void* dx, float* dgamma, float* dbeta,
                        int64_t R, int64_t C, int dtype, void* scratch, int64_t scratch_bytes, void* stream);
+
+int64_t mtlora_linear_fwd_stats_blocks(const mtlora_linear_desc* d);
+int mtlora_linear_fwd_stats(const mtlora_linear_desc* d, const void* x, const void* W, const float* bias, void* y, float* part,
+                            int64_t part_bytes, void* stream);
+int mtlora_bn_relu_fwd_from_partials(const void* x, const float* gamma, const float* beta, float* running_mean, float* running_var,
+                                     float momentum, float eps, int relu, void* y, float* save_mean, float* save_rstd,
+                                     float* save_scale, float* save_shift, int64_t R, int64_t C, int dtype, const float* part,
+                                     int64_t nblk, int64_t part_bytes, void* stream);
 
 int mtlora_residual_droppath_fwd(int n, const void* const* res, const void* const* y, void* const* out,
                                  const float* scale, int64_t M, int64_t C, int64_t B, int res_dtype, int y_dtype,
diff --git a/mtlora_amd/_lib.py b/mtlora_amd/_lib.py
--- a/mtlora_amd/_lib.py
+++ b/mtlora_amd/_lib.py
@@ -167,6 +167,11 @@
                                    c_void_p]),
     "mtlora_bn_relu_bwd": (c_int, [c_void_p, c_void_p, c_void_p, c_void_p, c_void_p, c_void_p, c_int, c_void_p, c_void_p,
                                    c_void_p, c_int64, c_int64, c_int, c_void_p, c_int64, c_void_p]),
+    "mtlora_linear_fwd_stats_blocks": (c_int64, [POINTER(LinearDesc)]),
+    "mtlora_linear_fwd_stats": (c_int, [POINTER(LinearDesc), c_void_p, c_void_p, c_void_p, c_void_p, c_void_p, c_int64, c_void_p]),
+    "mtlora_bn_relu_fwd_from_partials": (c_int, [c_void_p, c_void_p, c_void_p, c_void_p, c_void_p, c_float, c_float, c_int, c_void_p,
+                                                 c_void_p, c_void_p, c_void_p, c_void_p, c_int64, c_int64, c_int, c_void_p, c_int64,
+                                                 c_int64, c_void_p]),
     "mtlora_residual_droppath_fwd": (c_int, [c_int, POINTER(c_void_p), POINTER(c_void_p), POINTER(c_void_p), c_void_p,
                                              c_int64, c_int64, c_int64, c_int, c_int, c_void_p]),
     "mtlora_residual_droppath_bwd": (c_int, [c_int, POINTER(c_void_p), POINTER(c_void_p), c_void_p, c_void_p, c_int64,
diff --git a/mtlora_amd/csrc/dense.h b/mtlora_amd/csrc/dense.h
--- a/mtlora_amd/csrc/dense.h
+++ b/mtlora_amd/csrc/dense.h
@@ -276,8 +276,10 @@
 constexpr int NE_DPW = NE_ROWS / 16 / 4;
 constexpr int NE_ORS = 128 + 8;
 
-template <bool ACT, bool MLR, bool GATE>
+template <bool ACT, bool MLR, bool GATE, bool STATS = false>
 __global__ __launch_bounds__(256, 2) void k_nte(const NlParams P) {
+    static_assert(!STATS || (!ACT && !GATE), "column statistics: the plain output only");
+    static_assert(4 * 32 * NE_ORS + 4 * CS_WAVE_FLOATS * 4 <= NE_STAGE, "images + statistics slots fit one ring slot");
     constexpr int EPI_OPS = 16 * (1 + (ACT ? 1 : 0)) + (GATE ? 16 : 0);
     extern __shared__ __attribute__((aligned(16))) unsigned char smem[];
     const int tid = threadIdx.x, lane = tid & 63, wave = __builtin_amdgcn_readfirstlane(tid >> 6);
@@ -479,6 +481,9 @@
         unsigned char* img = smem + img_slot * NE_STAGE + wave * (32 * NE_ORS);
         const int c16 = lane & 7;
         const int n = n0c + wn * 64 + c16 * 8;
+        ColStats<bf16> cst;
+        (void)cst;
+        if constexpr (STATS) cst.zero();
 #pragma unroll
         for (int sm = 0; sm < 4; ++sm) {
             u32x4 hv[4];
@@ -511,6 +516,7 @@
                 if constexpr (GATE) {
                     v = mtl_gelu_gate_pk4<bf16, false>(v, hv[it]);
                 }
+                if constexpr (STATS) cst.add(v, m < M && n < n_rows);
                 sp_bstore(v, orsrc, off);
                 if constexpr (ACT) {
                     const u32x4 av = mtl_gelu_pk4<bf16, false>(v);
@@ -519,6 +525,12 @@
             }
             __builtin_amdgcn_wave_barrier();
         }
+        if constexpr (STATS) {
+            float* slots = reinterpret_cast<float*>(smem + img_slot * NE_STAGE + 4 * 32 * NE_ORS);
+            cst.to_lds(slots + wave * CS_WAVE_FLOATS, lane);
+            __syncthreads();
+            colstats_store<2>(slots, P.stats + (int64_t)(m0c / NE_TM) * 2 * n_rows, n0c, n_rows, tid, [](int half, int m) { return m * 2 + half; });
+        }
     }
 }
 
diff --git a/mtlora_amd/csrc/glue.hip b/mtlora_amd/csrc/glue.hip
--- a/mtlora_amd/csrc/glue.hip
+++ b/mtlora_amd/csrc/glue.hip
@@ -266,6 +266,35 @@
     BnParams p = {};
     if (bn_setup(p, R, C, dtype) != MTLORA_OK) return -1;
     return ((int64_t)p.nblk * 2 * C + 4 * C) * 4 + 256;
+}
+
+static int bn_fwd_run(const BnParams& p, int dtype, bool colsum, hipStream_t s) {
+    const int64_t R = p.R, C = p.C;
+    const int threads = (int)mtl_round_up((int64_t)p.rows_per_iter * p.VW, 64);
+    const unsigned apply_blocks = (unsigned)(mtl_ceil_div(R, 16) < BN_APPLY_BLOCKS ? mtl_ceil_div(R, 16) : BN_APPLY_BLOCKS);
+    const size_t lds = (size_t)p.rows_per_iter * 2 * C * 4;
+    const int es = mtl_elem_size(dtype);
+    if (colsum) {
+        MtlProfScope prof(PK_BN, (double)R * C * es, s);
+        if (dtype == MTLORA_F32)
+            hipLaunchKernelGGL((k_bn_colsum<float, false>), dim3(p.nblk), dim3(threads), lds, s, p);
+        else if (dtype == MTLORA_F16)
+            hipLaunchKernelGGL((k_bn_colsum<f16, false>), dim3(p.nblk), dim3(threads), lds, s, p);
+        else
+            hipLaunchKernelGGL((k_bn_colsum<bf16, false>), dim3(p.nblk), dim3(threads), lds, s, p);
+    }
+    hipLaunchKernelGGL(k_bn_finalize, dim3((unsigned)mtl_ceil_div(C, 64)), dim3(64 * BN_FW), 0, s, p);
+    {
+        MtlProfScope prof(PK_BN, (double)R * C * es * 2, s);
+        if (dtype == MTLORA_F32)
+            hipLaunchKernelGGL((k_bn_apply<float, false>), dim3(apply_blocks), dim3(threads), 0, s, p);
+        else if (dtype == MTLORA_F16)
+            hipLaunchKernelGGL((k_bn_apply<f16, false>), dim3(apply_blocks), dim3(threads), 0, s, p);
+        else
+            hipLaunchKernelGGL((k_bn_apply<bf16, false>), dim3(apply_blocks), dim3(threads), 0, s, p);
+    }
+    MTL_CHECK_LAUNCH();
+    return MTLORA_OK;
 }
 
 int mtlora_bn_relu_fwd(const void* x, const float* gamma, const float* beta, float* running_mean, float* running_var,
@@ -293,32 +322,37 @@
     p.momentum = momentum;
     p.eps = eps;
     p.relu = relu;
-    hipStream_t s = (hipStream_t)stream;
-    const int threads = (int)mtl_round_up((int64_t)p.rows_per_iter * p.VW, 64);
-    const unsigned apply_blocks = (unsigned)(mtl_ceil_div(R, 16) < BN_APPLY_BLOCKS ? mtl_ceil_div(R, 16) : BN_APPLY_BLOCKS);
-    const size_t lds = (size_t)p.rows_per_iter * 2 * C * 4;
-    const int es = mtl_elem_size(dtype);
-    {
-        MtlProfScope prof(PK_BN, (double)R * C * es, s);
-        if (dtype == MTLORA_F32)
-            hipLaunchKernelGGL((k_bn_colsum<float, false>), dim3(p.nblk), dim3(threads), lds, s, p);
-        else if (dtype == MTLORA_F16)
-            hipLaunchKernelGGL((k_bn_colsum<f16, false>), dim3(p.nblk), dim3(threads), lds, s, p);
-        else
-            hipLaunchKernelGGL((k_bn_colsum<bf16, false>), dim3(p.nblk), dim3(threads), lds, s, p);
-    }
-    hipLaunchKernelGGL(k_bn_finalize, dim3((unsigned)mtl_ceil_div(C, 64)), dim3(64 * BN_FW), 0, s, p);
-    {
-        MtlProfScope prof(PK_BN, (double)R * C * es * 2, s);
-        if (dtype == MTLORA_F32)
-            hipLaunchKernelGGL((k_bn_apply<float, false>), dim3(apply_blocks), dim3(threads), 0, s, p);
-        else if (dtype == MTLORA_F16)
-            hipLaunchKernelGGL((k_bn_apply<f16, false>), dim3(apply_blocks), dim3(threads), 0, s, p);
-        else
-            hipLaunchKernelGGL((k_bn_apply<bf16, false>), dim3(apply_blocks), dim3(threads), 0, s, p);
-    }
-    MTL_CHECK_LAUNCH();
-    return MTLORA_OK;
+    return bn_fwd_run(p, dtype, true, (hipStream_t)stream);
+}
+
+int mtlora_bn_relu_fwd_from_partials(const void* x, const float* gamma, const float* beta, float* running_mean, float* running_var,
+                                     float momentum, float eps, int relu, void* y, float* save_mean, float* save_rstd,
+                                     float* save_scale, float* save_shift, int64_t R, int64_t C, int dtype, const float* part,
+                                     int64_t nblk, int64_t part_bytes, void* stream) {
+    BnParams p = {};
+    int st = bn_setup(p, R, C, dtype);
+    if (st != MTLORA_OK) return st;
+    if (nblk <= 0 || nblk > 0x7FFFFFFF) return MTLORA_ERR_SHAPE;
+    if (!x || !gamma || !beta || !y || !save_mean || !save_rstd || !save_scale || !save_shift || !part)
+        return MTLORA_ERR_NULL;
+    if (((uintptr_t)x | (uintptr_t)y | (uintptr_t)part) & 15u) return MTLORA_ERR_ALIGN;
+    if (part_bytes < nblk * 2 * C * (int64_t)sizeof(float)) return MTLORA_ERR_WORKSPACE;
+    p.x = x;
+    p.y = y;
+    p.gamma = gamma;
+    p.beta = beta;
+    p.running_mean = running_mean;
+    p.running_var = running_var;
+    p.mean = save_mean;
+    p.rstd = save_rstd;
+    p.scale = save_scale;
+    p.shift = save_shift;
+    p.part = const_cast<float*>(part);
+    p.nblk = (int)nblk;
+    p.momentum = momentum;
+    p.eps = eps;
+    p.relu = relu;
+    return bn_fwd_run(p, dtype, false, (hipStream_t)stream);
 }
 
 int mtlora_bn_relu_bwd(const void* dy, const void* x, const float* save_mean, const float* save_rstd,
diff --git a/mtlora_amd/csrc/linear.hip b/mtlora_amd/csrc/linear.hip
--- a/mtlora_amd/csrc/linear.hip
+++ b/mtlora_amd/csrc/linear.hip
@@ -162,6 +162,7 @@
     q.act_mask = dense ? 0 : P.act_mask;
     q.use_base = P.out[0].use_base;
     q.drop = P.drop;
+    q.stats = P.stats;
     return q;
 }
 
@@ -181,6 +182,32 @@
         go(N{}, N{}, N{});
 }
 
+static bool nt_dense_plan(const Tune& tu, const NtParams& P, int variant, bool& use_e) {
+    const int ntd_mode = tu.ntd;
+    bool dense = false;
+    use_e = false;
+    int ksteps = 0;
+    if (variant == 2 && P.n_out == 1 && P.nz == 0 && ntd_mode != 0 && P.act_mask == 0 && P.n_rows % 8 == 0 && P.n_rows >= 64 &&
+        P.M < (int64_t)0x7FFFFF00 && P.out[0].ptr != nullptr && !(P.out[0].gate && P.out[0].act)) {
+        const int seg = P.L ? P.out[0].seg_hi - P.out[0].seg_lo : 0;
+        const int kk = (P.act[0] && P.out[0].use_base ? P.K : 0);
+        ksteps = (seg + ND_KE - 1) / ND_KE + (kk + ND_KE - 1) / ND_KE;
+        const int64_t tiles = mtl_ceil_div(P.M, ND_TM) * mtl_ceil_div(P.n_rows, ND_TN);
+        const int64_t lim = ((int64_t)1 << 32) - 4096;
+        const bool fits = P.M * P.ld_out * 2 < lim && P.M * P.ld_act * 2 < lim && P.M * P.ldL * 2 < lim && (int64_t)P.n_rows * P.ld_wgt * 2 < lim &&
+                          (int64_t)P.n_rows * P.ldR * 2 < lim && P.K % 8 == 0 && seg % 8 == 0 && (P.ld_act % 8) == 0 && (P.ld_wgt % 8) == 0 &&
+                          (P.ldL % 8) == 0 && (P.ldR % 8) == 0 && (P.L == nullptr || (P.out[0].seg_lo % 8) == 0);
+        const int64_t slots = num_cu(tu);
+        const double eff = (double)tiles / (double)(mtl_ceil_div(tiles, slots) * slots);
+        use_e = ntd_mode == 3 || (ntd_mode == 1 && nte_prefer(tiles, ksteps, slots) && (P.n_rows % ND_TN == 0 || P.n_rows > 2 * ND_TN));
+        dense = fits && ksteps >= 1 &&
+                (ntd_mode == 2 || ntd_mode == 3 || use_e ||
+                 (ksteps >= 6 && (eff >= 0.7 || (tiles <= slots && tiles >= slots / 2)) && (P.n_rows % ND_TN == 0 || P.n_rows > 2 * ND_TN)));
+    }
+    if (dense && P.stats) use_e = true;
+    return dense;
+}
+
 template <typename T>
 static void launch_nt(const Tune& tu, const NtParams& P, hipStream_t s, int kind, double alg_bytes, double s8d_bytes = 0.0, double flops = 0.0) {
     mtl_prof_tag("M%lld K%d N%d ldL%lld no%d na%d nz%d", (long long)P.M, P.K, P.n_rows, (long long)P.ldL, P.n_out, P.n_act, P.nz);
@@ -207,31 +234,18 @@
     }
     mlr = mlr && P.drop.enabled();
     if constexpr (std::is_same<T, bf16>::value) {
-        const int ntd_mode = tu.ntd;
-        bool dense = false, use_e = false;
-        int ksteps = 0;
-        if (variant == 2 && P.n_out == 1 && P.nz == 0 && ntd_mode != 0 && P.act_mask == 0 && P.n_rows % 8 == 0 && P.n_rows >= 64 &&
-            P.M < (int64_t)0x7FFFFF00 && P.out[0].ptr != nullptr && !(P.out[0].gate && P.out[0].act)) {
-            const int seg = P.L ? P.out[0].seg_hi - P.out[0].seg_lo : 0;
-            const int kk = (P.act[0] && P.out[0].use_base ? P.K : 0);
-            ksteps = (seg + ND_KE - 1) / ND_KE + (kk + ND_KE - 1) / ND_KE;
-            const int64_t tiles = mtl_ceil_div(P.M, ND_TM) * mtl_ceil_div(P.n_rows, ND_TN);
-            const int64_t lim = ((int64_t)1 << 32) - 4096;
-            const bool fits = P.M * P.ld_out * 2 < lim && P.M * P.ld_act * 2 < lim && P.M * P.ldL * 2 < lim && (int64_t)P.n_rows * P.ld_wgt * 2 < lim &&
-                              (int64_t)P.n_rows * P.ldR * 2 < lim && P.K % 8 == 0 && seg % 8 == 0 && (P.ld_act % 8) == 0 && (P.ld_wgt % 8) == 0 &&
-                              (P.ldL % 8) == 0 && (P.ldR % 8) == 0 && (P.L == nullptr || (P.out[0].seg_lo % 8) == 0);
-            const int64_t slots = num_cu(tu);
-            const double eff = (double)tiles / (double)(mtl_ceil_div(tiles, slots) * slots);
-            use_e = ntd_mode == 3 || (ntd_mode == 1 && nte_prefer(tiles, ksteps, slots) && (P.n_rows % ND_TN == 0 || P.n_rows > 2 * ND_TN));
-            dense = fits && ksteps >= 1 &&
-                    (ntd_mode == 2 || ntd_mode == 3 || use_e ||
-                     (ksteps >= 6 && (eff >= 0.7 || (tiles <= slots && tiles >= slots / 2)) && (P.n_rows % ND_TN == 0 || P.n_rows > 2 * ND_TN)));
-        }
+        bool use_e = false;
+        const bool dense = nt_dense_plan(tu, P, variant, use_e);
         if (dense) {
             const int64_t mt = mtl_ceil_div(P.M, ND_TM), nt = mtl_ceil_div(P.n_rows, ND_TN);
             const NlParams q = make_nl(P, mt, nt, true);
             const bool ml0 = P.out[0].mask_lr != 0 && P.drop.enabled() && q.seg_hi > q.seg_lo;
             const uint32_t nwg = (uint32_t)(mt * nt), cus = (uint32_t)num_cu(tu);
+            if (q.stats) {
+                MTL_RAISE_LDS((k_nte<false, false, false, true>), SP_LDS_MAX);
+                hipLaunchKernelGGL((k_nte<false, false, false, true>), dim3(nwg < 2u * cus ? nwg : 2u * cus), dim3(256), (size_t)NE_LDS, s, q);
+                return;
+            }
             nl_dispatch(q, ml0, [&](auto ac, auto ml, auto ga) {
                 constexpr bool AC = decltype(ac)::value, ML = decltype(ml)::value, GA = decltype(ga)::value;
                 if (use_e) {
@@ -250,7 +264,7 @@
             const int64_t t128 = m_tiles * mtl_ceil_div(P.n_rows, 128), t192 = m_tiles * mtl_ceil_div(P.n_rows, 192);
             const int64_t slots = 2 * (int64_t)dev_num_cu();
             const double c128 = (double)mtl_ceil_div(t128, slots), c192 = 1.5 * (double)mtl_ceil_div(t192, slots);
-            const bool wide = !P.out[0].act && P.n_rows >= 192 && c192 < c128 - 0.01;
+            const bool wide = !P.out[0].act && !P.stats && P.n_rows >= 192 && c192 < c128 - 0.01;
             const int64_t nt = wide ? mtl_ceil_div(P.n_rows, 192) : n_tiles;
             const NlParams q = make_nl(P, m_tiles, nt, false);
             const bool ml0 = P.out[0].mask_lr != 0 && P.drop.enabled() && q.seg_hi > q.seg_lo;
@@ -261,7 +275,9 @@
         if ((LDSV) > 64 * 1024) MTL_RAISE_LDS((k_ntl<AC, ML, SNV>), 160 * 1024 - 512);        \
         hipLaunchKernelGGL((k_ntl<AC, ML, SNV>), dim3(nwg), dim3(512), (size_t)(LDSV), s, q); \
     } while (0)
-            if (q.act2)
+            if (q.stats)
+                hipLaunchKernelGGL((k_ntl<false, false, 2, true>), dim3(nwg), dim3(512), (size_t)STAGE_BYTES, s, q);
+            else if (q.act2)
                 MTL_NTL_GO(true, false, 2, STAGE_BYTES);
             else if (wide && ml0)
                 MTL_NTL_GO(false, true, 3, LDS192);
@@ -282,7 +298,9 @@
         else                                                                                            \
             hipLaunchKernelGGL((k_nt<T, MU, MSRC, ML, 4, GA, AC>), g, dim3(256), lds, s, P);            \
     } while (0)
-    if (acted) {
+    if (P.stats) {
+        if constexpr (W8) hipLaunchKernelGGL((k_nt<T, false, false, false, 8, false, false, true>), g, dim3(512), lds, s, P);
+    } else if (acted) {
         if (variant == 0)
             MTL_NT_GO(true, false, false, false, true);
         else
@@ -963,7 +981,7 @@
 static int fwd_impl(const mtlora_linear_desc* d, const void* x, const void* const* x_t, const void* W,
                     const float* bias, const float* A_s, const float* B_s, const float* const* A_t,
                     const float* const* B_t, void* y_s, void* const* y_t, void* ctx, hipStream_t s, void* a_s = nullptr,
-                    void* const* a_t = nullptr) {
+                    void* const* a_t = nullptr, float* stats = nullptr) {
     const Segs sg = make_segs(d);
     const Tune tu = make_tune(d);
     const CtxLayout L = ctx_layout(d, sg);
@@ -1019,6 +1037,7 @@
     m.ldR = sg.R;
     m.ld_out = d->N;
     m.drop = dc;
+    m.stats = stats;
     m.n_out = 1 + d->T;
     for (int o = 0; o < sg.n; ++o) {
         NtOut& O = m.out[o];
@@ -1975,6 +1994,51 @@
     return linear_fwd_entry(d, x, x_t, W, bias, A_s, B_s, A_t, B_t, y_s, y_t, a_s, a_t, ctx, ctx_bytes, stream);
 }
 
+static int64_t fwd_stats_blocks(const mtlora_linear_desc* d) {
+    if (check_desc(d) != MTLORA_OK || d->dtype == MTLORA_F32 || d->r_s != 0 || d->T != 0 || d->hid != 0 || d->dropout_p != 0.f || d->M <= 0) return 0;
+    if (d->dtype == MTLORA_BF16) {
+        NtParams m = {};
+        m.act[0] = m.wgt = d;
+        m.out[0].ptr = const_cast<mtlora_linear_desc*>(d);
+        m.n_act = m.n_out = 1;
+        m.ld_act = m.ld_wgt = d->K;
+        m.M = d->M;
+        m.n_rows = (int)d->N;
+        m.K = (int)d->K;
+        m.ld_out = d->N;
+        m.out[0].use_base = 1;
+        m.stats = reinterpret_cast<float*>(const_cast<mtlora_linear_desc*>(d));
+        bool use_e = false;
+        if (nt_dense_plan(make_tune(d), m, 2, use_e)) return mtl_ceil_div(d->M, NE_TM);
+    }
+    return mtl_ceil_div(d->M, TILE);
+}
+
+int64_t mtlora_linear_fwd_stats_blocks(const mtlora_linear_desc* d) {
+    const int64_t n = fwd_stats_blocks(d);
+    return n > 0 ? n : -1;
+}
+
+int mtlora_linear_fwd_stats(const mtlora_linear_desc* d, const void* x, const void* W, const float* bias, void* y, float* part,
+                            int64_t part_bytes, void* stream) {
+    int st = check_desc(d);
+    if (st != MTLORA_OK) return st;
+    if (d->dtype == MTLORA_F32) return MTLORA_ERR_DTYPE;
+    if (d->r_s != 0 || d->T != 0 || d->hid != 0 || d->dropout_p != 0.f) return MTLORA_ERR_UNSUPPORTED;
+    if (!x || !W || !y || !part) return MTLORA_ERR_NULL;
+    if (misaligned(x) || misaligned(W) || misaligned(y) || misaligned(bias) || misaligned(part)) return MTLORA_ERR_ALIGN;
+    if (d->M == 0) return MTLORA_OK;
+    if (part_bytes < fwd_stats_blocks(d) * 2 * d->N * (int64_t)sizeof(float)) return MTLORA_ERR_WORKSPACE;
+    hipStream_t s = (hipStream_t)stream;
+    if (d->dtype == MTLORA_F16)
+        st = fwd_impl<f16>(d, x, nullptr, W, bias, nullptr, nullptr, nullptr, nullptr, y, nullptr, nullptr, s, nullptr, nullptr, part);
+    else
+        st = fwd_impl<bf16>(d, x, nullptr, W, bias, nullptr, nullptr, nullptr, nullptr, y, nullptr, nullptr, s, nullptr, nullptr, part);
+    if (st != MTLORA_OK) return st;
+    MTL_CHECK_LAUNCH();
+    return MTLORA_OK;
+}
+
 static int linear_bwd_entry(const mtlora_linear_desc* d, const void* x, const void* const* x_t, const void* Wt,
                             const void* dy_s, const void* const* dy_t, const void* ctx, int64_t ctx_bytes, void* dx,
                             void* const* dx_t, float* dA_s, float* dB_s, float* const* dA_t, float* const* dB_t,
diff --git a/mtlora_amd/csrc/nt.h b/mtlora_amd/csrc/nt.h
--- a/mtlora_amd/csrc/nt.h
+++ b/mtlora_amd/csrc/nt.h
@@ -193,6 +193,7 @@
     const void* zact[MAXO];
     int zrow0[MAXO], zrows[MAXO], zmask[MAXO];
     DropoutCfg drop;
+    float* stats;
 };
 
 typedef const __attribute__((address_space(4))) NtParams* NtPtr;
@@ -416,8 +417,57 @@
     return h * (0.5f + 0.5f * copysignf(erf_abs, h));
 }
 
-template <typename T, bool MULTI, bool MS, bool MLR, int NW, bool GATE = false, bool ACT = false>
+constexpr int CS_WAVE_FLOATS = 2 * 64;
+
+template <typename T>
+struct ColStats {
+    float s[8], q[8];
+    __device__ __forceinline__ void zero() {
+#pragma unroll
+        for (int e = 0; e < 8; ++e) s[e] = q[e] = 0.f;
+    }
+    __device__ __forceinline__ void add(const u32x4& v, bool valid) {
+        float f[8];
+        VOps<T>::unpack(v, f);
+#pragma unroll
+        for (int e = 0; e < 8; ++e) {
+            const float x = valid ? f[e] : 0.f;
+            s[e] += x;
+            q[e] += x * x;
+        }
+    }
+    __device__ __forceinline__ void to_lds(float* slot, int lane) {
+#pragma unroll
+        for (int off = 8; off < 64; off <<= 1)
+#pragma unroll
+            for (int e = 0; e < 8; ++e) {
+                s[e] += __shfl_xor(s[e], off, 64);
+                q[e] += __shfl_xor(q[e], off, 64);
+            }
+        if (lane < 8) {
+#pragma unroll
+            for (int e = 0; e < 8; ++e) {
+                slot[lane * 8 + e] = s[e];
+                slot[64 + lane * 8 + e] = q[e];
+            }
+        }
+    }
+};
+
+template <int NWM, typename F>
+__device__ __forceinline__ void colstats_store(const float* slots, float* part, int n0, int n_rows, int tid, F wave_of) {
+    if (tid < 256) {
+        const int stat = tid >> 7, col = tid & 127;
+        float t = 0.f;
+#pragma unroll
+        for (int wm = 0; wm < NWM; ++wm) t += slots[wave_of(col >> 6, wm) * CS_WAVE_FLOATS + stat * 64 + (col & 63)];
+        if (n0 + col < n_rows) part[(int64_t)stat * n_rows + n0 + col] = t;
+    }
+}
+
+template <typename T, bool MULTI, bool MS, bool MLR, int NW, bool GATE = false, bool ACT = false, bool STATS = false>
 __global__ __launch_bounds__(64 * NW, NW == 4 ? 2 : 4) void k_nt(const NtParams Pv) {
+    static_assert(!STATS || (sizeof(T) == 2 && NW == 8 && !MULTI && !GATE && !ACT), "column statistics: the lean 16-bit 8-wave variant");
     constexpr int SM = 8 / NW;
     constexpr int MW = 32 * SM;
     constexpr int NT = 64 * NW;
@@ -536,6 +586,8 @@
                 }
         }
     };
+    ColStats<T> cst;
+    (void)cst;
     auto store = [&](const f32x16(&a)[2][SM], void* ptr, const void* gate_ptr, void* act_ptr) __attribute__((always_inline)) {
         T* outp = reinterpret_cast<T*>(ptr);
         const T* gate = reinterpret_cast<const T*>(gate_ptr);
@@ -581,6 +633,18 @@
                     }
                 }
             }
+            if constexpr (STATS) {
+                float cs = 0.f, cq = 0.f;
+#pragma unroll 8
+                for (int ml = 0; ml < MW; ++ml) {
+                    const float f = mtl_lo2<T>((uint32_t) * reinterpret_cast<const uint16_t*>(img + ml * ORS + lane * 2));
+                    const float x = (m0 + wm * MW + ml < P->M) ? f : 0.f;
+                    cs += x;
+                    cq += x * x;
+                }
+                cst.s[0] = cs;
+                cst.q[0] = cq;
+            }
             __builtin_amdgcn_wave_barrier();
         } else {
 #pragma unroll
@@ -650,7 +714,15 @@
             }
             run_part(2 * o + 1, acc);
             if (O.use_base) affine(acc);
+            if constexpr (STATS) cst.zero();
             store(acc, O.ptr, O.gate, O.act);
+            if constexpr (STATS) {
+                float* slots = reinterpret_cast<float*>(smem + EPI_BYTES);
+                slots[wave * CS_WAVE_FLOATS + lane] = cst.s[0];
+                slots[wave * CS_WAVE_FLOATS + 64 + lane] = cst.q[0];
+                __syncthreads();
+                colstats_store<4>(slots, P->stats + bm * 2 * (int64_t)n_rows, n0, n_rows, tid, [](int half, int m) { return half * 4 + m; });
+            }
             __syncthreads();
         }
     }
@@ -675,10 +747,12 @@
     uint32_t q8, r8;
     int act_mask, use_base;
     DropoutCfg drop;
+    float* stats;
 };
 
-template <bool ACT, bool MLR, int SN>
+template <bool ACT, bool MLR, int SN, bool STATS = false>
 __global__ __launch_bounds__(512, 4) void k_ntl(const NlParams P) {
+    static_assert(!STATS || (SN == 2 && !ACT), "column statistics: the 128-column tile without a second output");
     constexpr int KE = ROWB / 2;
     constexpr int TN = 64 * SN;
     extern __shared__ __attribute__((aligned(16))) unsigned char smem[];
@@ -815,7 +889,9 @@
         }
         __syncthreads();
     }
-    if (!wave_live) return;
+    if constexpr (!STATS) {
+        if (!wave_live) return;
+    }
 
     if (!bias_first && (P.alpha || P.bias) && P.use_base) {
 #pragma unroll
@@ -836,6 +912,9 @@
         constexpr int ORS = 64 * SN + 8;
         constexpr int CPRW = 4 * SN;
         unsigned char* img = smem + wave * (32 * ORS);
+        ColStats<bf16> cst;
+        (void)cst;
+        if constexpr (STATS) cst.zero();
 #pragma unroll
         for (int sn = 0; sn < SN; ++sn)
 #pragma unroll
@@ -853,6 +932,7 @@
             const int m = m0 + wm * 32 + ml;
             const int n = n0 + wn * (32 * SN) + c16 * 8;
             u32x4 v = *reinterpret_cast<const u32x4*>(img + ml * ORS + c16 * 16);
+            if constexpr (STATS) cst.add(v, m < M && n < n_rows);
             if (m < M && n < n_rows) {
                 const int64_t o = (int64_t)m * P.ld_out + n;
                 __builtin_nontemporal_store(v, reinterpret_cast<u32x4*>(P.out + o));
@@ -864,7 +944,13 @@
                 }
             }
         }
-    }
-}
-
-}
+        if constexpr (STATS) {
+            float* slots = reinterpret_cast<float*>(smem + EPI_BYTES);
+            cst.to_lds(slots + wave * CS_WAVE_FLOATS, lane);
+            __syncthreads();
+            colstats_store<4>(slots, P.stats + (int64_t)bm * 2 * n_rows, n0, n_rows, tid, [](int half, int m) { return half * 4 + m; });
+        }
+    }
+}
+
+}
diff --git a/mtlora_amd/functional.py b/mtlora_amd/functional.py
--- a/mtlora_amd/functional.py
+++ b/mtlora_amd/functional.py
@@ -1126,9 +1126,12 @@
 
 class BatchNormReluFn(torch.autograd.Function):
     @staticmethod
-    def forward(ctx, x, weight, bias, running_mean, running_var, momentum: float, eps: float, relu: bool):
-        L.require_gpu(x, weight, bias)
+    def forward(ctx, x, weight, bias, running_mean, running_var, momentum: float, eps: float, relu: bool, part=None):
+        L.require_gpu(x, weight, bias, part)
         R, C = x.shape
+        if part is not None and not (x.is_contiguous() and part.is_contiguous() and part.dtype == torch.float32
+                                     and part.dim() == 3 and tuple(part.shape[1:]) == (2, C)):
+            part = None
         x = x.contiguous()
         w, b = weight.detach().float().contiguous(), bias.detach().float().contiguous()
         y = torch.empty_like(x)
@@ -1137,11 +1140,18 @@
         sb = lib.mtlora_bn_scratch_bytes(R, C, L.dtype_code(x))
         if sb < 0:
             raise RuntimeError(f"mtlora_amd: unsupported BatchNorm shape ({R}, {C}) {x.dtype}")
-        scratch = torch.empty(sb, dtype=torch.uint8, device=x.device)
-        st = lib.mtlora_bn_relu_fwd(L.ptr(x), L.ptr(w), L.ptr(b), L.ptr(running_mean), L.ptr(running_var), float(momentum),
-                                    float(eps), int(relu), L.ptr(y), L.ptr(saves[0]), L.ptr(saves[1]), L.ptr(saves[2]),
-                                    L.ptr(saves[3]), R, C, L.dtype_code(x), L.ptr(scratch), sb, L.stream_ptr())
-        L.check(st, "mtlora_bn_relu_fwd")
+        if part is not None:
+            st = lib.mtlora_bn_relu_fwd_from_partials(L.ptr(x), L.ptr(w), L.ptr(b), L.ptr(running_mean), L.ptr(running_var),
+                                                      float(momentum), float(eps), int(relu), L.ptr(y), L.ptr(saves[0]),
+                                                      L.ptr(saves[1]), L.ptr(saves[2]), L.ptr(saves[3]), R, C, L.dtype_code(x),
+                                                      L.ptr(part), part.shape[0], part.numel() * 4, L.stream_ptr())
+            L.check(st, "mtlora_bn_relu_fwd_from_partials")
+        else:
+            scratch = torch.empty(sb, dtype=torch.uint8, device=x.device)
+            st = lib.mtlora_bn_relu_fwd(L.ptr(x), L.ptr(w), L.ptr(b), L.ptr(running_mean), L.ptr(running_var), float(momentum),
+                                        float(eps), int(relu), L.ptr(y), L.ptr(saves[0]), L.ptr(saves[1]), L.ptr(saves[2]),
+                                        L.ptr(saves[3]), R, C, L.dtype_code(x), L.ptr(scratch), sb, L.stream_ptr())
+            L.check(st, "mtlora_bn_relu_fwd")
         ctx.save_for_backward(x, saves)
         ctx.relu = relu
         return y
@@ -1161,7 +1171,7 @@
                                     int(ctx.relu), L.ptr(dx), L.ptr(dg), L.ptr(db), R, C, L.dtype_code(x), L.ptr(scratch), sb,
                                     L.stream_ptr())
         L.check(st, "mtlora_bn_relu_bwd")
-        return dx, dg, db, None, None, None, None, None
+        return dx, dg, db, None, None, None, None, None, None
 
 
 class ResidualDropPathFn(torch.autograd.Function):
@@ -1528,7 +1538,8 @@
 class PlainLinearFn(torch.autograd.Function):
 
     @staticmethod
-    def forward(ctx, x, weight, bias, splits: int, zero_bias_grad: bool, cdtype, col_index=None, n_cols=0, pad_rows=0):
+    def forward(ctx, x, weight, bias, splits: int, zero_bias_grad: bool, cdtype, col_index=None, n_cols=0, pad_rows=0,
+                bn_stats: bool = False):
         L.require_gpu(x, weight)
         M, K = x.shape
         w, bias_l = _layout_weight(weight, bias, cdtype, col_index, n_cols, pad_rows)
@@ -1543,19 +1554,32 @@
         ctxbuf = torch.empty(max(ctx_bytes, 16), dtype=torch.uint8, device=x.device)
         y = torch.empty((M, N), dtype=cdtype, device=x.device)
         bf = None if bias_l is None else bias_l.float().contiguous()
-        st = lib.mtlora_linear_fwd(ctypes.byref(d), L.ptr(x), L.ptr_array(None), L.ptr(w), L.ptr(bf), L.ptr(None), L.ptr(None),
-                                   L.ptr_array(None), L.ptr_array(None), L.ptr(y), L.ptr_array(None), L.ptr(ctxbuf), ctx_bytes,
-                                   L.stream_ptr())
-        L.check(st, "mtlora_linear_fwd (rank 0)")
+        part = None
+        if bn_stats:
+            nblk = lib.mtlora_linear_fwd_stats_blocks(ctypes.byref(d))
+            if nblk < 0:
+                raise RuntimeError(f"mtlora_amd: no column statistics for the plain linear M={M} K={K} N={N} {cdtype}")
+            part = torch.empty((nblk, 2, N), dtype=torch.float32, device=x.device)
+            st = lib.mtlora_linear_fwd_stats(ctypes.byref(d), L.ptr(x), L.ptr(w), L.ptr(bf), L.ptr(y), L.ptr(part), part.numel() * 4,
+                                             L.stream_ptr())
+            L.check(st, "mtlora_linear_fwd_stats")
+        else:
+            st = lib.mtlora_linear_fwd(ctypes.byref(d), L.ptr(x), L.ptr_array(None), L.ptr(w), L.ptr(bf), L.ptr(None), L.ptr(None),
+                                       L.ptr_array(None), L.ptr_array(None), L.ptr(y), L.ptr_array(None), L.ptr(ctxbuf), ctx_bytes,
+                                       L.stream_ptr())
+            L.check(st, "mtlora_linear_fwd (rank 0)")
         ctx.save_for_backward(x, w, ctxbuf)
         ctx.wlayout = (col_index, pad_rows)
         ctx.meta, ctx.splits, ctx.zero_bias_grad = meta, splits, zero_bias_grad
         ctx.has_bias, ctx.wdtype = bias is not None, weight.dtype
         ctx.bdtype = None if bias is None else bias.dtype
+        if part is not None:
+            ctx.mark_non_differentiable(part)
+            return y, part
         return y
 
     @staticmethod
-    def backward(ctx, gy):
+    def backward(ctx, gy, _gpart=None):
         x, w, ctxbuf = ctx.saved_tensors
         gy = gy.contiguous()
         M, K = x.shape
@@ -1590,7 +1614,7 @@
             return _unlayout_grads(dw, db, *ctx.wlayout)
 
         dw, db = wgrads()
-        return dx, dw, db, None, None, None, None, None, None
+        return dx, dw, db, None, None, None, None, None, None, None
 
 
 def gemm_tn(a: torch.Tensor, b: torch.Tensor) -> torch.Tensor:
@@ -1613,18 +1637,22 @@
 
 
 _PLAIN_VIA_KNT = os.environ.get("MTLORA_HEAD_GEMM", "knt") != "blas"
-
-
-def _big_linear(x, weight, bias, S, feeds_batchnorm, cdtype, col_index=None, pad_rows=0):
+BN_EPILOGUE = os.environ.get("MTLORA_BN_EPILOGUE", "1") != "0"
+
+
+def _big_linear(x, weight, bias, S, feeds_batchnorm, cdtype, col_index=None, pad_rows=0, bn_stats=False):
     K, N = x.shape[1], weight.shape[0] + pad_rows
     if (_PLAIN_VIA_KNT and cdtype in _HOT_DTYPES and K % 8 == 0 and N % 8 == 0
             and x.dtype == cdtype):
+        if bn_stats and cdtype in (torch.bfloat16, torch.float16):
+            return PlainLinearFn.apply(x, weight, bias, S, feeds_batchnorm, cdtype, col_index, K, pad_rows, True)
         return PlainLinearFn.apply(x, weight, bias, S, feeds_batchnorm, cdtype, col_index, K, pad_rows)
     return SplitKLinearFn.apply(x, weight, bias, S, feeds_batchnorm, cdtype, col_index, K, pad_rows)
 
 
 def linear_big_m(x: torch.Tensor, weight: torch.Tensor, bias: Optional[torch.Tensor],
-                 feeds_batchnorm: bool = False, col_index: Optional[torch.Tensor] = None, pad_rows: int = 0) -> torch.Tensor:
+                 feeds_batchnorm: bool = False, col_index: Optional[torch.Tensor] = None, pad_rows: int = 0,
+                 bn_stats: bool = False):
     M = x.shape[0]
     if x.dim() == 2 and x.is_cuda and weight.requires_grad and torch.is_grad_enabled() and M >= 1 and x.is_contiguous():
         S = 1
@@ -1638,8 +1666,8 @@
         if torch.is_autocast_enabled("cuda"):
             dt = torch.get_autocast_dtype("cuda")
             with torch.autocast("cuda", enabled=False):
-                return _big_linear(x.to(dt), weight, bias, S, feeds_batchnorm, dt, col_index, pad_rows)
-        return _big_linear(x, weight, bias, S, feeds_batchnorm, x.dtype, col_index, pad_rows)
+                return _big_linear(x.to(dt), weight, bias, S, feeds_batchnorm, dt, col_index, pad_rows, bn_stats and feeds_batchnorm)
+        return _big_linear(x, weight, bias, S, feeds_batchnorm, x.dtype, col_index, pad_rows, bn_stats and feeds_batchnorm)
     if col_index is not None:
         weight = weight.new_zeros(weight.shape[0], x.shape[1]).index_copy(1, col_index, weight)
     if pad_rows:
diff --git a/mtlora_amd/mtl_harness.py b/mtlora_amd/mtl_harness.py
--- a/mtlora_amd/mtl_harness.py
+++ b/mtlora_amd/mtl_harness.py
@@ -148,12 +148,13 @@
             cat = torch.cat([x[0]] + [F.interpolate(m, (Hh, Ww), mode="bilinear") for m in x[1:]], 1)
             t = cat.permute(0, 2, 3, 1).reshape(B * Hh * Ww, cat.shape[1])
             col_idx = None
-        h = Fn.linear_big_m(t, w2d, c0.bias, feeds_batchnorm=bn.training, col_index=col_idx)
+        h = Fn.linear_big_m(t, w2d, c0.bias, feeds_batchnorm=bn.training, col_index=col_idx, bn_stats=bn.training and Fn.BN_EPILOGUE)
+        h, part = h if isinstance(h, tuple) else (h, None)
         if bn.training and bn.track_running_stats and bn.num_batches_tracked is not None:
             bn.num_batches_tracked.add_(1)
         if bn.training and h.is_cuda and h.dtype in (torch.float32, torch.bfloat16, torch.float16) and h.shape[1] % 8 == 0:
             h = BatchNormReluFn.apply(h, bn.weight, bn.bias, bn.running_mean, bn.running_var, bn.momentum, bn.eps,
-                                      getattr(self, "relu", True))
+                                      getattr(self, "relu", True), part)
         else:
             h = F.batch_norm(h, bn.running_mean, bn.running_var, bn.weight, bn.bias, bn.training or not bn.track_running_stats,
                              bn.momentum, bn.eps)
```
